# lms-07/LGTEUN

Hardware: AMD Instinct MI355X
Metric: train image-pairs/sec, GF-2 4-band 128x128, K=4, bs=32/GPU (higher is better)
Workload: dtype f32 (GEMMs and the local mixer: split 16-bit MFMA -- f16 pairs in the forward FFN, the W2 products of its backward and P V, bf16 triples elsewhere -- fp32 accumulate; fp32-equivalent); 1 GPU; BASELINE configs[1]: C=4, MS 32x32, PAN 128x128, K=4, 32 pairs/GPU, train step = fwd + L1 + bwd + Adam + StepLR tick; mode=faithful, global_batch=32, parallelism=dp1, dropout=True

## Files before the change

### include/lgteun_hip.h

```cpp
#ifndef LGTEUN_HIP_H
#define LGTEUN_HIP_H

#include <stddef.h>
#include <stdint.h>

#ifdef __cplusplus
extern "C" {
#endif

#define LG_TENSORS_SHARED 12
#define LG_TENSORS_PER_STAGE 119

#define LG_FLAG_FAITHFUL 1
#define LG_FLAG_SAVE 2
#define LG_FLAG_DROPOUT 4

#define LG_FLAG_BWD_LGT 8
#define LG_FLAG_BWD_DATA 16

#define LG_FLAG_CHAINED 32

#define LG_FLAG_DEFER_DEAD 64

#define LG_FLAG_STAGEWISE 128

#define LG_FLAG_LIVE_APART 256

enum lg_kernel_id {
    LG_K_NONE = 0, LG_K_FFN1, LG_K_FFN2, LG_K_FFT, LG_K_ATTN, LG_K_UPFUSE, LG_K_DOWN, LG_K_EMBED, LG_K_TAIL, LG_K_DATASTEP,
    LG_K_FFN1_BWD, LG_K_FFN2_BWD, LG_K_FFT_BWD, LG_K_ATTN_BWD, LG_K_WGRAD, LG_K_BATCH, LG_K_SCENE_GATHER, LG_K_SCENE_BLEND, LG_K_COUNT
};

typedef struct lg_config {
    int32_t C;
    int32_t K;
    int32_t H, W;
    int32_t precision;
    uint32_t variant;
} lg_config;

#define LG_VAR_FFN_IMPL_MASK 3u
#define LG_VAR_FFN_STRIP 1u
#define LG_VAR_FFN_SAVE_MASK (3u << 2)
#define LG_VAR_FFN_SAVE3 (1u << 2)
#define LG_VAR_FFN_SAVE5 (2u << 2)
#define LG_VAR_FFN_BWD32_PAIR (1u << 4)
#define LG_VAR_FFN_DWBWD_TILE (1u << 5)
#define LG_VAR_ATTN_BWD_R3 (1u << 6)
#define LG_VAR_DSTEP_TILES (1u << 7)
#define LG_VAR_ATTN_FWD_VALU (1u << 8)
#define LG_VAR_FFN_BF16X3 (1u << 9)
#define LG_VAR_FFT_FULL (1u << 10)
#define LG_VAR_FFN_BWD_BF16X3 (1u << 11)
#define LG_VAR_ATTN_BWD_CORE_M (1u << 12)
#define LG_VAR_FFN_XS (1u << 13)
#define LG_VAR_ATTN_BF16X3 (1u << 14)
#define LG_VAR_FFN_H3_RECOMPUTE (1u << 15)
#define LG_VAR_ATTN_BWD_RESTATS (1u << 16)
#define LG_VAR_REDUCE_PER_BLOCK (1u << 17)
#define LG_VAR_ALL 0x3ffffu

typedef struct lg_plan lg_plan;

const char* lg_version(void);
#define LG_ABI_VERSION 2
int32_t lg_abi_version(void);
const char* lg_last_error(void);

int lg_plan_create(const lg_config* cfg, const int64_t* offsets, int32_t n_offsets, lg_plan** out);
void lg_plan_destroy(lg_plan* plan);
int lg_plan_describe(const lg_plan* plan, char* buf, size_t n);
size_t lg_workspace_bytes(const lg_plan* plan, int32_t B, int32_t train);

int lgteun_forward(const lg_plan* plan, const float* params, const float* ms, const float* pan, float* out,
                   void* workspace, size_t workspace_bytes, int32_t B, int32_t flags, uint64_t seed, void* stream);

int lgteun_dead_forward(const lg_plan* plan, const float* params, void* workspace, size_t workspace_bytes, int32_t B, int32_t flags,
                        uint64_t seed, void* stream);

int lgteun_backward(const lg_plan* plan, const float* params, float* grads, const float* ms, const float* pan,
                    const float* dout, void* workspace, size_t workspace_bytes, int32_t B, int32_t flags,
                    uint64_t seed, void* stream);

int lg_l1_loss(const float* out, const float* gt, float* dout, float* loss_accum, int64_t n_local, int64_t n_global,
               float scale, void* stream);

int lg_adam_step(float* params, const float* grads, float* exp_avg, float* exp_avg_sq, const int64_t* ranges,
                 int32_t n_ranges, int64_t max_range, int32_t step, float lr, float beta1, float beta2, float eps,
                 float grad_scale, void* stream);

int lg_l2_loss(const float* out, const float* gt, float* dout, float* loss_accum, int64_t n_local, int64_t n_global,
               float scale, void* stream);

#define LG_OPT_ADAM 0
#define LG_OPT_ADAMW 1
#define LG_OPT_SGD 2
#define LG_OPT_RMSPROP 3
#define LG_OPT_AMSGRAD 1
#define LG_OPT_NESTEROV 2
#define LG_OPT_CENTERED 4
int lg_optim_step(float* params, const float* grads, float* state0, float* state1, float* state2, const int64_t* ranges,
                  int32_t n_ranges, int64_t max_range, int32_t step, int32_t algo, int32_t flags, double lr, double h0, double h1,
                  double eps, double weight_decay, double grad_scale, void* stream);

size_t lg_grad_norm_workspace_bytes(int32_t n_ranges, int64_t max_range);
int lg_grad_norm(const float* grads, const int64_t* ranges, int32_t n_ranges, int64_t max_range, double max_norm, float* out,
                 void* workspace, size_t workspace_bytes, void* stream);

int lg_optim_step_ex(float* params, const float* grads, float* state0, float* state1, float* state2, const int64_t* ranges,
                     int32_t n_ranges, int64_t max_range, int32_t step, int32_t algo, int32_t flags, double lr, double h0, double h1,
                     double eps, double weight_decay, double grad_scale, const float* clip_coef, float* ema, double ema_decay,
                     int32_t plain_adam, void* stream);

int lg_prof_enable(int32_t kernel_id, int32_t max_launches);
int lg_prof_reset(void);
void lg_prof_pause(int32_t paused);
int lg_prof_read(double* total_ms, int64_t* launches);
void lg_prof_disable(void);
const char* lg_kernel_name(int32_t kernel_id);

int lg_dropout_mask(uint64_t seed, int32_t stage, int32_t blk, int64_t first, int64_t n, float* out, void* stream);

int lg_op_resample(const float* x, float* y, int32_t planes, int32_t hi, int32_t wi, int32_t mode, void* stream);
int lg_op_data_step(const lg_plan* plan, const float* params, int32_t stage, const float* z_in, const float* ms,
                    const float* pan, float* z_out, float* tmp, int32_t B, void* stream);
int lg_op_lgt(const lg_plan* plan, const float* params, int32_t stage, const float* z, float* out, void* workspace,
              size_t workspace_bytes, int32_t B, int32_t flags, uint64_t seed, void* stream);
int lg_op_lgt_stages(const lg_plan* plan, const float* params, int32_t stage0, int32_t n, const float* z, float* out, void* workspace,
                     size_t workspace_bytes, int32_t B, int32_t flags, uint64_t seed, int32_t grid_cap, void* stream);
int lg_workspace_deadout(const lg_plan* plan, int32_t B, int32_t train, size_t* offset, size_t* stage_stride);
int lg_debug_live_slot(const lg_plan* plan, int32_t B, int32_t train, size_t* out53);
int lg_debug_stage_runs(int32_t kind, int32_t units, int32_t per_stage, int32_t grid, int32_t split, int32_t* out, int32_t n_out);
int lg_debug_stage_decision(int32_t kind, int32_t h, int32_t w, int32_t Bs, int32_t n, int32_t grid_cap, int32_t* out8);
int lg_op_block(const lg_plan* plan, const float* params, int32_t stage, int32_t blk, int32_t which, const float* x,
                float* y, void* workspace, size_t workspace_bytes, int32_t B, void* stream);

int lg_op_block_bwd(const lg_plan* plan, const float* params, float* grads, int32_t stage, int32_t blk, int32_t which,
                    const float* x, const float* dy, float* dx, void* workspace, size_t workspace_bytes, int32_t B,
                    void* stream);

int lg_op_data_step_bwd(const lg_plan* plan, const float* params, float* grads, int32_t stage, const float* z_in, const float* ms,
                        const float* pan, const float* dz_out, float* dz_in, void* workspace, size_t workspace_bytes, int32_t B,
                        void* stream);
int lg_op_lgt_bwd(const lg_plan* plan, const float* params, float* grads, int32_t stage, const float* z, const float* dout, float* dz,
                  void* workspace, size_t workspace_bytes, int32_t B, int32_t flags, uint64_t seed, void* stream);

#define LG_IQA_PEAK 2047.5
#define LG_IQA_SSIM_TAPS 11
#define LG_IQA_SSIM_SIGMA 1.5
#define LG_IQA_Q_BLOCK 8
#define LG_IQA_RATIO 4
#define LG_IQA_QNR_BLOCK 32
#define LG_IQA_MTF_TAPS 41
#define LG_IQA_MTF_GAIN 0.15
#define LG_IQA_MAX_BANDS 16
size_t lg_iqa_workspace_bytes(int32_t B, int32_t C, int32_t H, int32_t W, int32_t no_ref);
int lg_iqa_ref(const float* pred, const float* gt, double* out, int32_t B, int32_t C, int32_t H, int32_t W, float scale,
               void* workspace, size_t workspace_bytes, void* stream);
int lg_iqa_no_ref(const float* pred, const float* pan, const float* ms, double* out, int32_t B, int32_t C, int32_t H, int32_t W,
                  float scale, void* workspace, size_t workspace_bytes, void* stream);
int lg_iqa_mtf_taps(double* out41);

#define LG_IQA_Q2N_BLOCK 32
#define LG_IQA_Q2N_MAX_BANDS 8
size_t lg_iqa_ext_workspace_bytes(int32_t B, int32_t C, int32_t H, int32_t W);
int lg_iqa_ref_ext(const float* pred, const float* gt, double* out, int32_t B, int32_t C, int32_t H, int32_t W, float scale,
                   void* workspace, size_t workspace_bytes, void* stream);
int lg_iqa_q2n(const float* gt, const float* fused, double* out, int32_t B, int32_t C, int32_t H, int32_t W, float scale,
               void* workspace, size_t workspace_bytes, void* stream);

size_t lg_qnr_workspace_bytes(int32_t B, int32_t C, int32_t H, int32_t W);
int lg_qnr_stats(const float* out, const float* pan, const float* ms, const float* pan_l, double* q, double* table, int32_t B, int32_t C,
                 int32_t H, int32_t W, void* workspace, size_t workspace_bytes, void* stream);
int lg_qnr_grad(const float* out, const float* pan, const double* table, float* dout, float* loss_accum, double* indices, int32_t B,
                int64_t B_global, int32_t C, int32_t H, int32_t W, float scale, int32_t accumulate, const void* workspace,
                size_t workspace_bytes, void* stream);

size_t lg_recloss_workspace_bytes(int32_t B, int32_t C, int32_t H, int32_t W);
int lg_sam_loss(const float* out, const float* gt, float* dout, float* loss_accum, int32_t B, int64_t B_global, int32_t C, int32_t H, int32_t W,
                float scale, int32_t accumulate, void* workspace, size_t workspace_bytes, void* stream);
int lg_ssim_loss(const float* out, const float* gt, float* dout, float* loss_accum, int32_t B, int64_t B_global, int32_t C, int32_t H, int32_t W,
                 float scale, float data_range, int32_t accumulate, void* workspace, size_t workspace_bytes, void* stream);

#define LG_DT_U8 0
#define LG_DT_U16 1
#define LG_DT_F32 2
int lg_pyr_down2(const void* pan, float* pan_l, int64_t planes, int32_t H, int32_t W, int32_t dtype, void* stream);
int lg_batch_assemble(const void* pan, const void* lr, const void* mul, const float* pan_l, int64_t N, const int32_t* idx, int64_t idx_offset,
                      const uint32_t* flips, float* o_pan, float* o_lr, float* o_mul, float* o_pan_l, int32_t B, int32_t C, int32_t H, int32_t W,
                      int32_t h, int32_t w, int32_t dtype, float divisor, int32_t n_div, float post_scale, void* stream);

int lg_fir_decimate4(const void* in, void* out, const double* taps, int64_t planes, int32_t H, int32_t W, int32_t n_taps, int32_t phase,
                     int32_t dtype, int32_t out_f32, void* stream);
int lg_window_assemble(const void* pan, const void* lr, const void* mul, const int32_t* origins, int64_t n_windows, int64_t first,
                       const uint32_t* flips, float* o_pan, float* o_lr, float* o_mul, float* o_pan_l, int32_t B, int32_t C, int32_t Hs, int32_t Ws,
                       int32_t P, int32_t Q, int32_t dtype, float divisor, int32_t n_div, float post_scale, void* stream);

int lg_scene_gather(const void* pan, const void* ms, const int32_t* origins, int64_t n_tiles, int64_t first, float* o_pan, float* o_ms,
                    int32_t B, int32_t C, int32_t H, int32_t W, int32_t th, int32_t tw, int32_t dtype, float divisor, int32_t n_div,
                    float post_scale, void* stream);
int lg_scene_blend(const float* tiles, float* scene, int64_t first, int32_t B, int32_t C, int32_t H, int32_t W, int32_t th, int32_t tw,
                   int32_t overlap, void* stream);
int lg_scene_to_u16(const float* src, uint16_t* dst, int64_t n, float scale, void* stream);

#define LG_CLASSICAL_SFIM 0
#define LG_CLASSICAL_GSA 1
size_t lg_classical_workspace_bytes(int32_t B, int32_t C, int32_t h, int32_t w, int32_t method);
int lg_interp23_up4(const float* ms, float* out, int32_t B, int32_t C, int32_t h, int32_t w, void* stream);
int lg_sfim(const float* ms, const float* pan, float* out, int32_t B, int32_t C, int32_t h, int32_t w, void* workspace, size_t workspace_bytes,
            void* stream);
int lg_gsa(const float* ms, const float* pan, float* out, double* stats, int32_t B, int32_t C, int32_t h, int32_t w, void* workspace,
           size_t workspace_bytes, void* stream);
int lg_wavelet(const float* ms, const float* pan, float* out, int32_t B, int32_t C, int32_t h, int32_t w, void* stream);
// ... 16 lines not shown
```

### lgteun_amd/_lib.py

```python
import ctypes
import os
from ctypes import POINTER, c_char_p, c_double, c_float, c_int32, c_int64, c_size_t, c_uint64, c_void_p

_HERE = os.path.dirname(os.path.abspath(__file__))
LIB_PATH = os.environ.get('LGTEUN_HIP_LIB') or os.path.join(_HERE, '_lgteun_hip.so')

LG_FLAG_FAITHFUL = 1
LG_FLAG_SAVE = 2
LG_FLAG_DROPOUT = 4
LG_FLAG_BWD_LGT = 8
LG_FLAG_BWD_DATA = 16
LG_FLAG_CHAINED = 32
LG_FLAG_DEFER_DEAD = 64
LG_FLAG_STAGEWISE = 128
LG_FLAG_LIVE_APART = 256
KERNEL_IDS = {n: i for i, n in enumerate(['none', 'ffn1', 'ffn', 'fft', 'attn', 'upfuse', 'down', 'embed', 'tail', 'datastep', 'ffn1_bwd',
                                           'ffn2_bwd', 'fft_bwd', 'attn_bwd', 'wgrad', 'batch', 'scene_gather', 'scene_blend'])}


class LgConfig(ctypes.Structure):
    _fields_ = [('C', c_int32), ('K', c_int32), ('H', c_int32), ('W', c_int32), ('precision', c_int32), ('variant', ctypes.c_uint32)]


LG_VAR_FFN_STRIP = 1
LG_VAR_FFN_SAVE3, LG_VAR_FFN_SAVE5 = 1 << 2, 2 << 2
LG_VAR_FFN_BWD32_PAIR, LG_VAR_FFN_DWBWD_TILE, LG_VAR_ATTN_BWD_R3 = 1 << 4, 1 << 5, 1 << 6
LG_VAR_DSTEP_TILES = 1 << 7
LG_VAR_ATTN_FWD_VALU = 1 << 8
LG_VAR_FFN_BF16X3 = 1 << 9
LG_VAR_FFT_FULL = 1 << 10
LG_VAR_FFN_BWD_BF16X3 = 1 << 11
LG_VAR_ATTN_BWD_CORE_M = 1 << 12
LG_VAR_FFN_XS = 1 << 13
LG_VAR_ATTN_BF16X3 = 1 << 14
LG_VAR_FFN_H3_RECOMPUTE = 1 << 15
LG_VAR_ATTN_BWD_RESTATS = 1 << 16
LG_VAR_REDUCE_PER_BLOCK = 1 << 17
LG_OPT_ADAM, LG_OPT_ADAMW, LG_OPT_SGD, LG_OPT_RMSPROP = 0, 1, 2, 3
LG_OPT_AMSGRAD, LG_OPT_NESTEROV, LG_OPT_CENTERED = 1, 2, 4
LG_DT_U8, LG_DT_U16, LG_DT_F32 = 0, 1, 2
LG_CLASSICAL_SFIM, LG_CLASSICAL_GSA = 0, 1
LG_MTFGLP_GLP, LG_MTFGLP_HPM, LG_MTFGLP_CBD = 0, 1, 2
LG_ABI_VERSION = 2


def variant_from_env(env=None):
    env = os.environ if env is None else env
    v = {'strip': LG_VAR_FFN_STRIP, 'tile': 2, 'xp': 3}.get(env.get('LG_FFN_IMPL', ''), 0)
    v |= {'3': LG_VAR_FFN_SAVE3, '5': LG_VAR_FFN_SAVE5}.get(env.get('LG_FFN_SAVE', ''), 0)
    if env.get('LG_FFN_BWD32') == 'pair':
        v |= LG_VAR_FFN_BWD32_PAIR
    if env.get('LG_FFN_DWBWD') == 'tile':
        v |= LG_VAR_FFN_DWBWD_TILE
    if env.get('LG_ATTN_BWD') in ('old', 'r3'):
        v |= LG_VAR_ATTN_BWD_R3
    if env.get('LG_DSTEP') == 'tiles':
        v |= LG_VAR_DSTEP_TILES
    if env.get('LG_ATTN_FWD', '') == 'valu':
        v |= LG_VAR_ATTN_FWD_VALU
    if env.get('LG_FFN_SPLIT', '') == 'bf16x3':
        v |= LG_VAR_FFN_BF16X3
    if env.get('LG_FFT', '') == 'full':
        v |= LG_VAR_FFT_FULL
    if env.get('LG_FFN_BWD_SPLIT', '') == 'bf16x3':
        v |= LG_VAR_FFN_BWD_BF16X3
    if env.get('LG_ATTN_BWD_CORE', '') == 'm':
        v |= LG_VAR_ATTN_BWD_CORE_M
    if env.get('LG_FFN_FWD', '') == 'xs':
        v |= LG_VAR_FFN_XS
    if env.get('LG_ATTN_SPLIT', '') == 'bf16x3':
        v |= LG_VAR_ATTN_BF16X3
    if env.get('LG_FFN_H3', '') == 'recompute':
        v |= LG_VAR_FFN_H3_RECOMPUTE
    if env.get('LG_ATTN_BWD_STATS', '') == 'recompute':
        v |= LG_VAR_ATTN_BWD_RESTATS
    if env.get('LG_REDUCE', '') == 'per_block':
        v |= LG_VAR_REDUCE_PER_BLOCK
    return v


class LgteunHipError(RuntimeError):
    pass


_lib = None

SIGNATURES = {
    'lg_version': (c_char_p, []),
    'lg_abi_version': (c_int32, []),
    'lg_last_error': (c_char_p, []),
    'lg_plan_create': (c_int32, [POINTER(LgConfig), POINTER(c_int64), c_int32, POINTER(c_void_p)]),
    'lg_plan_destroy': (None, [c_void_p]),
    'lg_plan_describe': (c_int32, [c_void_p, c_char_p, c_size_t]),
    'lg_workspace_bytes': (c_size_t, [c_void_p, c_int32, c_int32]),
    'lgteun_forward': (c_int32, [c_void_p, c_void_p, c_void_p, c_void_p, c_void_p, c_void_p, c_size_t, c_int32, c_int32,
                                 c_uint64, c_void_p]),
    'lgteun_backward': (c_int32, [c_void_p, c_void_p, c_void_p, c_void_p, c_void_p, c_void_p, c_void_p, c_size_t, c_int32,
                                  c_int32, c_uint64, c_void_p]),
    'lgteun_dead_forward': (c_int32, [c_void_p, c_void_p, c_void_p, c_size_t, c_int32, c_int32, c_uint64, c_void_p]),
    'lg_l1_loss': (c_int32, [c_void_p, c_void_p, c_void_p, c_void_p, c_int64, c_int64, c_float, c_void_p]),
    'lg_adam_step': (c_int32, [c_void_p, c_void_p, c_void_p, c_void_p, c_void_p, c_int32, c_int64, c_int32, c_float, c_float,
                               c_float, c_float, c_float, c_void_p]),
    'lg_l2_loss': (c_int32, [c_void_p, c_void_p, c_void_p, c_void_p, c_int64, c_int64, c_float, c_void_p]),
    'lg_optim_step': (c_int32, [c_void_p, c_void_p, c_void_p, c_void_p, c_void_p, c_void_p, c_int32, c_int64, c_int32, c_int32, c_int32,
                                c_double, c_double, c_double, c_double, c_double, c_double, c_void_p]),
    'lg_grad_norm_workspace_bytes': (c_size_t, [c_int32, c_int64]),
    'lg_grad_norm': (c_int32, [c_void_p, c_void_p, c_int32, c_int64, c_double, c_void_p, c_void_p, c_size_t, c_void_p]),
    'lg_optim_step_ex': (c_int32, [c_void_p, c_void_p, c_void_p, c_void_p, c_void_p, c_void_p, c_int32, c_int64, c_int32, c_int32, c_int32,
                                   c_double, c_double, c_double, c_double, c_double, c_double, c_void_p, c_void_p, c_double, c_int32,
                                   c_void_p]),
    'lg_op_resample': (c_int32, [c_void_p, c_void_p, c_int32, c_int32, c_int32, c_int32, c_void_p]),
    'lg_op_data_step': (c_int32, [c_void_p, c_void_p, c_int32, c_void_p, c_void_p, c_void_p, c_void_p, c_void_p, c_int32,
                                  c_void_p]),
    'lg_op_lgt': (c_int32, [c_void_p, c_void_p, c_int32, c_void_p, c_void_p, c_void_p, c_size_t, c_int32, c_int32, c_uint64,
                            c_void_p]),
    'lg_op_lgt_stages': (c_int32, [c_void_p, c_void_p, c_int32, c_int32, c_void_p, c_void_p, c_void_p, c_size_t, c_int32, c_int32, c_uint64,
                                   c_int32, c_void_p]),
    'lg_debug_stage_runs': (c_int32, [c_int32, c_int32, c_int32, c_int32, c_int32, POINTER(c_int32), c_int32]),
    'lg_debug_stage_decision': (c_int32, [c_int32, c_int32, c_int32, c_int32, c_int32, c_int32, POINTER(c_int32)]),
    'lg_workspace_deadout': (c_int32, [c_void_p, c_int32, c_int32, POINTER(c_size_t), POINTER(c_size_t)]),
    'lg_debug_live_slot': (c_int32, [c_void_p, c_int32, c_int32, POINTER(c_size_t)]),
    'lg_op_block': (c_int32, [c_void_p, c_void_p, c_int32, c_int32, c_int32, c_void_p, c_void_p, c_void_p, c_size_t, c_int32,
                              c_void_p]),
    'lg_dropout_mask': (c_int32, [c_uint64, c_int32, c_int32, c_int64, c_int64, c_void_p, c_void_p]),
    'lg_prof_enable': (c_int32, [c_int32, c_int32]),
    'lg_prof_reset': (c_int32, []),
    'lg_prof_pause': (None, [c_int32]),
    'lg_prof_read': (c_int32, [POINTER(ctypes.c_double), POINTER(c_int64)]),
    'lg_prof_disable': (None, []),
    'lg_kernel_name': (c_char_p, [c_int32]),
    'lg_op_data_step_bwd': (c_int32, [c_void_p, c_void_p, c_void_p, c_int32, c_void_p, c_void_p, c_void_p, c_void_p, c_void_p, c_void_p,
                                      c_size_t, c_int32, c_void_p]),
    'lg_op_lgt_bwd': (c_int32, [c_void_p, c_void_p, c_void_p, c_int32, c_void_p, c_void_p, c_void_p, c_void_p, c_size_t, c_int32, c_int32,
                                c_uint64, c_void_p]),
    'lg_op_block_bwd': (c_int32, [c_void_p, c_void_p, c_void_p, c_int32, c_int32, c_int32, c_void_p, c_void_p, c_void_p, c_void_p,
                                  c_size_t, c_int32, c_void_p]),
    'lg_iqa_workspace_bytes': (c_size_t, [c_int32, c_int32, c_int32, c_int32, c_int32]),
    'lg_iqa_ref': (c_int32, [c_void_p, c_void_p, c_void_p, c_int32, c_int32, c_int32, c_int32, c_float, c_void_p, c_size_t, c_void_p]),
    'lg_iqa_no_ref': (c_int32, [c_void_p, c_void_p, c_void_p, c_void_p, c_int32, c_int32, c_int32, c_int32, c_float, c_void_p, c_size_t,
                                c_void_p]),
    'lg_iqa_mtf_taps': (c_int32, [c_void_p]),
    'lg_iqa_ext_workspace_bytes': (c_size_t, [c_int32, c_int32, c_int32, c_int32]),
    'lg_iqa_ref_ext': (c_int32, [c_void_p, c_void_p, c_void_p, c_int32, c_int32, c_int32, c_int32, c_float, c_void_p, c_size_t, c_void_p]),
    'lg_iqa_q2n': (c_int32, [c_void_p, c_void_p, c_void_p, c_int32, c_int32, c_int32, c_int32, c_float, c_void_p, c_size_t, c_void_p]),
    'lg_qnr_workspace_bytes': (c_size_t, [c_int32, c_int32, c_int32, c_int32]),
    'lg_qnr_stats': (c_int32, [c_void_p, c_void_p, c_void_p, c_void_p, c_void_p, c_void_p, c_int32, c_int32, c_int32, c_int32, c_void_p, c_size_t,
                               c_void_p]),
    'lg_qnr_grad': (c_int32, [c_void_p, c_void_p, c_void_p, c_void_p, c_void_p, c_void_p, c_int32, c_int64, c_int32, c_int32, c_int32, c_float,
                              c_int32, c_void_p, c_size_t, c_void_p]),
    'lg_recloss_workspace_bytes': (c_size_t, [c_int32, c_int32, c_int32, c_int32]),
    'lg_sam_loss': (c_int32, [c_void_p, c_void_p, c_void_p, c_void_p, c_int32, c_int64, c_int32, c_int32, c_int32, c_float, c_int32, c_void_p,
                              c_size_t, c_void_p]),
    'lg_ssim_loss': (c_int32, [c_void_p, c_void_p, c_void_p, c_void_p, c_int32, c_int64, c_int32, c_int32, c_int32, c_float, c_float, c_int32,
                               c_void_p, c_size_t, c_void_p]),
    'lg_pyr_down2': (c_int32, [c_void_p, c_void_p, c_int64, c_int32, c_int32, c_int32, c_void_p]),
    'lg_batch_assemble': (c_int32, [c_void_p, c_void_p, c_void_p, c_void_p, c_int64, c_void_p, c_int64, c_void_p, c_void_p, c_void_p, c_void_p,
                                    c_void_p, c_int32, c_int32, c_int32, c_int32, c_int32, c_int32, c_int32, c_float, c_int32, c_float, c_void_p]),
    'lg_fir_decimate4': (c_int32, [c_void_p, c_void_p, c_void_p, c_int64, c_int32, c_int32, c_int32, c_int32, c_int32, c_int32, c_void_p]),
    'lg_window_assemble': (c_int32, [c_void_p, c_void_p, c_void_p, c_void_p, c_int64, c_int64, c_void_p, c_void_p, c_void_p, c_void_p, c_void_p,
                                     c_int32, c_int32, c_int32, c_int32, c_int32, c_int32, c_int32, c_float, c_int32, c_float, c_void_p]),
    'lg_scene_gather': (c_int32, [c_void_p, c_void_p, c_void_p, c_int64, c_int64, c_void_p, c_void_p, c_int32, c_int32, c_int32, c_int32, c_int32,
                                  c_int32, c_int32, c_float, c_int32, c_float, c_void_p]),
    'lg_scene_blend': (c_int32, [c_void_p, c_void_p, c_int64, c_int32, c_int32, c_int32, c_int32, c_int32, c_int32, c_int32, c_void_p]),
    'lg_scene_to_u16': (c_int32, [c_void_p, c_void_p, c_int64, c_float, c_void_p]),
    'lg_classical_workspace_bytes': (c_size_t, [c_int32, c_int32, c_int32, c_int32, c_int32]),
    'lg_interp23_up4': (c_int32, [c_void_p, c_void_p, c_int32, c_int32, c_int32, c_int32, c_void_p]),
    'lg_sfim': (c_int32, [c_void_p, c_void_p, c_void_p, c_int32, c_int32, c_int32, c_int32, c_void_p, c_size_t, c_void_p]),
    'lg_gsa': (c_int32, [c_void_p, c_void_p, c_void_p, c_void_p, c_int32, c_int32, c_int32, c_int32, c_void_p, c_size_t, c_void_p]),
    'lg_wavelet': (c_int32, [c_void_p, c_void_p, c_void_p, c_int32, c_int32, c_int32, c_int32, c_void_p]),
    'lg_wavelet_taps': (c_int32, [c_void_p]),
    'lg_mtfglp_workspace_bytes': (c_size_t, [c_int32, c_int32, c_int32, c_int32, c_int32, c_int32]),
    'lg_mtf_glp': (c_int32, [c_void_p, c_void_p, c_void_p, c_void_p, c_void_p, c_int32, c_int32, c_int32, c_int32, c_int32, c_int32, c_int32, c_void_p,
                             c_size_t, c_void_p]),
    'lg_bdsd_workspace_bytes': (c_size_t, [c_int32, c_int32, c_int32, c_int32, c_int32]),
    'lg_bdsd': (c_int32, [c_void_p, c_void_p, c_void_p, c_void_p, c_void_p, c_int32, c_void_p, c_int32, c_int32, c_int32, c_int32, c_int32, c_int32, c_void_p,
                          c_size_t, c_void_p]),
}


def lib():
    global _lib
    if _lib is None:
        if not os.path.exists(LIB_PATH):
            raise LgteunHipError(
                f'HIP extension not built: {LIB_PATH} is missing. Run `make` (or __graft_entry__.build()). '
                'lgteun_amd has no CPU/PyTorch fallback.')
        L = ctypes.CDLL(LIB_PATH)
        for name, (res, args) in SIGNATURES.items():
            fn = getattr(L, name)
            fn.restype = res
            fn.argtypes = args
        got = int(L.lg_abi_version())
        if got != LG_ABI_VERSION:
            raise LgteunHipError(f'{LIB_PATH}: ABI version {got}, this binding was written for {LG_ABI_VERSION} (include/lgteun_hip.h): rebuild with `make`')
        _lib = L
    return _lib


def check(rc, what):
    if rc != 0:
        msg = lib().lg_last_error().decode(errors='replace')
        raise LgteunHipError(f'{what} failed (rc={rc}): {msg}')
```

### lgteun_amd/csrc/api.hip

```cpp
#include <stdarg.h>
#include <stdio.h>
#include <stdlib.h>
#include <string.h>

#include "abi.h"
#include "kernels.h"
#include "workspace.h"
#include "forward.h"
#include "backward.h"

static thread_local char g_err[512] = "";

void lg_set_error(const char* fmt, ...) {
    va_list ap;
    va_start(ap, fmt);
    vsnprintf(g_err, sizeof(g_err), fmt, ap);
    va_end(ap);
}

extern "C" const char* lg_version(void) { return "lgteun_hip 0.2 (gfx950)"; }
extern "C" int32_t lg_abi_version(void) { return LG_ABI_VERSION; }
extern "C" const char* lg_last_error(void) { return g_err; }

static void lg_plan_stage_batch(lg_plan* p);
// ... 44 lines not shown
    free(plan->off);
    delete plan;
}

extern "C" int lg_plan_describe(const lg_plan* plan, char* buf, size_t n) {
    if (!plan) { lg_set_error("plan_describe: null argument"); return -1; }
    return lg_describe_route(plan->cfg, plan->route, buf, n);
}

extern "C" size_t lg_workspace_bytes(const lg_plan* plan, int32_t B, int32_t train) {
    if (!plan || B <= 0 || train < 0 || train > 2) return 0;
    NetBufs nb;
    carve(plan, B, train, nullptr, nb);
    size_t fwd = nb.bytes;
    if (train) fwd += bwd_workspace_bytes(plan, B);
    return fwd;
}

extern "C" int lg_workspace_deadout(const lg_plan* plan, int32_t B, int32_t train, size_t* offset, size_t* stage_stride) {
    if (!plan || B <= 0 || train < 0 || train > 2 || !offset || !stage_stride) { lg_set_error("workspace_deadout: invalid argument"); return -1; }
    NetBufs nb;
    char base[1];
    carve(plan, B, train, base, nb);
    *offset = (size_t)(reinterpret_cast<char*>(nb.deadout) - base);
    *stage_stride = (plan->stage_batch && train != 2) ? (size_t)B * plan->cfg.C * plan->cfg.H * plan->cfg.W * sizeof(float) : 0;
    return 0;
}

extern "C" int lg_debug_live_slot(const lg_plan* plan, int32_t B, int32_t train, size_t* out53) {
    if (!plan || B <= 0 || train < 0 || train > 2 || !out53) { lg_set_error("debug_live_slot: invalid argument"); return -1; }
    NetBufs nb;
    char base[1];
    carve(plan, B, train, base, nb);
    const NetBufs lv = live_view(nb);
    size_t* o = out53;
    *o++ = nb.bytes; *o++ = train ? bwd_workspace_bytes(plan, B) : 0; *o++ = nb.live_s0;
    auto off = [&](const float* p) { return (size_t)(reinterpret_cast<const char*>(p) - base); };
    for (int j = 0; j < LG_NBLK; ++j) {
        const BlockBufs &a = nb.blk[j], &l = lv.blk[j];
        const float* pa[5] = {a.xin, a.xmid, a.xout, a.g, a.o2};
        const float* pl[5] = {l.xin, l.xmid, l.xout, l.g, l.o2};
        for (int f = 0; f < 5; ++f) { *o++ = off(pa[f]); *o++ = off(pl[f]); }
    }
    return 0;
}

extern "C" int lgteun_backward(const lg_plan* plan, const float* params, float* grads, const float* ms, const float* pan,
                               const float* dout, void* workspace, size_t workspace_bytes, int32_t B, int32_t flags, uint64_t seed,
                               void* stream) {
    if (!plan || !params || !grads || !ms || !pan || !dout || !workspace || B <= 0) { lg_set_error("backward: null/invalid argument"); return -1; }
    if ((flags & LG_FLAG_CHAINED) && (flags & (LG_FLAG_BWD_LGT | LG_FLAG_BWD_DATA))) {
        lg_set_error("backward: LG_FLAG_BWD_LGT / LG_FLAG_BWD_DATA do not apply to LG_FLAG_CHAINED");
        return -2;
    }
    NetBufs nb;
    if (int rc = carve_checked("backward", plan, B, (flags & LG_FLAG_CHAINED) ? 2 : 1, workspace, workspace_bytes, nb)) return rc;
    return net_backward(plan, params, grads, ms, pan, dout, nb, (char*)workspace + nb.bytes, B, flags, seed, (hipStream_t)stream);
}

extern "C" int lg_op_resample(const float* x, float* y, int32_t planes, int32_t hi, int32_t wi, int32_t mode, void* stream) {
    if (!x || !y || planes <= 0 || hi <= 0 || wi <= 0 || mode < 0 || mode > 2) { lg_set_error("op_resample: invalid argument"); return -1; }
    if (mode == 0 && ((hi & 1) || (wi & 1))) { lg_set_error("op_resample: x0.5 needs even sizes"); return -2; }
    return launch_resample(mode, x, y, planes, hi, wi, (hipStream_t)stream);
}

extern "C" int lg_op_data_step(const lg_plan* plan, const float* params, int32_t stage, const float* z_in, const float* ms,
                               const float* pan, float* z_out, float* tmp, int32_t B, void* stream) {
    if (!plan || !params || !z_in || !ms || !pan || !z_out || !tmp || stage < 0 || stage >= plan->cfg.K) { lg_set_error("op_data_step: invalid argument"); return -1; }
    const lg_config& c = plan->cfg;
    size_t q = (size_t)B * c.C * c.H * c.W / 4;
    return data_step_fwd(plan, params, stage, z_in, ms, pan, z_out, tmp, tmp + q, tmp + 2 * q, tmp + 3 * q, B, (hipStream_t)stream);
}

extern "C" int lg_op_lgt(const lg_plan* plan, const float* params, int32_t stage, const float* z, float* out, void* workspace,
                         size_t workspace_bytes, int32_t B, int32_t flags, uint64_t seed, void* stream) {
    if (!plan || !params || !z || !out || !workspace || stage < 0 || stage >= plan->cfg.K) { lg_set_error("op_lgt: invalid argument"); return -1; }
    NetBufs nb;
    if (int rc = carve_checked("op_lgt", plan, B, (flags & LG_FLAG_SAVE) ? 1 : 0, workspace, workspace_bytes, nb)) return rc;
    nb = live_view(nb);
    if (int rc = prep_stages(plan, params, stage, stage + 1, nb, (hipStream_t)stream)) return rc;
    return lgt_fwd(plan, params, stage, z, out, nb, B, flags, seed, (hipStream_t)stream);
}

extern "C" int lg_op_lgt_stages(const lg_plan* plan, const float* params, int32_t stage0, int32_t n, const float* z, float* out, void* workspace,
                                size_t workspace_bytes, int32_t B, int32_t flags, uint64_t seed, int32_t grid_cap, void* stream) {
    if (!plan || !params || !z || !out || !workspace || B <= 0 || stage0 < 0 || n < 1 || stage0 + n > plan->cfg.K || grid_cap < 0) { lg_set_error("op_lgt_stages: invalid argument"); return -1; }
    if (flags & ~LG_FLAG_DROPOUT) { lg_set_error("op_lgt_stages: only LG_FLAG_DROPOUT applies (nothing is saved)"); return -2; }
    if (n > 1 && (!plan->stage_batch || n > plan->cfg.K - 1)) { lg_set_error("op_lgt_stages: this plan runs one stage per pass (lg_plan_stage_batch), or n > K-1"); return -2; }
    NetBufs nb;
    if (int rc = carve_checked("op_lgt_stages", plan, B, 0, workspace, workspace_bytes, nb)) return rc;
    hipStream_t s = (hipStream_t)stream;
    if (int rc = prep_stages(plan, params, stage0, stage0 + n, nb, s)) return rc;
    return lgt_fwd(plan, params, stage0, z, out, nb, B, flags, seed, s, n, (long)B * plan->cfg.C * plan->cfg.H * plan->cfg.W, grid_cap);
}

extern "C" int lg_debug_stage_runs(int32_t kind, int32_t units, int32_t per_stage, int32_t grid, int32_t split, int32_t* out, int32_t n_out) {
    if (kind < 0 || kind > 1 || units <= 0 || per_stage <= 0 || units % per_stage || grid <= 0 || !out || n_out < 0 || (int64_t)units * grid >= (1ll << 31)) {
        lg_set_error("debug_stage_runs: invalid argument");
        return -1;
    }
    const bool uneven = kind == 0 ? split != 0 : split != 4;
    if (!uneven && grid > units) { lg_set_error("debug_stage_runs: more workgroups than units"); return -1; }
    if (uneven && ((grid & 1) || (kind == 0 ? 2 * units < grid : units < grid) || (kind == 1 && (split < 1 || split > 7)))) { lg_set_error("debug_stage_runs: an uneven split needs an even grid, a unit per workgroup and 1 <= eighths <= 7"); return -2; }
    int rows = 0;
    for (int wg = 0; wg < grid; ++wg) {
        const StageRun r = !uneven ? stage_run_even(units, grid, wg) : (kind == 0 ? stage_run_pairs(units, grid, wg) : stage_run_chunk(units, grid, wg, split));
        int seg0 = r.run0;
        do {
            const int st = seg0 / per_stage, seg1 = stage_seg_end(st, r.run1, per_stage);
            if (rows < n_out) { int32_t* o = out + 5 * (size_t)rows; o[0] = wg; o[1] = seg0; o[2] = seg1; o[3] = st; o[4] = r.base; }
            ++rows;
            seg0 = seg1;
        } while (seg0 < r.run1);
    }
    return rows;
}

extern "C" int lg_debug_stage_decision(int32_t kind, int32_t h, int32_t w, int32_t Bs, int32_t n, int32_t grid_cap, int32_t* out8) {
    if ((kind != 0 && kind != 8 && kind != 16) || h <= 0 || w <= 0 || Bs <= 0 || n < 1 || grid_cap < 0 || !out8 || (int64_t)Bs * n * h * w >= (1ll << 31)) { lg_set_error("debug_stage_decision: invalid argument"); return -1; }
    if (kind == 0) {
        const XrGeo q = ffn_xr_geometry(h, w, Bs * n, Bs, n, grid_cap);
        const int sh = q.dS ? 1 : 0;
        const int32_t o[8] = {q.dS != 0, q.dS, q.nstrips >> sh, (Bs * q.tiles_x * q.strips_y) >> sh, q.grid, q.SH, q.tiles_x, q.strips_y};
        memcpy(out8, o, sizeof(o));
    } else {
        if ((h & 7) || (w & 7) || (Bs * (h / 8) * (w / 8)) % 4) { lg_set_error("debug_stage_decision: not whole window quads per stage"); return -2; }
        const AttnMGeo q = attn_m_geometry(kind, h, w, Bs * n, n, grid_cap, 2);
        const int32_t o[8] = {q.uneven != 0, q.uneven ? q.uneven : 4, q.nquads, q.nquads / n, q.grid, q.nwin, 0, 0};
        memcpy(out8, o, sizeof(o));
    }
    return 0;
}

extern "C" int lg_op_block(const lg_plan* plan, const float* params, int32_t stage, int32_t blk, int32_t which, const float* x,
                           float* y, void* workspace, size_t workspace_bytes, int32_t B, void* stream) {
    if (!plan || !params || !x || !y || !workspace || stage < 0 || stage >= plan->cfg.K || blk < 0 || blk > 4 || which < 0 || which > 2) {
        lg_set_error("op_block: invalid argument");
        return -1;
    }
    hipStream_t s = (hipStream_t)stream;
    NetBufs nb;
    int rc;
    if ((rc = carve_checked("op_block", plan, B, 0, workspace, workspace_bytes, nb))) return rc;
    nb = live_view(nb);
    Blk k = nb.block(plan, params, nullptr, stage, blk);
    BlockBufs& bb = k.b;
    if (which == 0 || which == 1) {
        if ((rc = launch_ln_split(bb.e, x, k.p(B_LN1G), k.p(B_LN1B), bb.g, B, bb.h * bb.w, s))) return rc;
    }
    if (which == 0) {
        FftArgs f;
        f.g = bb.g; f.o = y; f.amp = nullptr; f.pha = nullptr; f.sgn = nullptr; f.scratch = nb.fft_scratch;
        f.ampw = k.p(B_AMPW); f.ampb = k.p(B_AMPB); f.phaw = k.p(B_PHAW); f.phab = k.p(B_PHAB);
        f.ch = bb.e / 2; f.planes = B * f.ch; f.n = bb.h; f.h = bb.h; f.w = bb.w; f.full = plan->route.fft_full;
        return launch_fftmix(f, s);
    }
    if ((rc = prep_stages(plan, params, stage, stage + 1, nb, s))) return rc;
    if (which == 1) {
        bb.xin = const_cast<float*>(x);
        bb.xmid = y;
        return block_mixer_fwd(k, B, 0, 0, s);
    }
    bb.xmid = const_cast<float*>(x);
    bb.xout = y;
    return block_ffn_fwd(k, nullptr, B, 0, s);
}

extern "C" int lg_op_block_bwd(const lg_plan* plan, const float* params, float* grads, int32_t stage, int32_t blk, int32_t which,
                               const float* x, const float* dy, float* dx, void* workspace, size_t workspace_bytes, int32_t B,
                               void* stream) {
    if (!plan || !params || !grads || !x || !dy || !dx || !workspace || stage < 0 || stage >= plan->cfg.K || blk < 0 || blk > 4 ||
        which < 0 || which > 2) {
        lg_set_error("op_block_bwd: invalid argument");
        return -1;
    }
    hipStream_t s = (hipStream_t)stream;
    NetBufs nb;
    int rc;
    if ((rc = carve_checked("op_block_bwd", plan, B, 1, workspace, workspace_bytes, nb))) return rc;
    nb = live_view(nb);
    Blk k = nb.block(plan, params, grads, stage, blk);
    BlockBufs& bb = k.b;
    if (which == 0 || which == 1) {
        if ((rc = launch_ln_split(bb.e, x, k.p(B_LN1G), k.p(B_LN1B), bb.g, B, bb.h * bb.w, s))) return rc;
        if ((rc = prep_stages(plan, params, stage, stage + 1, nb, s))) return rc;
        bb.xin = const_cast<float*>(x);
        if ((rc = block_mixer_fwd(k, B, LG_FLAG_SAVE, 0, s))) return rc;
    } else {
        bb.xmid = const_cast<float*>(x);
        if ((rc = prep_stages(plan, params, stage, stage + 1, nb, s))) return rc;
        if ((rc = block_ffn_fwd(k, nullptr, B, LG_FLAG_SAVE, s))) return rc;
    }
    return op_block_bwd(k, which, dy, dx, (char*)workspace + nb.bytes, B, s);
}

extern "C" int lg_op_data_step_bwd(const lg_plan* plan, const float* params, float* grads, int32_t stage, const float* z_in,
                                   const float* ms, const float* pan, const float* dz_out, float* dz_in, void* workspace,
                                   size_t workspace_bytes, int32_t B, void* stream) {
    if (!plan || !params || !grads || !z_in || !ms || !pan || !dz_out || !dz_in || !workspace || B <= 0 || stage < 0 || stage >= plan->cfg.K) {
        lg_set_error("op_data_step_bwd: invalid argument");
        return -1;
    }
    hipStream_t s = (hipStream_t)stream;
    NetBufs nb;
    int rc;
    if ((rc = carve_checked("op_data_step_bwd", plan, B, 1, workspace, workspace_bytes, nb))) return rc;
    if ((rc = data_step_fwd(plan, params, stage, z_in, ms, pan, nb.Z[stage + 1], nb.t1[stage], nb.r[stage], nb.s1[stage], nb.pr, B, s))) return rc;
    return op_data_step_bwd(plan, params, grads, stage, nb, (char*)workspace + nb.bytes, z_in, pan, dz_out, dz_in, B, s);
}

extern "C" int lg_op_lgt_bwd(const lg_plan* plan, const float* params, float* grads, int32_t stage, const float* z, const float* dout,
                             float* dz, void* workspace, size_t workspace_bytes, int32_t B, int32_t flags, uint64_t seed, void* stream) {
    if (!plan || !params || !grads || !z || !dout || !dz || !workspace || B <= 0 || stage < 0 || stage >= plan->cfg.K) {
        lg_set_error("op_lgt_bwd: invalid argument");
        return -1;
    }
    if (flags & ~LG_FLAG_DROPOUT) { lg_set_error("op_lgt_bwd: only LG_FLAG_DROPOUT applies"); return -2; }
    hipStream_t s = (hipStream_t)stream;
    NetBufs nb;
    int rc;
    if ((rc = carve_checked("op_lgt_bwd", plan, B, 1, workspace, workspace_bytes, nb))) return rc;
    nb = live_view(nb);
    if ((rc = prep_stages(plan, params, stage, stage + 1, nb, s))) return rc;
    if ((rc = lgt_fwd(plan, params, stage, z, nb.deadout, nb, B, flags | LG_FLAG_SAVE, seed, s))) return rc;
    return op_lgt_bwd(plan, params, grads, stage, nb, (char*)workspace + nb.bytes, z, dout, dz, B, flags, seed, s);
}
```

### lgteun_amd/csrc/bwd_kernels.h

```cpp
#pragma once
#include "common.h"

struct WgradArgs {
    const void* Y;
    const void* X;
    float* dW;
    float* db;
    long P;
    int ldy, ldx, ldw;
    int N, K;
    int n_valid, k_valid;
    int ybf, xbf;
    int xgelu;
};
size_t wgrad_slab_floats(int N, int K, long P);
#define PIXEL_PART_WGS 2048
size_t chan_partial_floats(int C, int B, int H, int W);
struct ChanReduce {
    float* dst[14];
    float* dst2[14];
    int stride[14];
    int NK, C, nslices;
    unsigned allc_mask;
};
// ... 125 lines not shown
    float* du;
    const float* dskip;
    float* dx;
    const float* w;
    int B, H, W;
};
int launch_down_bwd_a(int E, const DownBwdArgs& a, hipStream_t s);
int launch_down_bwd_b(int E, const DownBwdArgs& a, hipStream_t s);

struct UpFuseBwdArgs {
    const float* dy;
    float* dt;
    float* dskip;
    float* v;
    float* dxb;
    float* tmp;
    const float *fw, *upw;
    int B, H, W;
};
int launch_upfuse_bwd_a(int E, const UpFuseBwdArgs& a, hipStream_t s);
int launch_upfuse_bwd_b(int E, const UpFuseBwdArgs& a, hipStream_t s);

struct FfnDwBwdArgs {
    const float* dy;
    const void* g3;
    const void* h2;
    void* dh2;
    int hbf;
    int pre;
    const float *w3t;
    const float* dww;
    float *slab_w, *slab_b;
    float *d_dww, *d_dwb;
    int B, h, w;
};
size_t ffn_dw_bwd_slab_floats(int e, int B, int h, int w);
int launch_ffn_dw_bwd(int e, const FfnDwBwdArgs& a, hipStream_t s);
struct Ffn1BwdArgs {
    const void* dh2;
    const void* g1;
    const float* x;
    const float* dy;
    void* dh1;
    float* y2;
    float* dx;
    const float *w2t, *w1t, *ln2g, *ln2b;
    float *d_ln2g, *d_ln2b;
    float* part;
    float *w1slab, *d_w1, *d_b1;
    float *w2slab, *d_w2, *d_b2;
    long P;
    int hbf;
    int pre;
    const float* w1;
    void* wsplit;
};
#define FFN1_BWD_WGS 512
inline bool ffn1_bwd_fuses_w1(int e) { return e <= 32; }
#ifndef LG_FW2
#define LG_FW2 0
#endif
inline bool ffn1_bwd_fuses_w2(int e, int pre) { return LG_FW2 && pre && e == 16; }
int launch_ffn1_bwd(int e, Ffn1BwdKernel k, const Ffn1BwdArgs& a, hipStream_t s);
int launch_ffn1_bwd_x32(const Ffn1BwdArgs& a, const float* w1, void* wsplit, hipStream_t s);
struct Ffn1BwdXArgs {
    const void* dh2;
    int hbf;
    const float* x;
    const float* dy;
    float* dx;
    const float *w1, *b1;
    const float *w2t, *w1t;
    const float *ln2g, *ln2b;
    float* slab;
    float *d_w1, *d_b1, *d_w2, *d_b2, *d_ln2g, *d_ln2b;
    long P;
    const float* scales = nullptr;
};
inline int ffn1_bwd_x_wgs(int e) { return e == 16 ? 512 : 256; }
size_t ffn1_bwd_x_slab_floats(int e);
int launch_ffn1_bwd_xs(int e, const Ffn1BwdXArgs& a, hipStream_t s);
struct FfnDwBwdXArgs {
    const float* dy;
    const void* h3;
    const void* h2;
    void* dh2;
    int hbf;
    const float* w3t;
    const float* dww;
    const float* dwb = nullptr;
    float* slab;
    float *d_dww, *d_dwb, *d_w3, *d_b3;
    int B, h, w;
    float* dh2_max = nullptr;
};
#define FFN_DW_BWD_X_WGS 512
#define FFN_DW_BWD_X_DB 576
#define FFN_DW_BWD_X_W3 640
#define FFN_DW_BWD_X_B3 1664
#define FFN_DW_BWD_X_ROW 1680
#define FFN_DW_BWD_X32_ROW 2720
inline size_t ffn_dw_bwd_x_slab_floats(int e) { return (size_t)FFN_DW_BWD_X_WGS * (e == 16 ? FFN_DW_BWD_X_ROW : FFN_DW_BWD_X32_ROW); }
int launch_ffn_dw_bwd_xs(int e, const FfnDwBwdXArgs& a, hipStream_t s);
#define FFN_DW_BWD_H_WGS 512
#define FFN_DW_BWD_H_ROW 848
inline size_t ffn_dw_bwd_h_slab_floats() { return (size_t)2 * FFN_DW_BWD_H_WGS * FFN_DW_BWD_H_ROW; }
int launch_ffn_dw_bwd_h(const FfnDwBwdXArgs& a, hipStream_t s);
inline int reduce_ffn_dw_bwd_slab(const FfnDwBwdXArgs& a, int e, int nhalf, int gx, int r_db, int r_w3, int r_b3, int row, hipStream_t s) {
    const int n1 = 4 * e, nh = n1 / nhalf;
    ReduceJob j;
    j.dst2 = nullptr; j.nslices = gx; j.slice_stride = row;
    int rc = 0;
    for (int half = 0; half < nhalf && !rc; ++half) {
        const float* base = a.slab + (size_t)half * gx * row;
        auto job = [&](int off, float* dst, int rows, int cols, int ld) {
            j.slab = base + off; j.dst = dst; j.rows = rows; j.cols = cols; j.row_stride = cols; j.ld = ld; j.rows_valid = rows; j.cols_valid = cols;
            return launch_reduce_job(j, s);
        };
        rc = job(0, a.d_dww + (size_t)half * nh * 9, nh, 9, 9);
        if (!rc) rc = job(r_db, a.d_dwb + half * nh, 1, nh, nh);
        if (!rc) rc = job(r_w3, a.d_w3 + half * nh, e, nh, n1);
        if (!rc && half == 0) rc = job(r_b3, a.d_b3, 1, e, e);
    }
    return rc;
}
int launch_transpose(const float* src, float* dst, int rows, int cols, hipStream_t s);
int launch_transpose3(const float* const* src, float* const* dst, const int* rows, const int* cols, int njobs, hipStream_t s, float* const* clear = nullptr, int nclear = 0);

struct ProjO2BwdArgs {
    const float* dy;
    float* do2;
    float* dym;
    const float* projw;
    int HW;
    long total;
    int dropout;
    uint64_t seed;
};
int launch_proj_o2_bwd(int e, const ProjO2BwdArgs& a, hipStream_t s);

struct FftBwdArgs {
    const float* do2;
    const float* sgn;
    const float* amp;
    const float* pha;
    float* dg;
    float* scratch;
    const float *ampw, *ampb, *phaw, *phab;
    float *d_ampw, *d_ampb, *d_phaw, *d_phab;
    float* part;
    int planes, ch, n;
    int h, w;
    int full = 0;
};
size_t fft_bwd_part_floats(int planes, int h, int w);
int launch_fftmix_bwd(const FftBwdArgs& a, hipStream_t s);

struct AttnBwdArgs {
    const float* x;
    const float* dy;
    const float* dym;
    const float* o2;
    const float* dg;
    float* dx;
    float* cat;
    float* y1;
    float* dqkv;
    const float* pos;
    const float* unused = nullptr;
    float* dpos_slab;
    const float *ln1g, *ln1b, *qkvw, *qkvb, *projw;
    float *d_ln1g, *d_ln1b;
    float *d_qkvw, *d_qkvb;
    float* part;
    int B, h, w;
    const float* so = nullptr;
    const float* sl = nullptr;
    float* stats = nullptr;
    int core_m = 0;
};
int launch_attn_bwd_core_m(int e, const AttnBwdArgs& a, int grid, int nwin, int ngroups, hipStream_t s);
#ifndef LG_ATTN_FUSE_QKV
#define LG_ATTN_FUSE_QKV 1
#endif
constexpr bool attn_bwd_fuses_qkv(int e) { return LG_ATTN_FUSE_QKV && e == 16; }
inline size_t attn_bwd_part_floats(int e) { return (size_t)PIXEL_PART_WGS * 2 * e + (attn_bwd_fuses_qkv(e) ? (size_t)1024 * ((3 * e / 2) * (e / 2) + 3 * e / 2) : 0); }
int attn_bwd_grid(int e, int B, int h, int w);
int launch_attn_bwd(int e, const AttnBwdArgs& a, hipStream_t s);

struct ProjO2BwdKArgs {
    const float* dy;
    float* do2;
    uint32_t* keep;
    const float* projw;
    float* slab;
    float* d_projb;
    int HW;
    long total;
    uint64_t seed;
};
#ifndef PROJ_O2_K_WGS
#define PROJ_O2_K_WGS 512
#endif
int launch_proj_o2_bwd_k(int e, const ProjO2BwdKArgs& a, hipStream_t s);
struct AttnBwdFArgs {
    const float* x;
    const float* dy;
    const uint32_t* keep;
    const float* o2;
    const float* dg;
    float* dx;
    const float* pos;
    const float *ln1g, *ln1b, *qkvw, *qkvb, *projw;
    const float* so = nullptr;
    const float* sl = nullptr;
    float* slab;
    float *d_pos, *d_qkvw, *d_qkvb, *d_projw, *d_ln1g, *d_ln1b;
    int B, h, w;
    unsigned rcp_nwx, rcp_nwy;
};
#define ATTN_BWD_F_WGS 256
#define ATTN_BWD_F_WQ 8192
#define ATTN_BWD_F_ROW (8192 + 192 + 24 + 256 + 32)
inline bool attn_bwd_fused(int e) { return e == 16; }
int attn_bwd_f_grid(int B, int h, int w);
int launch_attn_bwd_f(int e, const AttnBwdFArgs& a, hipStream_t s);
```

### lgteun_amd/csrc/k_bwd.hip

```cpp
#include <string.h>

#include "kernels.h"
#include "bwd_kernels.h"
#include "backward.h"

struct BwdBufs {
    float *dzA, *dzB, *gu3, *gs1, *gu1, *gr, *gd3, *gt1, *gd1;
    float *dx[3];
    float *dh2, *dh1, *y2, *do2, *dg, *dym, *cat, *y1, *dqkv;
    float *w3t[LG_NBLK], *w2t[LG_NBLK], *w1t[LG_NBLK], *wsp, *dt, *dskip, *v, *du;
    float* slab_arena;
    float* attn_stats;
    size_t slab_cap;
    ReduceQueue rq;
    size_t bytes;
};

static const size_t R3_DPOS_SLAB = 512 * POS_TABLE;
static size_t dpos_slab_floats() {
    const size_t f = (size_t)ATTN_BWD_F_WGS * ATTN_BWD_F_ROW;
    return f > R3_DPOS_SLAB ? f : R3_DPOS_SLAB;
}
static void carve_bwd(const lg_plan* plan, int B, void* base, BwdBufs& bb) {
    const lg_config& c = plan->cfg;
    Carver cv{reinterpret_cast<char*>(base), 0};
    const size_t P0 = (size_t)c.H * c.W * B, P1 = P0 / 4, E = 4 * (size_t)c.C, C = c.C;
    bb.dzA = cv.take(C * P0); bb.dzB = cv.take(C * P0); bb.gu3 = cv.take(C * P0);
    bb.gs1 = cv.take(C * P1); bb.gu1 = cv.take(C * P1); bb.gt1 = cv.take(C * P1); bb.gd1 = cv.take(C * P1);
    bb.gr = cv.take(C * P1 / 4); bb.gd3 = cv.take(C * P1 / 4);
    for (int i = 0; i < 3; ++i) bb.dx[i] = cv.take(P0 * E);
    bb.dh2 = cv.take(P0 * 4 * E); bb.dh1 = cv.take(P0 * 4 * E);
    bb.y2 = cv.take(P0 * E); bb.do2 = cv.take(P0 * E / 2); bb.dg = cv.take(P0 * E / 2);
    bb.dym = cv.take(P0 * E); bb.cat = cv.take(P0 * E); bb.y1 = cv.take(P0 * 16 > P0 * E / 2 ? P0 * 16 : P0 * E / 2);
    bb.dqkv = cv.take(P0 * 2 * E);
    bb.attn_stats = cv.take(P0 * 8);
    for (int j = 0; j < LG_NBLK; ++j) { bb.w3t[j] = cv.take(8 * E * 2 * E); bb.w2t[j] = cv.take(8 * E * 8 * E); bb.w1t[j] = cv.take(8 * E * 2 * E); }
    bb.wsp = cv.take(ffn_wsplit_bytes(32) / sizeof(float));
    size_t sl = wgrad_slab_floats((int)(8 * E), (int)(8 * E), (long)P0);
    size_t sl2 = wgrad_slab_floats(64, 64, (long)P0);
    size_t sl3 = ffn_dw_bwd_slab_floats((int)E, B, c.H, c.W);
    if (sl2 > sl) sl = sl2;
    size_t sl4 = chan_partial_floats(c.C, B, c.H, c.W);
    const size_t sl5 = (size_t)PIXEL_PART_WGS * (2 * 8 * c.C + 2 * c.C);
    if (sl5 > sl4) sl4 = sl5;
    if (sl4 > sl) sl = sl4;
    if (sl3 > sl) sl = sl3;
    for (const FfnRoute& fr : plan->route.ffn)
        if (fr.px == FFN1_BWD_XS && ffn1_bwd_x_slab_floats(fr.e) > sl) sl = ffn1_bwd_x_slab_floats(fr.e);
    if (ffn_dw_bwd_x_slab_floats(16) > sl) sl = ffn_dw_bwd_x_slab_floats(16);
    if (ffn_dw_bwd_x_slab_floats(32) > sl) sl = ffn_dw_bwd_x_slab_floats(32);
    if (ffn_dw_bwd_h_slab_floats() > sl) sl = ffn_dw_bwd_h_slab_floats();
    bb.slab_cap = LG_NBLK * (4 * sl + dpos_slab_floats());
    bb.slab_arena = cv.take(bb.slab_cap);
    bb.dt = cv.take(P0 * E); bb.dskip = cv.take(P0 * E); bb.v = cv.take(P1 * E); bb.du = cv.take(P1 * E);
    bb.bytes = cv.off;
}

size_t bwd_workspace_bytes(const lg_plan* plan, int B) {
    BwdBufs bb;
    carve_bwd(plan, B, nullptr, bb);
    return bb.bytes;
}

#define RC(x) do { int rc__ = (x); if (rc__) return rc__; } while (0)

struct ReduceQueueScope {
    explicit ReduceQueueScope(BwdBufs& bb, hipStream_t s, bool per_block) {
        bb.rq.init(bb.slab_arena, bb.slab_cap, s, per_block);
        reduce_queue_begin(&bb.rq);
    }
    ~ReduceQueueScope() { (void)reduce_queue_end(); }
};

static int wgrad(const void* Y, int ldy, const void* X, int ldx, float* dW, int ldw, float* db, long P, int N, int K, int nv, int kv,
                 int ybf, int xbf, BwdBufs& bb, hipStream_t s, int xgelu = 0) {
    float* slab = bb.rq.take(wgrad_slab_floats(N, K, P));
    if (!slab) return -3;
    WgradArgs a;
    a.Y = Y; a.X = X; a.dW = dW; a.db = db; a.P = P; a.ldy = ldy; a.ldx = ldx; a.ldw = ldw; a.N = N; a.K = K;
    a.n_valid = nv; a.k_valid = kv; a.ybf = ybf; a.xbf = xbf; a.xgelu = xgelu;
    return launch_wgrad(a, slab, s);
}

static int ffn_transposes(const Blk* blocks, int nk, BwdBufs& bb, hipStream_t s) {
    const float* tsrc[3 * LG_NBLK];
    float* tdst[3 * LG_NBLK];
    float* clear[LG_NBLK];
    int trows[3 * LG_NBLK], tcols[3 * LG_NBLK], n = 0, nclear = 0;
    for (int i = 0; i < nk; ++i) {
        const Blk& k = blocks[i];
        const int j = k.j, e = k.b.e, n1 = 4 * e;
        tsrc[n] = k.p(B_W3); tdst[n] = bb.w3t[j]; trows[n] = e; tcols[n] = n1; ++n;
        tsrc[n] = k.p(B_W2); tdst[n] = bb.w2t[j]; trows[n] = n1; tcols[n] = n1; ++n;
        tsrc[n] = k.p(B_W1); tdst[n] = bb.w1t[j]; trows[n] = n1; tcols[n] = e; ++n;
        if (k.pl->ffn(e).bwd_scales) clear[nclear++] = k.ffn_scales + 6;
    }
    return launch_transpose3(tsrc, tdst, trows, tcols, n, s, clear, nclear);
}

static int ffn_half_bwd(const Blk& k, BwdBufs& bb, const float* dy, float* tmp, int B, hipStream_t s) {
    const BlockBufs& fb = k.b;
    const FfnRoute& fr = k.pl->ffn(fb.e);
    const int j = k.j, e = fb.e, n1 = 4 * e;
    const int hbf = fr.hbf ? 1 : 0;
    const int pre = fr.pre ? 1 : 0;
    const long Pn = (long)B * fb.h * fb.w;
    float* fsc = fr.bwd_scales ? k.ffn_scales : nullptr;
    if (fr.dw == FFN_DWBWD_TILE) {
        FfnDwBwdArgs fd;
        fd.dy = dy; fd.g3 = pre ? fb.a3 : fb.g3; fd.h2 = fb.h2; fd.dh2 = bb.dh2; fd.w3t = bb.w3t[j]; fd.dww = k.p(B_DWW);
        fd.slab_w = bb.rq.take(ffn_dw_bwd_slab_floats(e, B, fb.h, fb.w));
        if (!fd.slab_w) return -3;
        fd.slab_b = fd.slab_w + ffn_dw_bwd_slab_floats(e, B, fb.h, fb.w) / 10 * 9;
        fd.d_dww = k.g(B_DWW); fd.d_dwb = k.g(B_DWB);
        fd.B = B; fd.h = fb.h; fd.w = fb.w; fd.hbf = hbf; fd.pre = pre;
        RC(launch_ffn_dw_bwd(e, fd, s));
    } else {
        const bool h3re = fr.dw == FFN_DWBWD_H;
        FfnDwBwdXArgs fk;
        fk.dy = dy; fk.h3 = h3re ? nullptr : fb.a3; fk.h2 = fb.h2; fk.dh2 = bb.dh2; fk.w3t = bb.w3t[j]; fk.dww = k.p(B_DWW); fk.dwb = k.p(B_DWB);
        fk.slab = bb.rq.take(h3re ? ffn_dw_bwd_h_slab_floats() : ffn_dw_bwd_x_slab_floats(e));
        if (!fk.slab) return -3;
        fk.d_dww = k.g(B_DWW); fk.d_dwb = k.g(B_DWB); fk.d_w3 = k.g(B_W3); fk.d_b3 = k.g(B_B3);
        fk.B = B; fk.h = fb.h; fk.w = fb.w; fk.hbf = hbf;
        fk.dh2_max = fsc ? fsc + 6 : nullptr;
        RC(h3re ? launch_ffn_dw_bwd_h(fk, s) : launch_ffn_dw_bwd_xs(e, fk, s));
    }
    if (fr.px == FFN1_BWD_XS) {
        Ffn1BwdXArgs fx;
        fx.scales = fsc;
        fx.dh2 = bb.dh2; fx.x = fb.xmid; fx.dy = dy; fx.dx = tmp;
        fx.w1 = k.p(B_W1); fx.b1 = k.p(B_B1); fx.w2t = bb.w2t[j]; fx.w1t = bb.w1t[j]; fx.ln2g = k.p(B_LN2G); fx.ln2b = k.p(B_LN2B);
        fx.slab = bb.rq.take(ffn1_bwd_x_slab_floats(e));
        if (!fx.slab) return -3;
        fx.d_w1 = k.g(B_W1); fx.d_b1 = k.g(B_B1); fx.d_w2 = k.g(B_W2); fx.d_b2 = k.g(B_B2); fx.d_ln2g = k.g(B_LN2G); fx.d_ln2b = k.g(B_LN2B);
        fx.P = Pn; fx.hbf = hbf;
        RC(launch_ffn1_bwd_xs(e, fx, s));
    } else {
        Ffn1BwdArgs f1;
        f1.dh2 = bb.dh2; f1.g1 = pre ? fb.a1 : fb.g1; f1.x = fb.xmid; f1.dy = dy; f1.dh1 = bb.dh1; f1.y2 = bb.y2; f1.dx = tmp;
        f1.w2t = bb.w2t[j]; f1.w1t = bb.w1t[j];
        f1.ln2g = k.p(B_LN2G); f1.ln2b = k.p(B_LN2B);
        f1.d_ln2g = k.g(B_LN2G); f1.d_ln2b = k.g(B_LN2B); f1.part = bb.rq.take((size_t)PIXEL_PART_WGS * 2 * e);
        if (!f1.part) return -3;
        f1.P = Pn; f1.hbf = hbf; f1.pre = pre;
        f1.w1 = nullptr; f1.wsplit = nullptr;
        if (fr.px == FFN1_BWD_X32) { f1.w1 = k.p(B_W1); f1.wsplit = bb.wsp; }
        f1.w1slab = nullptr; f1.d_w1 = nullptr; f1.d_b1 = nullptr;
        if (!fr.wgrad_w1) {
            f1.w1slab = bb.rq.take((size_t)FFN1_BWD_WGS * ((size_t)n1 * e + n1));
            if (!f1.w1slab) return -3;
            f1.d_w1 = k.g(B_W1); f1.d_b1 = k.g(B_B1);
        }
        f1.w2slab = nullptr; f1.d_w2 = nullptr; f1.d_b2 = nullptr;
        if (!fr.wgrad_w2) {
            f1.w2slab = bb.rq.take((size_t)FFN1_BWD_WGS * ((size_t)n1 * n1 + n1));
            if (!f1.w2slab) return -3;
            f1.d_w2 = k.g(B_W2); f1.d_b2 = k.g(B_B2);
        }
        RC(launch_ffn1_bwd(e, fr.px, f1, s));
    }
    if (fr.wgrad_w2) RC(wgrad(bb.dh2, n1, fb.a1, n1, k.g(B_W2), n1, k.g(B_B2), Pn, n1, n1, n1, n1, hbf, hbf, bb, s, pre));
    if (fr.wgrad_w1) RC(wgrad(bb.dh1, n1, bb.y2, e, k.g(B_W1), e, k.g(B_B1), Pn, n1, e, n1, e, hbf, 0, bb, s));
    if (fr.wgrad_w3) RC(wgrad(dy, e, fb.a3, n1, k.g(B_W3), n1, k.g(B_B3), Pn, e, n1, e, n1, 0, hbf, bb, s, pre));
    return 0;
}

static int fft_bwd_call(const Blk& k, const float* do2, float* dg, int B, hipStream_t s, float* part) {
    const BlockBufs& fb = k.b;
    const int hc = fb.e / 2;
    FftBwdArgs fa;
    fa.do2 = do2; fa.sgn = fb.sgn; fa.amp = fb.amp; fa.pha = fb.pha; fa.dg = dg; fa.scratch = k.fft_scratch;
    fa.ampw = k.p(B_AMPW); fa.ampb = k.p(B_AMPB); fa.phaw = k.p(B_PHAW); fa.phab = k.p(B_PHAB);
    fa.d_ampw = k.g(B_AMPW); fa.d_ampb = k.g(B_AMPB); fa.d_phaw = k.g(B_PHAW); fa.d_phab = k.g(B_PHAB);
    fa.ch = hc; fa.planes = B * hc; fa.n = fb.h; fa.h = fb.h; fa.w = fb.w; fa.part = part; fa.full = k.pl->route.fft_full;
    return launch_fftmix_bwd(fa, s);
}

static int mixer_half_bwd(const Blk& k, BwdBufs& bb, const float* tmp, float* dx_out, int B, int flags, uint64_t seed, hipStream_t s) {
    const BlockBufs& fb = k.b;
    const int e = fb.e, hc = e / 2;
    const long Pn = (long)B * fb.h * fb.w;
    const int drop = (flags & LG_FLAG_DROPOUT) ? 1 : 0;
    const MixerRoute& mr = k.pl->mixer(e);
    if (mr.bwd == ATTN_BWD_F) {
        uint32_t* keep = drop ? reinterpret_cast<uint32_t*>(bb.dym) : nullptr;
        ProjO2BwdKArgs pk;
        pk.dy = tmp; pk.do2 = bb.do2; pk.keep = keep; pk.projw = k.p(B_PROJW);
        pk.slab = bb.rq.take((size_t)PROJ_O2_K_WGS * e);
        if (!pk.slab) return -3;
        pk.d_projb = k.g(B_PROJB); pk.HW = fb.h * fb.w; pk.total = Pn; pk.seed = mix_seed(seed, k.st, k.j);
        RC(launch_proj_o2_bwd_k(e, pk, s));
        float* fpart = bb.rq.take(fft_bwd_part_floats(B * hc, fb.h, fb.w));
        if (!fpart) return -3;
        RC(fft_bwd_call(k, bb.do2, bb.dg, B, s, fpart));
        AttnBwdFArgs af;
        af.x = fb.xin; af.dy = tmp; af.keep = keep; af.o2 = fb.o2; af.dg = bb.dg; af.dx = dx_out;
        af.pos = k.p(B_POS); af.ln1g = k.p(B_LN1G); af.ln1b = k.p(B_LN1B); af.qkvw = k.p(B_QKVW); af.qkvb = k.p(B_QKVB); af.projw = k.p(B_PROJW);
        af.slab = bb.rq.take((size_t)ATTN_BWD_F_WGS * ATTN_BWD_F_ROW);
        if (!af.slab) return -3;
        af.d_pos = k.g(B_POS); af.d_qkvw = k.g(B_QKVW); af.d_qkvb = k.g(B_QKVB); af.d_projw = k.g(B_PROJW); af.d_ln1g = k.g(B_LN1G); af.d_ln1b = k.g(B_LN1B);
        af.B = B; af.h = fb.h; af.w = fb.w;
        if (mr.stats) { af.so = fb.att_o; af.sl = fb.att_l; }
        return launch_attn_bwd_f(e, af, s);
    }
    ProjO2BwdArgs po;
    po.dy = tmp; po.do2 = bb.do2; po.dym = drop ? bb.dym : nullptr; po.projw = k.p(B_PROJW);
    po.HW = fb.h * fb.w; po.total = Pn; po.dropout = drop; po.seed = mix_seed(seed, k.st, k.j);
    RC(launch_proj_o2_bwd(e, po, s));
    const float* dym = drop ? bb.dym : tmp;
    float* fpart = bb.rq.take(fft_bwd_part_floats(B * hc, fb.h, fb.w));
    if (!fpart) return -3;
    RC(fft_bwd_call(k, bb.do2, bb.dg, B, s, fpart));
    AttnBwdArgs at;
    at.x = fb.xin; at.dy = tmp; at.dym = dym; at.o2 = fb.o2; at.dg = bb.dg; at.dx = dx_out;
    at.cat = bb.cat; at.y1 = bb.y1; at.dqkv = bb.dqkv;
    at.pos = k.p(B_POS); at.dpos_slab = bb.rq.take(R3_DPOS_SLAB);
    if (!at.dpos_slab) return -3;
    at.ln1g = k.p(B_LN1G); at.ln1b = k.p(B_LN1B); at.qkvw = k.p(B_QKVW); at.qkvb = k.p(B_QKVB); at.projw = k.p(B_PROJW);
    at.d_ln1g = k.g(B_LN1G); at.d_ln1b = k.g(B_LN1B); at.part = bb.rq.take(attn_bwd_part_floats(e));
    at.d_qkvw = k.g(B_QKVW); at.d_qkvb = k.g(B_QKVB);
    if (attn_bwd_fuses_qkv(e)) at.y1 = nullptr;
    if (!at.part) return -3;
    at.B = B; at.h = fb.h; at.w = fb.w; at.core_m = mr.bwd == ATTN_BWD_R3_CORE_M ? 1 : 0; at.stats = bb.attn_stats;
    if (mr.stats) { at.so = fb.att_o; at.sl = fb.att_l; }
    RC(launch_attn_bwd(e, at, s));
    const int grid = attn_bwd_grid(e, B, fb.h, fb.w);
    RC(launch_reduce_slab(at.dpos_slab, grid, 1, POS_TABLE, k.g(B_POS), POS_TABLE, 1, POS_TABLE, s));
    RC(wgrad(dym, e, bb.cat, e, k.g(B_PROJW), e, k.g(B_PROJB), Pn, e, e, e, e, 0, 0, bb, s));
    if (!attn_bwd_fuses_qkv(e)) {
        const int y1ld = (hc + 15) / 16 * 16, dqld = (3 * hc + 15) / 16 * 16;
        RC(wgrad(bb.dqkv, dqld, bb.y1, y1ld, k.g(B_QKVW), hc, k.g(B_QKVB), Pn, dqld, y1ld, 3 * hc, hc, 0, 0,
                 bb, s));
    }
    return 0;
}

static int block_bwd(const Blk& k, BwdBufs& bb, const float* dy, float* tmp, float* dx_out, int B, int flags, uint64_t seed, hipStream_t s) {
    RC(ffn_half_bwd(k, bb, dy, tmp, B, s));
    RC(mixer_half_bwd(k, bb, tmp, dx_out, B, flags, seed, s));
    return bb.rq.block_end();
}

int op_block_bwd(const Blk& k, int which, const float* dy, float* dx, void* bwd_ws, int B, hipStream_t s) {
    BwdBufs bb;
    carve_bwd(k.pl, B, bwd_ws, bb);
    if (which == 0) return fft_bwd_call(k, dy, dx, B, s, bb.slab_arena);
    ReduceQueueScope rqs(bb, s, k.pl->route.reduce_per_block);
    int rc = which == 1 ? 0 : ffn_transposes(&k, 1, bb, s);
    if (!rc) rc = which == 1 ? mixer_half_bwd(k, bb, dy, dx, B, 0, 0, s) : ffn_half_bwd(k, bb, dy, dx, B, s);
    const int rc2 = reduce_queue_end();
    return rc ? rc : rc2;
}

static int data_step_bwd(const lg_plan* pl, const float* P, float* G, int st, const NetBufs& nb, BwdBufs& bb, const float* zin,
                         const float* pan, const float* g, float* dz, int B, hipStream_t s) {
    const lg_config& c = pl->cfg;
    const int planes = B * c.C, H = c.H, W = c.W;
    if (pl->route.dstep_fused) {
        DstepBwdArgs a;
        a.g = g; a.z = zin; a.pan = pan; a.t1 = nb.t1[st]; a.r = nb.r[st]; a.s1 = nb.s1[st]; a.dz = dz;
        a.d1w = P + pl->shared(S_D1W); a.d3w = P + pl->shared(S_D3W); a.dt1w = P + pl->shared(S_DT1W); a.dt3w = P + pl->shared(S_DT3W);
        a.dt3b = P + pl->shared(S_DT3B);
        a.rw = P + pl->shared(S_RW); a.rb = P + pl->shared(S_RB); a.rtw = P + pl->shared(S_RTW); a.rtb = P + pl->shared(S_RTB);
        a.eta = P + pl->eta(st);
        a.B = B; a.C = c.C; a.N = H;
        float* part = bb.rq.take(dstep_bwd_part_floats(c.C, B, H));
        if (!part) return -3;
        const size_t bc = (size_t)B * c.C;
        a.part_top = part; a.part_dt1 = part + 14 * bc; a.part_d3 = part + 24 * bc; a.part_d1 = part + 34 * bc; a.part_pre = part + 44 * bc;
        DstepBwdGrads gg;
        gg.d1w = G + pl->shared(S_D1W); gg.d1b = G + pl->shared(S_D1B); gg.d3w = G + pl->shared(S_D3W); gg.d3b = G + pl->shared(S_D3B);
        gg.dt1w = G + pl->shared(S_DT1W); gg.dt1b = G + pl->shared(S_DT1B); gg.dt3w = G + pl->shared(S_DT3W); gg.dt3b = G + pl->shared(S_DT3B);
        gg.rw = G + pl->shared(S_RW); gg.rb = G + pl->shared(S_RB); gg.rtw = G + pl->shared(S_RTW); gg.rtb = G + pl->shared(S_RTB);
        gg.eta = G + pl->eta(st);
        RC(launch_dstep_bwd(a, gg, s));
        return bb.rq.block_end();
    }
    DstepTopArgs t;
    t.g = g; t.s1 = nb.s1[st]; t.z = zin; t.pan = pan; t.gu = bb.gu3; t.dz = dz;
    t.w9 = P + pl->shared(S_DT3W); t.b9 = P + pl->shared(S_DT3B);
    t.rw = P + pl->shared(S_RW); t.rb = P + pl->shared(S_RB); t.rtw = P + pl->shared(S_RTW); t.rtb = P + pl->shared(S_RTB);
    t.eta = P + pl->eta(st);
    t.dw9 = G + pl->shared(S_DT3W); t.dbias = G + pl->shared(S_DT3B);
    t.drw = G + pl->shared(S_RW); t.drb = G + pl->shared(S_RB); t.drtw = G + pl->shared(S_RTW); t.drtb = G + pl->shared(S_RTB);
    t.deta = G + pl->eta(st);
    t.C = c.C; t.B = B; t.H = H; t.W = W; t.part = bb.rq.take(chan_partial_floats(c.C, B, H, W));
    if (!t.part) return -3;
    RC(launch_dstep_top_bwd(t, s));
    RC(launch_resample_adj(1, bb.gu3, bb.gs1, planes, H / 2, W / 2, 0, s));
    DwBwdArgs d;
    d.C = c.C; d.planes = planes;
    d.gout = bb.gs1; d.in = nb.r[st]; d.gin = bb.gu1; d.w9 = P + pl->shared(S_DT1W);
    d.dw9 = G + pl->shared(S_DT1W); d.dbias = G + pl->shared(S_DT1B);
    d.hi = H / 4; d.wi = W / 4; d.n_h = H / 2; d.n_w = W / 2;
    d.part = bb.rq.take(chan_partial_floats(c.C, B, H, W));
    if (!d.part) return -3;
    RC(launch_dw_bwd(1, d, s));
    RC(launch_resample_adj(1, bb.gu1, bb.gr, planes, H / 4, W / 4, 0, s));
    d.gout = bb.gr; d.in = nb.t1[st]; d.gin = bb.gd3; d.w9 = P + pl->shared(S_D3W);
    d.dw9 = G + pl->shared(S_D3W); d.dbias = G + pl->shared(S_D3B);
    d.hi = H / 2; d.wi = W / 2; d.n_h = H / 4; d.n_w = W / 4;
    d.part = bb.rq.take(chan_partial_floats(c.C, B, H, W));
    if (!d.part) return -3;
    RC(launch_dw_bwd(0, d, s));
    RC(launch_resample_adj(0, bb.gd3, bb.gt1, planes, H / 2, W / 2, 0, s));
    d.gout = bb.gt1; d.in = zin; d.gin = bb.gd1; d.w9 = P + pl->shared(S_D1W);
    d.dw9 = G + pl->shared(S_D1W); d.dbias = G + pl->shared(S_D1B);
    d.hi = H; d.wi = W; d.n_h = H / 2; d.n_w = W / 2;
    d.part = bb.rq.take(chan_partial_floats(c.C, B, H, W));
    if (!d.part) return -3;
    RC(launch_dw_bwd(0, d, s));
    RC(launch_resample_adj(0, bb.gd1, dz, planes, H, W, 1, s));
    return bb.rq.block_end();
}

static int lgt_bwd(const lg_plan* pl, const float* P, float* G, int st, const NetBufs& nb, BwdBufs& bb, const float* dout,
                   const float* zin, int B, int flags, uint64_t seed, hipStream_t s) {
    const lg_config& c = pl->cfg;
    const int E = 4 * c.C;
    const long P0 = (long)B * c.H * c.W, P1 = P0 / 4;
    const LgtSlots L{pl, P, G, st};
    Blk k[LG_NBLK];
    for (int j = 0; j < LG_NBLK; ++j) k[j] = nb.block(pl, P, G, st, j);
    float *A = bb.dx[0], *Bf = bb.dx[1], *Cf = bb.dx[2];
    RC(ffn_transposes(k, LG_NBLK, bb, s));
    TailBwdArgs tb;
    tb.dout = dout; tb.x = nb.blk[4].xout; tb.dx = A; tb.dz = bb.dzA; tb.w = L.p(L_TAILW);
// ... 89 lines not shown
```

### lgteun_amd/csrc/k_fft.hip

```cpp
#include <math.h>
#include <string.h>

#include "kernels.h"
#include "bwd_kernels.h"

#define FFT_LD(n) ((n) + 1)
__constant__ float2 c_tw512[256];
static int lg_num_cus() {
    static std::atomic<int> cus[64];
    int d = 0; (void)hipGetDevice(&d); d &= 63;
    int c = cus[d].load(std::memory_order_relaxed);
    if (!c) {
        if (hipDeviceGetAttribute(&c, hipDeviceAttributeMultiprocessorCount, d) != hipSuccess || c <= 0) c = 256;
        cus[d].store(c, std::memory_order_relaxed);
    }
    return c;
}
static int fft_const_twiddles() {
    static DeviceOnce once;
    if (once.need()) {
        float2 h[256];
        for (int k = 0; k < 256; ++k) {
            const double ang = 2.0 * 3.14159265358979323846 * (double)k / 512.0;
            h[k] = make_float2((float)cos(ang), (float)(0.0 - sin(ang)));
// ... 152 lines not shown
}
template <bool INVERSE, bool COLS>
__device__ __forceinline__ void fft_pass(float2* buf, const float2* tw, int n, int lg) {
    if (COLS) fft_lines<INVERSE, 1>(buf, tw, lg, lg, 1, FFT_LD(n));
    else fft_lines<INVERSE, 0, true, INVERSE>(buf, tw, lg, lg, FFT_LD(n), 1);
}

__device__ __forceinline__ void edit_sincos(float x, float& sn, float& cs) {
    if (__builtin_amdgcn_ballot_w64(!(fabsf(x) <= 100.0f)) != 0) { sincosf(x, &sn, &cs); return; }
    const float k = rintf(x * 0.63661977236758134f);
    float r = fmaf(k, -1.57073974609375f, x);
    r = fmaf(k, -5.657970905303955078e-05f, r);
    r = fmaf(k, -9.920936294705029468e-10f, r);
    const float s = r * r;
    const float ps = fmaf(fmaf(-1.9515295891e-4f, s, 8.3321608736e-3f), s, -1.6666654611e-1f);
    const float si = fmaf(ps * s, r, r);
    const float pc = fmaf(fmaf(2.443315711809948e-5f, s, -1.388731625493765e-3f), s, 4.166664568298827e-2f);
    const float co = fmaf(pc * s, s, fmaf(-0.5f, s, 1.0f));
    const unsigned kq = (unsigned)(int)k;
    const float a = (kq & 1u) ? co : si, b = (kq & 1u) ? si : co;
    sn = __uint_as_float(__float_as_uint(a) ^ ((kq & 2u) << 30));
    cs = __uint_as_float(__float_as_uint(b) ^ (((kq + 1u) & 2u) << 30));
}
__device__ __forceinline__ void edit_abs_angle(float2 f, float& amp, float& pha) {
    const float ax = fabsf(f.x), ay = fabsf(f.y);
    const float mx = fmaxf(ax, ay), mn = fminf(ax, ay);
    if (__builtin_amdgcn_ballot_w64(!(mx <= 1e18f) || (mx < 1e-18f && mx > 0.0f)) != 0) { amp = hypotf(f.x, f.y); pha = atan2f(f.y, f.x); return; }
    amp = __builtin_amdgcn_sqrtf(fmaf(f.x, f.x, f.y * f.y));
    const float r = __builtin_amdgcn_rcpf(mx);
    float q = mn * r;
    q = fmaf(fmaf(-mx, q, mn), r, q);
    q = mx == 0.0f ? 0.0f : q;
    const float t = q * q;
    float p = -0.0017540286062285304f;
    p = fmaf(p, t, 0.010727421380579472f); p = fmaf(p, t, -0.030805569142103195f); p = fmaf(p, t, 0.05755317956209183f);
    p = fmaf(p, t, -0.08377385884523392f); p = fmaf(p, t, 0.10942058265209198f); p = fmaf(p, t, -0.14261938631534576f);
    p = fmaf(p, t, 0.1999826729297638f); p = fmaf(p, t, -0.3333328366279602f);
    p = fmaf(p * t, q, q);
    p = ay > ax ? (1.57079637050628662f - p) + -4.37113883e-8f : p;
    p = (__float_as_uint(f.x) >> 31) ? (3.14159274101257324f - p) + -8.74227766e-8f : p;
    pha = copysignf(p, f.y);
}

__device__ __forceinline__ float2 bin_edit_fwd(float2 f, float aw, float ab, float pw, float pb, float& amp, float& pha) {
    edit_abs_angle(f, amp, pha);
    const float am = aw * amp + ab, ph = pw * pha + pb;
    float sn, cs;
    edit_sincos(ph, sn, cs);
    return make_float2((am * cs + 1e-8f) + 1e-8f, am * sn + 1e-8f);
}
__device__ __forceinline__ float2 bin_edit_bwd(float2 f, float c, float nn, float A, float PH, float aw, float ab, float pw, float pb,
                                               float& s_aw, float& s_ab, float& s_pw, float& s_pb) {
    const float dR = f.x * (c / nn), dI = f.y * (c / nn);
    const float Am = aw * A + ab, Ph = pw * PH + pb;
    float sn, cs;
    edit_sincos(Ph, sn, cs);
    const float dAm = dR * cs + dI * sn;
    const float dPh = Am * (dI * cs - dR * sn);
    s_aw += dAm * A; s_ab += dAm; s_pw += dPh * PH; s_pb += dPh;
    const float dA = aw * dAm, dPH = pw * dPh;
    float sn0, cs0;
    edit_sincos(PH, sn0, cs0);
    float dFr = 0.f, dFi = 0.f;
    if (A > 0.f) {
        const float ia = 1.0f / A;
        dFr = dA * cs0 - dPH * sn0 * ia;
        dFi = dA * sn0 + dPH * cs0 * ia;
    }
    const float k2 = nn / c;
    return make_float2(dFr * k2, dFi * k2);
}

__device__ __forceinline__ void half_bin(int it, int n, int lg, int& q, int& p, int& c) {
    const int half = n >> 1;
    if (it < n * half) { q = it >> (lg - 1); c = it & (half - 1); p = 2 * c; }
    else { q = it - n * half; c = half; p = 1; }
}

__host__ __device__ constexpr int fft_threads(int lg) { return lg >= 7 ? 1024 : (lg >= 6 ? 512 : 256); }

template <int LG>
__global__ void k_fftmix(FftArgs a) {
    extern __shared__ float2 smem2[];
    constexpr int lg = LG, n = 1 << LG, half = n >> 1;
    constexpr int LD = FFT_LD(n);
    float2* buf = smem2;
    float2* tw = smem2 + n * LD;
    const int plane = blockIdx.x;
    const int ch = plane % a.ch;
    const float* g = a.g + (size_t)plane * n * n;
    for (int k = threadIdx.x; k < half; k += blockDim.x) {
        float ang = 2.0f * (float)k / (float)n;
        tw[k] = make_float2(cospif(ang), 0.0f - sinpif(ang));
    }
    {
        constexpr int NTH = fft_threads(LG), NLD = (n * n / 4 + NTH - 1) / NTH;
        float4 v[NLD];
#pragma unroll
        for (int k = 0; k < NLD; ++k) { const int i = (k * NTH + (int)threadIdx.x) * 4; v[k] = *reinterpret_cast<const float4*>(g + (i < n * n ? i : 0)); }
#pragma unroll
        for (int k = 0; k < NLD; ++k) {
            const int i = (k * NTH + (int)threadIdx.x) * 4;
            if (i < n * n) {
                float2* d = buf + (i >> lg) * LD + (i & (n - 1));
                d[0] = make_float2(v[k].x, 0.0f); d[1] = make_float2(v[k].y, 0.0f); d[2] = make_float2(v[k].z, 0.0f); d[3] = make_float2(v[k].w, 0.0f);
            }
        }
    }
    __syncthreads();
    fft_pass<false, false>(buf, tw, n, lg);
    for (int y = threadIdx.x; y < n; y += blockDim.x) { buf[y * LD + 0].y = 0.0f; buf[y * LD + 1].y = 0.0f; }
    __syncthreads();
    fft_pass<false, true>(buf, tw, n, lg);
    if (threadIdx.x < 4) buf[(threadIdx.x >> 1) * LD + (threadIdx.x & 1)].y = 0.0f;
    __syncthreads();
    const float aw = a.ampw[ch], ab = a.ampb[ch], pw = a.phaw[ch], pb = a.phab[ch];
    for (int it = threadIdx.x; it < n * (half + 1); it += blockDim.x) {
        int q, p, c;
        half_bin(it, n, lg, q, p, c);
        float amp, pha;
        const float2 ed = bin_edit_fwd(buf[q * LD + p], aw, ab, pw, pb, amp, pha);
        if (a.amp) {
            size_t o = ((size_t)plane * n + q) * (half + 1) + c;
            __builtin_nontemporal_store(amp, a.amp + o);
            __builtin_nontemporal_store(pha, a.pha + o);
        }
        buf[q * LD + p] = ed;
    }
    __syncthreads();
    fft_pass<true, true>(buf, tw, n, lg);
    fft_pass<true, false>(buf, tw, n, lg);
    const float sc = 1.0f / ((float)n * (float)n);
    float* o = a.o + (size_t)plane * n * n;
    for (int i = threadIdx.x * 4; i < n * n; i += blockDim.x * 4) {
        const float2* r = buf + (i >> lg) * LD + (i & (n - 1));
        const float v[4] = {r[0].x * sc, r[1].x * sc, r[2].x * sc, r[3].x * sc};
        *reinterpret_cast<float4*>(o + i) = make_float4(fabsf(v[0]), fabsf(v[1]), fabsf(v[2]), fabsf(v[3]));
        if (a.sgn) {
            float sg[4];
#pragma unroll
            for (int k = 0; k < 4; ++k) sg[k] = (v[k] > 0.f) ? 1.0f : ((v[k] < 0.f) ? -1.0f : 0.0f);
            { typedef float f4 __attribute__((ext_vector_type(4))); __builtin_nontemporal_store((f4){sg[0], sg[1], sg[2], sg[3]}, reinterpret_cast<f4*>(a.sgn + (size_t)plane * n * n + i)); }
        }
    }
}


#define FFT_HP(n) ((n) / 2 + 1)
__host__ __device__ constexpr int fftr_threads(int lg) { return lg >= 7 ? 1024 : (lg >= 6 ? 512 : 256); }

template <int LG>
__device__ __forceinline__ void fftr_unpack(float2* buf, const float2* tw) {
    constexpr int n = 1 << LG, half = n >> 1, quarter = n >> 2, HP = FFT_HP(n);
    for (int it = threadIdx.x; it < n * (quarter + 1); it += blockDim.x) {
        const int y = it & (n - 1), k = it >> LG;
        float2* row = buf + y * HP;
        if (k == 0) {
            const float2 A = row[0];
            row[0] = make_float2(A.x + A.y, 0.0f);
            row[half] = make_float2(A.x - A.y, 0.0f);
        } else {
            const int qa = (int)(__brev((unsigned)k) >> (33 - LG)), qb = (int)(__brev((unsigned)(half - k)) >> (33 - LG));
            const float2 A = row[qa], B = row[qb], w = tw[k];
            const float ex = 0.5f * (A.x + B.x), ey = 0.5f * (A.y - B.y);
            const float ox = 0.5f * (A.y + B.y), oy = 0.5f * (B.x - A.x);
            const float px = w.x * ox - w.y * oy, py = w.x * oy + w.y * ox;
            row[qa] = make_float2(ex + px, ey + py);
            row[qb] = make_float2(ex - px, py - ey);
        }
    }
    __syncthreads();
}
template <int LG>
__device__ __forceinline__ void fftr_pack(float2* buf, const float2* tw) {
    constexpr int n = 1 << LG, half = n >> 1, quarter = n >> 2, HP = FFT_HP(n);
    for (int it = threadIdx.x; it < n * (quarter + 1); it += blockDim.x) {
        const int y = it & (n - 1), k = it >> LG;
        float2* row = buf + y * HP;
        if (k == 0) {
            const float a = row[0].x, b = row[half].x;
            row[0] = make_float2(a + b, a - b);
        } else {
            const int qa = (int)(__brev((unsigned)k) >> (33 - LG)), qb = (int)(__brev((unsigned)(half - k)) >> (33 - LG));
            const float2 A = row[qa], B = row[qb], w = tw[k];
            const float ex = A.x + B.x, ey = A.y - B.y;
            const float dx = A.x - B.x, dy = A.y + B.y;
            const float ox = w.x * dx + w.y * dy, oy = w.x * dy - w.y * dx;
            row[qa] = make_float2(ex - oy, ey + ox);
            row[qb] = make_float2(ex + oy, ox - ey);
        }
    }
    __syncthreads();
}
template <int LG> __device__ __forceinline__ void fftr_rows_fwd(float2* buf, const float2* tw) {
    fft_lines<false, 0, true, false, false, true>(buf, tw, LG - 1, LG, FFT_HP(1 << LG), 1, LG);
    fftr_unpack<LG>(buf, tw);
}
template <int LG> __device__ __forceinline__ void fftr_rows_inv(float2* buf, const float2* tw) {
    fftr_pack<LG>(buf, tw);
    fft_lines<true, 0, true, false, false, true>(buf, tw, LG - 1, LG, FFT_HP(1 << LG), 1, LG);
}
template <bool INVERSE, int LG> __device__ __forceinline__ void fftr_cols(float2* buf, const float2* tw) {
    fft_lines<INVERSE, 2, false, false, false, true>(buf, tw, LG, LG, 1, FFT_HP(1 << LG));
}
__device__ __forceinline__ void fftr_bin(int it, int n, int lg, int& q, int& c) {
    const int half = n >> 1;
    if (it < n * half) { q = it >> (lg - 1); c = it & (half - 1); }
    else { q = it - n * half; c = half; }
}

#ifdef LG_FFT_STAMPS
__device__ unsigned long long fft_stamps[256][12];
#define FFT_STAMP(i) do { if (threadIdx.x == 0 && blockIdx.x < 256) fft_stamps[blockIdx.x][i] = __builtin_readcyclecounter(); } while (0)
#else
#define FFT_STAMP(i) do { } while (0)
#endif
template <int LG, int NTH>
__global__ void __launch_bounds__(NTH, (LG >= 7 && NTH == 512) ? 4 : 1) k_fftmix_r(FftArgs a) {
    extern __shared__ float2 smem2[];
    constexpr int lg = LG, n = 1 << LG, half = n >> 1, HP = FFT_HP(n);
    float2* buf = smem2;
    float2* tw = smem2 + n * HP;
    FFT_STAMP(0);
    const int plane = blockIdx.x;
    const int ch = plane % a.ch;
    const float* g = a.g + (size_t)plane * n * n;
    constexpr int NLD = (n * n / 4 + NTH - 1) / NTH;
    {
        float4 v[NLD];
#pragma unroll
        for (int k = 0; k < NLD; ++k) { const int i = (k * NTH + (int)threadIdx.x) * 4; v[k] = *reinterpret_cast<const float4*>(g + (i < n * n ? i : 0)); }
        fft_tw_from_const(tw, lg);
#pragma unroll
        for (int k = 0; k < NLD; ++k) {
            const int i = (k * NTH + (int)threadIdx.x) * 4;
            if (i < n * n) {
                float2* d = buf + (i >> lg) * HP + ((i & (n - 1)) >> 1);
                d[0] = make_float2(v[k].x, v[k].y); d[1] = make_float2(v[k].z, v[k].w);
            }
        }
    }
    __syncthreads();
    FFT_STAMP(1);
    fftr_rows_fwd<LG>(buf, tw);
    FFT_STAMP(2);
    fftr_cols<false, LG>(buf, tw);
    if (threadIdx.x < 4) buf[(threadIdx.x >> 1) * HP + (threadIdx.x & 1) * half].y = 0.0f;
    __syncthreads();
    FFT_STAMP(3);
    const long po = stage_of_unit(a.sg, plane, a.ch) * a.sg.pstride + ch;
    const float aw = a.ampw[po], ab = a.ampb[po], pw = a.phaw[po], pb = a.phab[po];
    const int splane = plane - a.sg.s0 * a.ch;
    for (int it = threadIdx.x; it < n * (half + 1); it += NTH) {
        int q, c;
        fftr_bin(it, n, lg, q, c);
        float amp, pha;
        const float2 ed = bin_edit_fwd(buf[q * HP + c], aw, ab, pw, pb, amp, pha);
        if (a.amp && splane >= 0) {
            size_t o = ((size_t)splane * n + q) * (half + 1) + c;
            __builtin_nontemporal_store(amp, a.amp + o);
            __builtin_nontemporal_store(pha, a.pha + o);
        }
        buf[q * HP + c] = ed;
    }
    __syncthreads();
    FFT_STAMP(4);
    fftr_cols<true, LG>(buf, tw);
    FFT_STAMP(5);
    fftr_rows_inv<LG>(buf, tw);
    FFT_STAMP(6);
    const float sc = 1.0f / ((float)n * (float)n);
    float* o = a.o + (size_t)plane * n * n;
    int tid_s = threadIdx.x;
    asm volatile("" : "+v"(tid_s));
#pragma unroll
    for (int k = 0; k < NLD; ++k) {
        const int i = (k * NTH + tid_s) * 4;
        if (i >= n * n) break;
        const float2* r = buf + (i >> lg) * HP + ((i & (n - 1)) >> 1);
        const float2 r0 = r[0], r1 = r[1];
        const float v[4] = {r0.x * sc, r0.y * sc, r1.x * sc, r1.y * sc};
        *reinterpret_cast<float4*>(o + i) = make_float4(fabsf(v[0]), fabsf(v[1]), fabsf(v[2]), fabsf(v[3]));
        if (a.sgn && splane >= 0) {
            float sg[4];
#pragma unroll
            for (int u = 0; u < 4; ++u) sg[u] = (v[u] > 0.f) ? 1.0f : ((v[u] < 0.f) ? -1.0f : 0.0f);
            { typedef float f4 __attribute__((ext_vector_type(4))); __builtin_nontemporal_store((f4){sg[0], sg[1], sg[2], sg[3]}, reinterpret_cast<f4*>(a.sgn + (size_t)splane * n * n + i)); }
        }
    }
    FFT_STAMP(7);
}


#define FFT_ROWS_PER_WG(n) (8192 / (n))
#define FFT_ROWS_NT 512
#define FFT_COLS_PER_WG(n) (8192 / (n))

__device__ __forceinline__ void make_twiddles(float2* tw, int n) {
    for (int k = threadIdx.x; k < (n >> 1); k += blockDim.x) {
        float ang = 2.0f * (float)k / (float)n;
        tw[k] = make_float2(cospif(ang), 0.0f - sinpif(ang));
    }
}

template <int LG>
__global__ void k_fft_rows_fwd(const float* __restrict__ in, const float* __restrict__ mul, float2* __restrict__ S, int force_real) {
    extern __shared__ float2 smem2[];
    constexpr int n = 1 << LG, lg = LG, R = FFT_ROWS_PER_WG(n), half = n >> 1, lgR = 13 - LG;
    static_assert((1 << lgR) == R, "rows per tile");
    constexpr int LD = n + 1;
    float2* buf = smem2;
    float2* tw = smem2 + R * LD;
    const size_t plane = blockIdx.x;
    const int row0 = blockIdx.y * R;
    const size_t base = (plane * n + row0) * n;
    {
        const float4* __restrict__ in4 = reinterpret_cast<const float4*>(in + base);
        float4 v[4], m[4];
#pragma unroll
        for (int k = 0; k < 4; ++k) v[k] = in4[threadIdx.x + FFT_ROWS_NT * k];
        if (mul) {
            const float4* __restrict__ mul4 = reinterpret_cast<const float4*>(mul + base);
#pragma unroll
            for (int k = 0; k < 4; ++k) m[k] = mul4[threadIdx.x + FFT_ROWS_NT * k];
        }
        make_twiddles(tw, n);
#pragma unroll
        for (int k = 0; k < 4; ++k) {
            float4 t = v[k];
            if (mul) { t.x *= m[k].x; t.y *= m[k].y; t.z *= m[k].z; t.w *= m[k].w; }
            const int i4 = threadIdx.x + FFT_ROWS_NT * k;
            const int c0 = 4 * (i4 % (n / 4));
            float2* row = buf + (i4 / (n / 4)) * LD;
            row[fft_pos<true>(c0)] = make_float2(t.x, 0.0f); row[fft_pos<true>(c0 + 1)] = make_float2(t.y, 0.0f);
            row[fft_pos<true>(c0 + 2)] = make_float2(t.z, 0.0f); row[fft_pos<true>(c0 + 3)] = make_float2(t.w, 0.0f);
        }
    }
    __syncthreads();
    fft_lines<false, false, true, false, true>(buf, tw, lg, lgR, LD, 1);
    for (int i = threadIdx.x; i < R * (half + 1); i += blockDim.x) {
        const int r = i / (half + 1), kx = i - r * (half + 1);
        float2 v = buf[r * LD + fft_pos<true>((int)(__brev((unsigned)kx) >> (32 - lg)))];
        if (force_real && (kx == 0 || kx == half)) v.y = 0.0f;
        S[(plane * n + row0 + r) * (half + 1) + kx] = v;
    }
}

template <bool BWD, int LG>
__global__ void k_fft_cols(FftArgs fa, FftBwdArgs ba, float2* __restrict__ S) {
    extern __shared__ float2 smem2[];
    constexpr int n = 1 << LG, lg = LG, CB = FFT_COLS_PER_WG(n), half = n >> 1, lgCB = 13 - LG;
    static_assert((1 << lgCB) == CB, "columns per tile");
    float2* buf = smem2;
    float2* tw = smem2 + n * CB;
    float* red = reinterpret_cast<float*>(tw + half);
    const size_t plane = blockIdx.x;
    const int chn = BWD ? ba.ch : fa.ch;
    const int ch = (int)(plane % chn);
    const int kx0 = blockIdx.y * CB;
    const int ncols = min(CB, half + 1 - kx0);
    {
        float2 v[16];
#pragma unroll
        for (int k = 0; k < 16; ++k) {
            const int i = threadIdx.x + 512 * k, y = i >> lgCB, c = i & (CB - 1);
            v[k] = S[(plane * n + y) * (half + 1) + kx0 + min(c, ncols - 1)];
        }
        make_twiddles(tw, n);
#pragma unroll
        for (int k = 0; k < 16; ++k) {
            const int i = threadIdx.x + 512 * k, c = i & (CB - 1);
            buf[i] = (c < ncols) ? v[k] : make_float2(0.f, 0.f);
        }
    }
    __syncthreads();
    fft_lines<false, false>(buf, tw, lg, lgCB, 1, CB);
    if (!BWD) {
        if (threadIdx.x < 2 * CB) {
            const int q = threadIdx.x / CB, c = threadIdx.x - q * CB;
            if (c < ncols && (kx0 + c == 0 || kx0 + c == half)) buf[q * CB + c].y = 0.0f;
        }
        __syncthreads();
    }
    const float aw = (BWD ? ba.ampw : fa.ampw)[ch], ab = (BWD ? ba.ampb : fa.ampb)[ch];
    const float pw = (BWD ? ba.phaw : fa.phaw)[ch], pb = (BWD ? ba.phab : fa.phab)[ch];
    const float nn = (float)n * (float)n;
    float s_aw = 0.f, s_ab = 0.f, s_pw = 0.f, s_pb = 0.f;
#pragma unroll 1
    for (int g = 0; g < 4; ++g) {
        float sa[4], sp[4];
        if (BWD) {
#pragma unroll
            for (int u = 0; u < 4; ++u) {
                const int i = threadIdx.x + 512 * (4 * g + u), q = i >> lgCB, c = min(i & (CB - 1), ncols - 1);
                const size_t o = (plane * n + (int)(__brev((unsigned)q) >> (32 - lg))) * (half + 1) + kx0 + c;
                sa[u] = ba.amp[o]; sp[u] = ba.pha[o];
            }
        }
#pragma unroll
        for (int u = 0; u < 4; ++u) {
            const int i = threadIdx.x + 512 * (4 * g + u);
            const int q = i >> lgCB, c = i & (CB - 1);
            if (c >= ncols) continue;
            const int ky = (int)(__brev((unsigned)q) >> (32 - lg)), kx = kx0 + c;
            const size_t o = (plane * n + ky) * (half + 1) + kx;
            if (!BWD) {
                float amp, pha;
                buf[i] = bin_edit_fwd(buf[i], aw, ab, pw, pb, amp, pha);
                if (fa.amp) { __builtin_nontemporal_store(amp, fa.amp + o); __builtin_nontemporal_store(pha, fa.pha + o); }
            } else {
                const float cw = (kx == 0 || kx == half) ? 1.0f : 2.0f;
                buf[i] = bin_edit_bwd(buf[i], cw, nn, sa[u], sp[u], aw, ab, pw, pb, s_aw, s_ab, s_pw, s_pb);
            }
        }
    }
    __syncthreads();
    fft_lines<true, false>(buf, tw, lg, lgCB, 1, CB);
    for (int i = threadIdx.x; i < n * CB; i += blockDim.x) {
        const int y = i >> lgCB, c = i & (CB - 1);
        if (c < ncols) S[(plane * n + y) * (half + 1) + kx0 + c] = buf[i];
// ... 210 lines not shown

template <bool BWD>
__global__ void k_gfft_cols(FftArgs fa, FftBwdArgs ba, float2* __restrict__ S, int h, int w, GDft d) {
    extern __shared__ float2 smem2[];
    const GLds g = gdft_carve(smem2, d);
    const size_t plane = blockIdx.x;
    const int chn = BWD ? ba.ch : fa.ch;
    const int ch = (int)(plane % chn);
    const int halfw = w >> 1, kx0 = blockIdx.y * d.L;
    const int ncols = min(d.L, halfw + 1 - kx0);
    gdft_setup(g, d);
    for (int i = threadIdx.x; i < h * d.L; i += blockDim.x) {
        const int y = i >> d.lgL, c = i & (d.L - 1);
        g.lines[(c << d.lgM) + y] = (c < ncols) ? S[(plane * h + y) * (halfw + 1) + kx0 + c] : make_float2(0.f, 0.f);
    }
    __syncthreads();
    gdft_lines(g, d);
    if (!BWD) {
        if (threadIdx.x < 2 * d.L) {
            const int q = threadIdx.x >> d.lgL, c = threadIdx.x & (d.L - 1);
            if (c < ncols && (kx0 + c == 0 || kx0 + c == halfw)) g.lines[(c << d.lgM) + (q ? (h >> 1) : 0)].y = 0.0f;
        }
        __syncthreads();
    }
    const float aw = (BWD ? ba.ampw : fa.ampw)[ch], ab = (BWD ? ba.ampb : fa.ampb)[ch];
    const float pw = (BWD ? ba.phaw : fa.phaw)[ch], pb = (BWD ? ba.phab : fa.phab)[ch];
    const float nn = (float)h * (float)w;
    float s_aw = 0.f, s_ab = 0.f, s_pw = 0.f, s_pb = 0.f;
    for (int i = threadIdx.x; i < d.L * h; i += blockDim.x) {
        const int c = i / h, ky = i - c * h;
        if (c >= ncols) continue;
        const int kx = kx0 + c, idx = (c << d.lgM) + ky;
        const size_t o = (plane * h + ky) * (halfw + 1) + kx;
        float2 v;
        if (!BWD) {
            float amp, pha;
            v = bin_edit_fwd(g.lines[idx], aw, ab, pw, pb, amp, pha);
            if (fa.amp) { __builtin_nontemporal_store(amp, fa.amp + o); __builtin_nontemporal_store(pha, fa.pha + o); }
        } else {
            const float cw = (kx == 0 || kx == halfw) ? 1.0f : 2.0f;
            v = bin_edit_bwd(g.lines[idx], cw, nn, ba.amp[o], ba.pha[o], aw, ab, pw, pb, s_aw, s_ab, s_pw, s_pb);
        }
        g.lines[idx] = make_float2(v.x, -v.y);
    }
    __syncthreads();
    gdft_lines(g, d);
    for (int i = threadIdx.x; i < h * d.L; i += blockDim.x) {
        const int y = i >> d.lgL, c = i & (d.L - 1);
        if (c < ncols) {
            const float2 v = g.lines[(c << d.lgM) + y];
            S[(plane * h + y) * (halfw + 1) + kx0 + c] = make_float2(v.x, -v.y);
        }
    }
    if (BWD) {
        float v[4] = {s_aw, s_ab, s_pw, s_pb};
        const int wave = threadIdx.x >> 6, lane = threadIdx.x & 63, nw = blockDim.x >> 6;
#pragma unroll
        for (int i = 0; i < 4; ++i) {
#pragma unroll
            for (int off = 32; off > 0; off >>= 1) v[i] += __shfl_xor(v[i], off);
            if (lane == 0) g.red[wave * 4 + i] = v[i];
        }
        __syncthreads();
        if (threadIdx.x < 4) {
            float sum = 0.f;
            for (int k = 0; k < nw; ++k) sum += g.red[k * 4 + threadIdx.x];
            ba.part[(((plane / chn) * gridDim.y + blockIdx.y) * chn + ch) * 4 + threadIdx.x] = sum;
        }
    }
}

__global__ void k_gfft_rows_inv(const float2* __restrict__ S, float* __restrict__ out, float* __restrict__ sgn, int h, int w, GDft d, int absout) {
    extern __shared__ float2 smem2[];
    const GLds g = gdft_carve(smem2, d);
    const size_t plane = blockIdx.x;
    const int row0 = blockIdx.y * d.L, halfw = w >> 1;
    gdft_setup(g, d);
    for (int i = threadIdx.x; i < d.L * (halfw + 1); i += blockDim.x) {
        const int l = i / (halfw + 1), kx = i - l * (halfw + 1), row = row0 + l;
        const float2 v = (row < h) ? S[(plane * h + row) * (halfw + 1) + kx] : make_float2(0.f, 0.f);
        float2* ln = g.lines + (l << d.lgM);
        if (kx == 0 || kx == halfw) {
            ln[kx] = make_float2(v.x, 0.0f);
        } else {
            ln[kx] = make_float2(v.x, -v.y);
            ln[w - kx] = v;
        }
    }
    __syncthreads();
    gdft_lines(g, d);
    const float sc = 1.0f / ((float)h * (float)w);
    for (int i = threadIdx.x; i < d.L * w; i += blockDim.x) {
        const int l = i / w, x = i - l * w, row = row0 + l;
        if (row >= h) continue;
        const float v = g.lines[(l << d.lgM) + x].x * sc;
        const size_t o = (plane * h + row) * w + x;
        if (absout) {
            out[o] = fabsf(v);
            if (sgn) sgn[o] = (v > 0.f) ? 1.0f : ((v < 0.f) ? -1.0f : 0.0f);
        } else {
            out[o] = v;
        }
    }
}

static int fft_generic_col_groups(int h, int w) { const GDft dh = gdft_plan(h); return (w / 2 + 1 + dh.L - 1) / dh.L; }

static int launch_fft_generic(const FftArgs* fa, const FftBwdArgs* ba, int h, int w, hipStream_t s) {
    const int planes = fa ? fa->planes : ba->planes;
    float2* S = reinterpret_cast<float2*>(fa ? fa->scratch : ba->scratch);
    if (!S) { lg_set_error("fftmix: plane %dx%d needs the generic path but no scratch buffer was given", h, w); return -2; }
    if (h < 8 || w < 8 || h > 1024 || w > 1024 || (h & 7) || (w & 7)) {
        lg_set_error("fftmix: plane %dx%d unsupported (sides: multiples of 8, 8..1024)", h, w);
        return -2;
    }
    static DeviceOnce attr_once;
    if (int rc = lds_attr_once(attr_once, "fft generic", 160 * 1024 - 1024, k_gfft_rows_fwd, k_gfft_cols<false>, k_gfft_cols<true>, k_gfft_rows_inv)) return rc;
    const GDft dw = gdft_plan(w), dh = gdft_plan(h);
    const size_t lds_r = gdft_lds_bytes(dw), lds_c = gdft_lds_bytes(dh);
    dim3 grows(planes, (h + dw.L - 1) / dw.L), gcols(planes, fft_generic_col_groups(h, w));
    if (fa) {
        k_gfft_rows_fwd<<<grows, 1024, lds_r, s>>>(fa->g, nullptr, S, h, w, dw, 1);
        LG_CHECK_LAUNCH();
        FftBwdArgs dummy;
        memset(&dummy, 0, sizeof(dummy));
        k_gfft_cols<false><<<gcols, 1024, lds_c, s>>>(*fa, dummy, S, h, w, dh);
        LG_CHECK_LAUNCH();
        k_gfft_rows_inv<<<grows, 1024, lds_r, s>>>(S, fa->o, fa->sgn, h, w, dw, 1);
        LG_CHECK_LAUNCH();
    } else {
        k_gfft_rows_fwd<<<grows, 1024, lds_r, s>>>(ba->do2, ba->sgn, S, h, w, dw, 0);
        LG_CHECK_LAUNCH();
        FftArgs dummy;
        memset(&dummy, 0, sizeof(dummy));
        k_gfft_cols<true><<<gcols, 1024, lds_c, s>>>(dummy, *ba, S, h, w, dh);
        LG_CHECK_LAUNCH();
        k_gfft_rows_inv<<<grows, 1024, lds_r, s>>>(S, ba->dg, nullptr, h, w, dw, 0);
        LG_CHECK_LAUNCH();
    }
    return 0;
}

int launch_fftmix(const FftArgs& a, hipStream_t s) {
    ProfScope prof__(LG_K_FFT, s, a.sg.n);
    const int ph = a.h ? a.h : a.n, pw = a.w ? a.w : a.n;
    if (a.sg.n > 1 && (a.full || fft_is_generic(ph, pw) || ph > 128)) { lg_set_error("fftmix: only the real-input in-LDS kernel takes several stages in one launch"); return -2; }
    if (fft_is_generic(ph, pw)) return launch_fft_generic(&a, nullptr, ph, pw, s);
    int n = ph, lg = 0;
    while ((1 << lg) < n) ++lg;
    if (n > 128) return launch_fft_split(&a, nullptr, s);
    if (!a.full) {
        if (int rc = fft_const_twiddles()) return rc;
        static DeviceOnce attr_r;
        if (int rc = lds_attr_once(attr_r, "fftmix", 80 * 1024 - 512, k_fftmix_r<7, 1024>, k_fftmix_r<7, 512>)) return rc;
        const size_t ldsr = ((size_t)n * FFT_HP(n) + n / 2) * sizeof(float2);
        switch (lg) {
            case 3: k_fftmix_r<3, fftr_threads(3)><<<a.planes, fftr_threads(3), ldsr, s>>>(a); break;
            case 4: k_fftmix_r<4, fftr_threads(4)><<<a.planes, fftr_threads(4), ldsr, s>>>(a); break;
            case 5: k_fftmix_r<5, fftr_threads(5)><<<a.planes, fftr_threads(5), ldsr, s>>>(a); break;
            case 6: k_fftmix_r<6, fftr_threads(6)><<<a.planes, fftr_threads(6), ldsr, s>>>(a); break;
            default:
                if (a.planes <= lg_num_cus()) k_fftmix_r<7, 1024><<<a.planes, 1024, ldsr, s>>>(a);
                else k_fftmix_r<7, 512><<<a.planes, 512, ldsr, s>>>(a);
                break;
        }
        LG_CHECK_LAUNCH();
        return 0;
    }
    size_t lds = ((size_t)n * FFT_LD(n) + n / 2) * sizeof(float2);
    static DeviceOnce attr_once;
    if (int rc = lds_attr_once(attr_once, "fftmix", 160 * 1024 - 1024, k_fftmix<7>)) return rc;
    int threads = fft_threads(lg);
    switch (lg) {
        case 3: k_fftmix<3><<<a.planes, threads, lds, s>>>(a); break;
        case 4: k_fftmix<4><<<a.planes, threads, lds, s>>>(a); break;
        case 5: k_fftmix<5><<<a.planes, threads, lds, s>>>(a); break;
        case 6: k_fftmix<6><<<a.planes, threads, lds, s>>>(a); break;
        default: k_fftmix<7><<<a.planes, threads, lds, s>>>(a); break;
    }
    LG_CHECK_LAUNCH();
    return 0;
}

template <int LG>
__global__ void k_fftmix_bwd(FftBwdArgs a) {
    extern __shared__ float2 smem2[];
    constexpr int lg = LG, n = 1 << LG, half = n >> 1;
    constexpr int LD = FFT_LD(n);
    float2* buf = smem2;
    float2* tw = smem2 + n * LD;
    float* red = reinterpret_cast<float*>(tw + half);
    const int plane = blockIdx.x;
    const int ch = plane % a.ch;
    const size_t base = (size_t)plane * n * n;
    for (int k = threadIdx.x; k < half; k += blockDim.x) {
        float ang = 2.0f * (float)k / (float)n;
        tw[k] = make_float2(cospif(ang), 0.0f - sinpif(ang));
    }
    constexpr int NTH = fft_threads(LG), NLD = (n * n / 4 + NTH - 1) / NTH, NBIN = n * (half + 1), NIT = (NBIN + NTH - 1) / NTH;
    {
        float4 u[NLD], sg[NLD];
#pragma unroll
        for (int k = 0; k < NLD; ++k) {
            const int i = (k * NTH + (int)threadIdx.x) * 4, ic = i < n * n ? i : 0;
            u[k] = *reinterpret_cast<const float4*>(a.do2 + base + ic);
            sg[k] = *reinterpret_cast<const float4*>(a.sgn + base + ic);
        }
#pragma unroll
        for (int k = 0; k < NLD; ++k) {
            const int i = (k * NTH + (int)threadIdx.x) * 4;
            if (i < n * n) {
                float2* d = buf + (i >> lg) * LD + (i & (n - 1));
                d[0] = make_float2(u[k].x * sg[k].x, 0.0f); d[1] = make_float2(u[k].y * sg[k].y, 0.0f);
                d[2] = make_float2(u[k].z * sg[k].z, 0.0f); d[3] = make_float2(u[k].w * sg[k].w, 0.0f);
            }
        }
    }
    __syncthreads();
    fft_pass<false, false>(buf, tw, n, lg);
    fft_pass<false, true>(buf, tw, n, lg);
    const float aw = a.ampw[ch], ab = a.ampb[ch], pw = a.phaw[ch], pb = a.phab[ch];
    const float nn = (float)n * (float)n;
    float s_aw = 0.f, s_ab = 0.f, s_pw = 0.f, s_pb = 0.f;
    float ampv[NIT], phav[NIT];
#pragma unroll
    for (int k = 0; k < NIT; ++k) {
        const int it = k * NTH + (int)threadIdx.x, itc = it < NBIN ? it : 0;
        int q, p, c;
        half_bin(itc, n, lg, q, p, c);
        const size_t o = ((size_t)plane * n + q) * (half + 1) + c;
        ampv[k] = a.amp[o];
        phav[k] = a.pha[o];
    }
#pragma unroll
    for (int k = 0; k < NIT; ++k) {
        const int it = k * NTH + (int)threadIdx.x;
        if (it < NBIN) {
            int q, p, c;
            half_bin(it, n, lg, q, p, c);
            const float cf = (c == 0 || c == half) ? 1.0f : 2.0f;
            buf[q * LD + p] = bin_edit_bwd(buf[q * LD + p], cf, nn, ampv[k], phav[k], aw, ab, pw, pb, s_aw, s_ab, s_pw, s_pb);
        }
    }
    __syncthreads();
    fft_pass<true, true>(buf, tw, n, lg);
    fft_pass<true, false>(buf, tw, n, lg);
    const float sc = 1.0f / nn;
    for (int i = threadIdx.x * 4; i < n * n; i += blockDim.x * 4) {
        const float2* r = buf + (i >> lg) * LD + (i & (n - 1));
        *reinterpret_cast<float4*>(a.dg + base + i) = make_float4(r[0].x * sc, r[1].x * sc, r[2].x * sc, r[3].x * sc);
    }
    float v[4] = {s_aw, s_ab, s_pw, s_pb};
    const int wave = threadIdx.x >> 6, lane = threadIdx.x & 63, nw = blockDim.x >> 6;
#pragma unroll
    for (int i = 0; i < 4; ++i) {
#pragma unroll
        for (int off = 32; off > 0; off >>= 1) v[i] += __shfl_xor(v[i], off);
        if (lane == 0) red[wave * 4 + i] = v[i];
    }
    __syncthreads();
    if (threadIdx.x < 4) {
        float s = 0.f;
        for (int w = 0; w < nw; ++w) s += red[w * 4 + threadIdx.x];
        a.part[(size_t)plane * 4 + threadIdx.x] = s;
    }
}

template <int LG, int NTH>
__global__ void __launch_bounds__(NTH, (LG >= 7 && NTH == 512) ? 4 : 1) k_fftmix_bwd_r(FftBwdArgs a) {
    extern __shared__ float2 smem2[];
    constexpr int lg = LG, n = 1 << LG, half = n >> 1, HP = FFT_HP(n);
    float2* buf = smem2;
    float2* tw = smem2 + n * HP;
    float* red = reinterpret_cast<float*>(tw + half);
    const int plane = blockIdx.x;
    const int ch = plane % a.ch;
    const size_t base = (size_t)plane * n * n;
    constexpr int NLD = (n * n / 4 + NTH - 1) / NTH, NBIN = n * (half + 1), NIT = (NBIN + NTH - 1) / NTH;
    constexpr int LB = NLD > 4 ? 4 : NLD;
#pragma unroll
    for (int b = 0; b < NLD; b += LB) {
        float4 u[LB], sg[LB];
#pragma unroll
        for (int k = 0; k < LB; ++k) {
            const int i = ((b + k) * NTH + (int)threadIdx.x) * 4, ic = i < n * n ? i : 0;
            u[k] = *reinterpret_cast<const float4*>(a.do2 + base + ic);
            sg[k] = *reinterpret_cast<const float4*>(a.sgn + base + ic);
        }
        if (b == 0) fft_tw_from_const(tw, lg);
#pragma unroll
        for (int k = 0; k < LB; ++k) {
            const int i = ((b + k) * NTH + (int)threadIdx.x) * 4;
            if (i >= n * n) continue;
            float2* d = buf + (i >> lg) * HP + ((i & (n - 1)) >> 1);
            d[0] = make_float2(u[k].x * sg[k].x, u[k].y * sg[k].y); d[1] = make_float2(u[k].z * sg[k].z, u[k].w * sg[k].w);
        }
    }
    __syncthreads();
    fftr_rows_fwd<LG>(buf, tw);
    fftr_cols<false, LG>(buf, tw);
    const float aw = a.ampw[ch], ab = a.ampb[ch], pw = a.phaw[ch], pb = a.phab[ch];
    const float nn = (float)n * (float)n;
    float s_aw = 0.f, s_ab = 0.f, s_pw = 0.f, s_pb = 0.f;
    constexpr int EB = NIT > 9 ? 9 : NIT;
#pragma unroll 1
    for (int b = 0; b < NIT; b += EB) {
        float ampv[EB], phav[EB];
#pragma unroll
        for (int k = 0; k < EB; ++k) {
            const int it = (b + k) * NTH + (int)threadIdx.x, itc = it < NBIN ? it : 0;
            int q, c;
            fftr_bin(itc, n, lg, q, c);
            const size_t o = ((size_t)plane * n + q) * (half + 1) + c;
            ampv[k] = a.amp[o];
            phav[k] = a.pha[o];
        }
#pragma unroll
        for (int k = 0; k < EB; ++k) {
            const int it = (b + k) * NTH + (int)threadIdx.x;
            if (it < NBIN) {
                int q, c;
                fftr_bin(it, n, lg, q, c);
                const float cf = (c == 0 || c == half) ? 1.0f : 2.0f;
                buf[q * HP + c] = bin_edit_bwd(buf[q * HP + c], cf, nn, ampv[k], phav[k], aw, ab, pw, pb, s_aw, s_ab, s_pw, s_pb);
            }
        }
    }
    __syncthreads();
    fftr_cols<true, LG>(buf, tw);
    fftr_rows_inv<LG>(buf, tw);
    const float sc = 1.0f / nn;
    int tid_s = threadIdx.x;
    asm volatile("" : "+v"(tid_s));
#pragma unroll
    for (int k = 0; k < NLD; ++k) {
        const int i = (k * NTH + tid_s) * 4;
        if (i >= n * n) break;
        const float2* r = buf + (i >> lg) * HP + ((i & (n - 1)) >> 1);
        const float2 r0 = r[0], r1 = r[1];
        *reinterpret_cast<float4*>(a.dg + base + i) = make_float4(r0.x * sc, r0.y * sc, r1.x * sc, r1.y * sc);
    }
    float v[4] = {s_aw, s_ab, s_pw, s_pb};
    const int wave = threadIdx.x >> 6, lane = threadIdx.x & 63, nw = NTH >> 6;
#pragma unroll
    for (int i = 0; i < 4; ++i) {
#pragma unroll
        for (int off = 32; off > 0; off >>= 1) v[i] += __shfl_xor(v[i], off);
        if (lane == 0) red[wave * 4 + i] = v[i];
    }
    __syncthreads();
    if (threadIdx.x < 4) {
        float s = 0.f;
        for (int w = 0; w < nw; ++w) s += red[w * 4 + threadIdx.x];
        a.part[(size_t)plane * 4 + threadIdx.x] = s;
    }
}

static int fft_bwd_col_groups(int h, int w) {
    if (fft_is_generic(h, w)) return fft_generic_col_groups(h, w);
    return h > 128 ? (h / 2 + 1 + FFT_COLS_PER_WG(h) - 1) / FFT_COLS_PER_WG(h) : 1;
}
size_t fft_bwd_part_floats(int planes, int h, int w) { return (size_t)planes * fft_bwd_col_groups(h, w) * 4; }
static int fft_bwd_reduce(const FftBwdArgs& a, hipStream_t s) {
    float* dst[4] = {a.d_ampw, a.d_ampb, a.d_phaw, a.d_phab};
    for (int k = 0; k < 4; ++k) {
        ReduceJob j;
        j.slab = a.part + k; j.dst = dst[k]; j.dst2 = nullptr;
        j.nslices = (long)(a.planes / a.ch) * fft_bwd_col_groups(a.h ? a.h : a.n, a.w ? a.w : a.n); j.slice_stride = (long)a.ch * 4;
        j.rows = a.ch; j.cols = 1; j.row_stride = 4; j.ld = 1; j.rows_valid = a.ch; j.cols_valid = 1;
        int rc = launch_reduce_job(j, s);
        if (rc) return rc;
    }
    return 0;
}
static int launch_fftmix_bwd_kernels(const FftBwdArgs& a, hipStream_t s);
int launch_fftmix_bwd(const FftBwdArgs& a, hipStream_t s) {
    if (!a.part) { lg_set_error("fftmix_bwd: partial-sum scratch missing"); return -2; }
    int rc = launch_fftmix_bwd_kernels(a, s);
    return rc ? rc : fft_bwd_reduce(a, s);
}
static int launch_fftmix_bwd_kernels(const FftBwdArgs& a, hipStream_t s) {
    ProfScope prof__(LG_K_FFT_BWD, s);
    const int ph = a.h ? a.h : a.n, pw = a.w ? a.w : a.n;
    if (fft_is_generic(ph, pw)) return launch_fft_generic(nullptr, &a, ph, pw, s);
    int n = ph, lg = 0;
    while ((1 << lg) < n) ++lg;
    if (n > 128) return launch_fft_split(nullptr, &a, s);
    if (!a.full) {
        if (int rc = fft_const_twiddles()) return rc;
        static DeviceOnce attr_r;
        if (int rc = lds_attr_once(attr_r, "fftmix_bwd", 80 * 1024 - 512, k_fftmix_bwd_r<7, 1024>, k_fftmix_bwd_r<7, 512>)) return rc;
        const size_t ldsr = ((size_t)n * FFT_HP(n) + n / 2) * sizeof(float2) + 64 * sizeof(float);
        switch (lg) {
            case 3: k_fftmix_bwd_r<3, fftr_threads(3)><<<a.planes, fftr_threads(3), ldsr, s>>>(a); break;
            case 4: k_fftmix_bwd_r<4, fftr_threads(4)><<<a.planes, fftr_threads(4), ldsr, s>>>(a); break;
            case 5: k_fftmix_bwd_r<5, fftr_threads(5)><<<a.planes, fftr_threads(5), ldsr, s>>>(a); break;
            case 6: k_fftmix_bwd_r<6, fftr_threads(6)><<<a.planes, fftr_threads(6), ldsr, s>>>(a); break;
            default:
                if (a.planes <= lg_num_cus()) k_fftmix_bwd_r<7, 1024><<<a.planes, 1024, ldsr, s>>>(a);
                else k_fftmix_bwd_r<7, 512><<<a.planes, 512, ldsr, s>>>(a);
                break;
        }
        LG_CHECK_LAUNCH();
        return 0;
    }
    size_t lds = ((size_t)n * FFT_LD(n) + n / 2) * sizeof(float2) + 64 * sizeof(float);
    static DeviceOnce attr_once;
    if (int rc = lds_attr_once(attr_once, "fftmix_bwd", 160 * 1024 - 1024, k_fftmix_bwd<7>)) return rc;
    int threads = fft_threads(lg);
    switch (lg) {
        case 3: k_fftmix_bwd<3><<<a.planes, threads, lds, s>>>(a); break;
        case 4: k_fftmix_bwd<4><<<a.planes, threads, lds, s>>>(a); break;
        case 5: k_fftmix_bwd<5><<<a.planes, threads, lds, s>>>(a); break;
        case 6: k_fftmix_bwd<6><<<a.planes, threads, lds, s>>>(a); break;
        default: k_fftmix_bwd<7><<<a.planes, threads, lds, s>>>(a); break;
    }
    LG_CHECK_LAUNCH();
    return 0;
}
```

### lgteun_amd/csrc/k_fwd.hip

```cpp
#include <string.h>

#include "abi.h"
#include "forward.h"

int data_step_fwd(const lg_plan* pl, const float* P, int stage, const float* z_in, const float* ms, const float* pan,
                  float* z_out, float* t1, float* r, float* s1, float* pr, int B, hipStream_t s) {
    const lg_config& c = pl->cfg;
    const int planes = B * c.C, H = c.H, W = c.W;
    if (pl->route.dstep_fused) {
        DstepFwdArgs f;
        f.z = z_in; f.ms = ms; f.pan = pan; f.zout = z_out; f.t1 = t1; f.r = r; f.s1 = s1; f.pr = pr;
        f.d1w = P + pl->shared(S_D1W); f.d1b = P + pl->shared(S_D1B); f.d3w = P + pl->shared(S_D3W); f.d3b = P + pl->shared(S_D3B);
        f.dt1w = P + pl->shared(S_DT1W); f.dt1b = P + pl->shared(S_DT1B); f.dt3w = P + pl->shared(S_DT3W); f.dt3b = P + pl->shared(S_DT3B);
        f.rw = P + pl->shared(S_RW); f.rb = P + pl->shared(S_RB); f.rtw = P + pl->shared(S_RTW); f.rtb = P + pl->shared(S_RTB);
        f.eta = P + pl->eta(stage);
        f.B = B; f.C = c.C; f.N = H;
        return launch_dstep_fwd(f, s);
    }
    DwArgs a;
    memset(&a, 0, sizeof(a));
    a.C = c.C; a.planes = planes;
    int rc;
    a.in = z_in; a.out = t1; a.w9 = P + pl->shared(S_D1W); a.bias = P + pl->shared(S_D1B);
    a.hi = H; a.wi = W; a.ho = H / 2; a.wo = W / 2;
    if ((rc = launch_resample_dw(0, 0, a, s))) return rc;
    a.in = t1; a.out = r; a.w9 = P + pl->shared(S_D3W); a.bias = P + pl->shared(S_D3B); a.sub = ms;
    a.hi = H / 2; a.wi = W / 2; a.ho = H / 4; a.wo = W / 4;
    if ((rc = launch_resample_dw(0, 1, a, s))) return rc;
    a.in = r; a.out = s1; a.w9 = P + pl->shared(S_DT1W); a.bias = P + pl->shared(S_DT1B); a.sub = nullptr;
    a.hi = H / 4; a.wi = W / 4; a.ho = H / 2; a.wo = W / 2;
    if ((rc = launch_resample_dw(1, 0, a, s))) return rc;
    a.in = s1; a.out = z_out; a.w9 = P + pl->shared(S_DT3W); a.bias = P + pl->shared(S_DT3B);
    a.z = z_in; a.pan = pan; a.rw = P + pl->shared(S_RW); a.rb = P + pl->shared(S_RB);
    a.rtw = P + pl->shared(S_RTW); a.rtb = P + pl->shared(S_RTB); a.eta = P + pl->eta(stage);
    a.hi = H / 2; a.wi = W / 2; a.ho = H; a.wo = W;
    return launch_resample_dw(1, 2, a, s);
}

static int mixer_fft_fwd(const Blk& k, int B, int flags, hipStream_t s, const StageSel& sg) {
    const lg_plan* pl = k.pl;
    const BlockBufs& bb = k.b;
    FftArgs f;
    f.g = bb.g; f.o = bb.o2;
    f.amp = (flags & LG_FLAG_SAVE) ? bb.amp : nullptr;
    f.pha = (flags & LG_FLAG_SAVE) ? bb.pha : nullptr;
    f.sgn = (flags & LG_FLAG_SAVE) ? bb.sgn : nullptr;
    f.scratch = k.fft_scratch;
    f.ampw = k.p(B_AMPW); f.ampb = k.p(B_AMPB); f.phaw = k.p(B_PHAW); f.phab = k.p(B_PHAB);
    f.ch = bb.e / 2; f.planes = B * f.ch; f.n = bb.h; f.h = bb.h; f.w = bb.w; f.full = pl->route.fft_full;
    f.sg = sg;
    return launch_fftmix(f, s);
}
static int mixer_local_fwd(const Blk& k, int B, int flags, uint64_t seed, hipStream_t s, const StageSel& sg) {
    const lg_plan* pl = k.pl;
    const BlockBufs& bb = k.b;
    const MixerRoute& mr = pl->mixer(bb.e);
    AttnArgs t;
    t.x = bb.xin; t.o2 = bb.o2; t.y = bb.xmid; t.posT = k.posT; t.pos = k.p(B_POS);
    t.bf16 = mr.bf16 ? 1 : 0;
    t.ln1g = k.p(B_LN1G); t.ln1b = k.p(B_LN1B); t.qkvw = k.p(B_QKVW); t.qkvb = k.p(B_QKVB); t.projw = k.p(B_PROJW); t.projb = k.p(B_PROJB);
    t.B = B; t.h = bb.h; t.w = bb.w;
    t.dropout = (flags & LG_FLAG_DROPOUT) ? 1 : 0;
    t.seed = mix_seed(seed, k.st, k.j);
    t.sg = sg; t.sg.seed = seed; t.sg.stage0 = k.st; t.sg.blk = k.j;
    t.scales = mr.f16x2 ? k.attn_scales : nullptr;
    if ((flags & LG_FLAG_SAVE) && mr.stats) { t.save_o = bb.att_o; t.save_l = bb.att_l; }
    if (sg.n > 1 && mr.fwd == ATTN_FWD_VALU) { lg_set_error("mixer: the vector-pipe kernel takes one stage per launch"); return -2; }
    return mr.fwd == ATTN_FWD_VALU ? launch_attn(bb.e, t, s) : launch_attn_m(bb.e, t, s);
}
int block_mixer_fwd(const Blk& k, int B, int flags, uint64_t seed, hipStream_t s, const StageSel& sg) {
    if (int rc = mixer_fft_fwd(k, B, flags, s, sg)) return rc;
    return mixer_local_fwd(k, B, flags, seed, s, sg);
}

int block_ffn_fwd(const Blk& k, const Blk* next, int B, int flags, hipStream_t s, const StageSel& sg) {
    int rc;
    const BlockBufs& bb = k.b;
    const FfnRoute& fr = k.pl->ffn(bb.e);
    const unsigned saves = (flags & LG_FLAG_SAVE) ? fr.saves : 0;
    Ffn1Args a1;
    a1.x = bb.xmid; a1.a1s = (saves & FFN_SLOT_A1) ? bb.a1 : nullptr; a1.g1s = (saves & FFN_SLOT_G1) ? bb.g1 : nullptr;
    a1.ln2g = k.p(B_LN2G); a1.ln2b = k.p(B_LN2B); a1.w1 = k.p(B_W1); a1.b1 = k.p(B_B1); a1.w2 = k.p(B_W2); a1.b2 = k.p(B_B2);
    a1.P = (long)B * bb.h * bb.w;
    a1.hbf = fr.hbf ? 1 : 0;
    a1.kernel = fr.fwd[(flags & LG_FLAG_SAVE) ? 1 : 0];
    a1.wsplit = k.wsplit;
    a1.wsplit_ready = bb.e >= 32 ? 1 : 0;
    a1.scales = fr.scales ? k.ffn_scales : nullptr;
    Ffn2Args a2;
    a2.h2 = bb.h2; a2.x = bb.xmid; a2.a3s = (saves & FFN_SLOT_A3) ? bb.a3 : nullptr; a2.g3s = (saves & FFN_SLOT_G3) ? bb.g3 : nullptr; a2.y = bb.xout;
    a2.g = next ? next->b.g : nullptr;
    a2.dww = k.p(B_DWW); a2.dwb = k.p(B_DWB); a2.w3 = k.p(B_W3); a2.b3 = k.p(B_B3);
    a2.n1g = next ? next->p(B_LN1G) : nullptr;
    a2.n1b = next ? next->p(B_LN1B) : nullptr;
    a2.B = B; a2.h = bb.h; a2.w = bb.w; a2.hbf = a1.hbf;
    a1.h2 = bb.h2;
    a1.sg = sg;
    if (sg.n > 1 && a1.kernel != FFN_FWD_XR && a1.kernel != FFN_FWD_X32) { lg_set_error("ffn: this route's kernel takes one stage per launch"); return -2; }
    if (a1.kernel == FFN_FWD_UNFUSED) {
        if ((rc = launch_ffn1(bb.e, a1, s))) return rc;
        return launch_ffn2(bb.e, a2, s);
    }
    if (!saves && bb.e != 64) a1.h2 = nullptr;
    return launch_ffn_fused(bb.e, a1, a2, s);
}

int prep_stages(const lg_plan* pl, const float* P, int st0, int st1, const NetBufs& nb, hipStream_t s) {
    if (st1 <= st0) return 0;
    const float* psrc[LG_NBLK * LG_MAX_K];
    float* pdst[LG_NBLK * LG_MAX_K];
    FfnPrepJob jobs[LG_NBLK * LG_MAX_K];
    SplitWJob sj[LG_NBLK * LG_MAX_K];
    int n = 0, ns = 0, rc;
    for (int st = st0; st < st1; ++st)
        for (int j = 0; j < LG_NBLK; ++j, ++n) {
            const Blk k = nb.block(pl, P, nullptr, st, j);
            psrc[n] = k.p(B_POS); pdst[n] = nb.posT_row(st, j);
            FfnPrepJob& q = jobs[n];
            q.ln2g = k.p(B_LN2G); q.ln2b = k.p(B_LN2B); q.w1 = k.p(B_W1); q.b1 = k.p(B_B1); q.w2 = k.p(B_W2); q.b2 = k.p(B_B2);
            q.dww = k.p(B_DWW); q.dwb = k.p(B_DWB); q.w3 = k.p(B_W3);
            q.e = k.b.e;
            q.ln1g = k.p(B_LN1G); q.ln1b = k.p(B_LN1B); q.qkvw = k.p(B_QKVW); q.qkvb = k.p(B_QKVB);
            if (k.b.e < 32 || k.b.e % 32) continue;
            SplitWJob& w = sj[ns++];
            w.w1 = k.p(B_W1); w.w2 = k.p(B_W2); w.w3 = k.p(B_W3);
            w.e = k.b.e; w.np = pl->ffn(k.b.e).wsplit_np;
            w.scales = w.np == 2 ? k.ffn_scales : nullptr;
            w.out = k.wsplit;
        }
    if (pl->route.mix[0].fwd == ATTN_FWD_VALU && (rc = launch_pos_transpose_n(n, psrc, pdst, s))) return rc;
    if (pl->route.ffn[0].scales &&
        (rc = launch_ffn_scales(n, jobs, nb.ffn_scales_row(st0, 0), s, pl->route.mix[0].f16x2 ? nb.attn_scales_row(st0, 0) : nullptr))) return rc;
    return ns ? launch_split_w_jobs(ns, sj, s) : 0;
}

int lgt_fwd(const lg_plan* pl, const float* P, int stage, const float* z, float* out, const NetBufs& nb, int B, int flags, uint64_t seed,
            hipStream_t s, int nst, long zstride, int grid_cap, float* live_out) {
    const lg_config& c = pl->cfg;
    const int E = 4 * c.C;
    const bool ride = live_out != nullptr;
    int rc;
    StageSel sg;
    if (nst > 1) {
        if (!pl->stage_batch || (!ride && (flags & LG_FLAG_SAVE))) { lg_set_error("lgt_fwd: this plan / call runs one stage per pass"); return -2; }
        sg.n = nst; sg.Bs = B; sg.pstride = pl->stage_stride; sg.zstride = zstride; sg.grid_cap = grid_cap;
        nb.stage_strides(sg);
    }
    if (ride && (stage != 0 || nst != c.K || nb.live_s0 != (size_t)(nst - 1) * B)) { lg_set_error("lgt_fwd: the live stage rides behind all K-1 dead ones, in slot K-1"); return -2; }
    const int Bs = B, fdead = flags & ~LG_FLAG_SAVE;
    StageSel sgd = sg;
    if (ride) { sg.s0 = (nst - 1) * Bs; sgd.n = nst - 1; }
    B *= nst;
    const LgtSlots L{pl, P, nullptr, stage};
    Blk k[LG_NBLK], kl[LG_NBLK];
    const NetBufs lv = ride ? live_view(nb) : nb;
    for (int j = 0; j < LG_NBLK; ++j) { k[j] = nb.block(pl, P, nullptr, stage, j); kl[j] = lv.block(pl, P, nullptr, stage + nst - 1, j); }
    auto block = [&](int j, int next) -> int {
        int r;
        if (!ride) return (r = block_mixer_fwd(k[j], B, flags, seed, s, sg)) ? r : block_ffn_fwd(k[j], next < 0 ? nullptr : &k[next], B, flags, s, sg);
        if ((r = mixer_fft_fwd(k[j], B, flags, s, sg))) return r;
        if ((r = mixer_local_fwd(kl[j], Bs, flags, seed, s, StageSel())) || (r = block_ffn_fwd(kl[j], next < 0 ? nullptr : &kl[next], Bs, flags, s, StageSel()))) return r;
        if ((r = mixer_local_fwd(k[j], sgd.n * Bs, fdead, seed, s, sgd))) return r;
        return block_ffn_fwd(k[j], next < 0 ? nullptr : &k[next], sgd.n * Bs, fdead, s, sgd);
    };
    EmbedArgs ea;
    ea.z = z; ea.x = nb.x0; ea.g = nb.blk[0].g;
    ea.dww = L.p(L_PE_DWW); ea.dwb = L.p(L_PE_DWB); ea.w = L.p(L_PE_W); ea.b = L.p(L_PE_B); ea.lng = L.p(L_PE_LNG); ea.lnb = L.p(L_PE_LNB);
    ea.n1g = k[0].p(B_LN1G); ea.n1b = k[0].p(B_LN1B);
    ea.HW = c.H * c.W; ea.total = (long)B * c.H * c.W; ea.sg = sg;
    if ((rc = launch_embed(c.C, ea, s))) return rc;
    if ((rc = block(0, 1))) return rc;
    if ((rc = block(1, -1))) return rc;
    DownArgs da;
    da.x = nb.blk[1].xout; da.y = nb.blk[2].xin; da.g = nb.blk[2].g;
    da.u_save = (flags & LG_FLAG_SAVE) ? nb.u_down : nullptr;
    da.w = L.p(L_DOWNW); da.b = L.p(L_DOWNB);
    da.n1g = k[2].p(B_LN1G); da.n1b = k[2].p(B_LN1B);
    da.B = B; da.H = c.H; da.W = c.W; da.sg = sg;
    if ((rc = launch_down(E, da, s))) return rc;
    if ((rc = block(2, -1))) return rc;
    UpFuseArgs ua;
    ua.xb = nb.blk[2].xout; ua.skip = nb.blk[1].xout; ua.y = nb.blk[3].xin; ua.g = nb.blk[3].g;
    ua.t_save = (flags & LG_FLAG_SAVE) ? nb.t_up : nullptr;
    ua.upw = L.p(L_UPW); ua.upb = L.p(L_UPB); ua.fw = L.p(L_FUSEW); ua.fb = L.p(L_FUSEB);
    ua.n1g = k[3].p(B_LN1G); ua.n1b = k[3].p(B_LN1B);
    ua.B = B; ua.H = c.H; ua.W = c.W; ua.sg = sg;
    if ((rc = launch_upfuse(E, ua, s))) return rc;
    if ((rc = block(3, 4))) return rc;
    if ((rc = block(4, -1))) return rc;
    TailArgs ta;
    ta.x = nb.blk[4].xout; ta.z = z; ta.out = out; ta.out_last = live_out;
    ta.w = L.p(L_TAILW); ta.b = L.p(L_TAILB);
    ta.HW = c.H * c.W; ta.total = (long)B * c.H * c.W; ta.sg = sg;
    return launch_tail(c.C, ta, s);
}

static float* dead_out(const lg_plan* pl, const NetBufs& nb, int i, int B) {
    return nb.deadout + (pl->stage_batch ? (size_t)i * B * pl->cfg.C * pl->cfg.H * pl->cfg.W : 0);
}
static bool dead_as_one_pass(const lg_plan* pl, int flags) { return pl->stage_batch && !(flags & LG_FLAG_STAGEWISE); }
static int dead_stages(const lg_plan* pl, const float* P, const NetBufs& nb, int B, int flags, uint64_t seed, hipStream_t s) {
    flags &= ~LG_FLAG_SAVE;
// ... 60 lines not shown
```

### lgteun_amd/csrc/kernels.h

```cpp
#pragma once
#include "common.h"

struct DwArgs {
    const float* in;
    float* out;
    const float* w9;
    const float* bias;
    const float* sub;
    const float* z;
    const float* pan;
    const float* rw;
    const float* rb;
    const float* rtw;
    const float* rtb;
    const float* eta;
    int C, planes, hi, wi, ho, wo;
};
int launch_resample_dw(int mode, int epi, const DwArgs& a, hipStream_t s);
int launch_resample(int mode, const float* x, float* y, int planes, int hi, int wi, hipStream_t s);
struct DstepFwdArgs {
    const float* z;
    const float* ms;
    const float* pan;
    float* zout;
    float *t1, *r, *s1;
    float* pr;
    const float *d1w, *d1b, *d3w, *d3b, *dt1w, *dt1b, *dt3w, *dt3b, *rw, *rb, *rtw, *rtb, *eta;
    int B, C, N;
};
bool dstep_fused_ok(int C, int H, int W);
int launch_dstep_fwd(const DstepFwdArgs& a, hipStream_t s);

struct StageSel {
    int n = 1;
    int Bs = 0;
    long pstride = 0;
    long zstride = 0;
    int fs_stride = 0;
    int as_stride = 0;
    long ws_stride = 0;
    int grid_cap = 0;
    int s0 = 0;
    uint64_t seed = 0;
    int stage0 = 0, blk = 0;
};
#ifdef __HIPCC__
__device__ __forceinline__ int stage_of(const StageSel& sg, int b) { return sg.n > 1 ? __builtin_amdgcn_readfirstlane(b / sg.Bs) : 0; }
__device__ __forceinline__ int stage_of_unit(const StageSel& sg, int unit, int per_sample) { return sg.n > 1 ? __builtin_amdgcn_readfirstlane(unit / (per_sample * sg.Bs)) : 0; }

struct StageRun { int run0, run1, base; };
__host__ __device__ inline StageRun stage_run_halves(int units, int half, int wg) {
    const int first = wg < half ? 1 : 0, j = wg - (first ? 0 : half);
    return {(int)((unsigned)j * (unsigned)units / (unsigned)half), (int)(((unsigned)j + 1u) * (unsigned)units / (unsigned)half), first ? 0 : units};
}
__host__ __device__ inline StageRun stage_run_even(int units, int grid, int wg) { return stage_run_halves(units, grid, wg); }
__host__ __device__ inline StageRun stage_run_pairs(int npairs, int grid, int wg) { return stage_run_halves(npairs, grid >> 1, wg); }
__host__ __device__ inline StageRun stage_run_chunk(int units, int grid, int wg, int u) {
    const StageRun ch = stage_run_halves(units, u ? grid >> 1 : grid, wg);
    if (!u) return ch;
    const int len = ch.run1 - ch.run0;
    int n1 = (len * u + 4) >> 3;
    n1 = n1 > len - 1 ? len - 1 : n1;
    n1 = n1 < 1 ? 1 : n1;
    return ch.base ? StageRun{ch.run0 + n1, ch.run1, 0} : StageRun{ch.run0, ch.run0 + n1, 0};
}
__host__ __device__ inline int stage_seg_end(int st, int run1, int per_stage) { return run1 < (st + 1) * per_stage ? run1 : (st + 1) * per_stage; }
#endif

struct StripGeo { int tiles_x, SH, strips_y, nstrips, grid; };
inline StripGeo strip_geometry(int h, int w, int B, int Bh, int wgs, int grid_cap) {
    StripGeo q;
    q.tiles_x = (w + 15) / 16;
    q.SH = (h + 7) / 8 * 8;
    while (q.SH > 16 && (long)Bh * q.tiles_x * ((h + q.SH - 1) / q.SH) < wgs) q.SH = (q.SH / 2 + 7) / 8 * 8;
    q.strips_y = (h + q.SH - 1) / q.SH;
    q.nstrips = B * q.tiles_x * q.strips_y;
    q.grid = q.nstrips < wgs ? q.nstrips : wgs;
    if (grid_cap > 0 && q.grid > grid_cap) q.grid = grid_cap;
    return q;
}
struct XrGeo : StripGeo { int dS; };
XrGeo ffn_xr_geometry(int h, int w, int B, int Bs, int n, int grid_cap);
struct AttnMGeo { int nwin, nquads, grid, uneven; };
AttnMGeo attn_m_geometry(int HC, int h, int w, int B, int n, int grid_cap, int per_cu);

struct EmbedArgs {
    const float* z;
    float* x;
    float* g;
    const float *dww, *dwb, *w, *b, *lng, *lnb, *n1g, *n1b;
    int HW;
    long total;
    StageSel sg;
};
int launch_embed(int C, const EmbedArgs& a, hipStream_t s);

struct DownArgs {
    const float* x;
    float* y;
    float* g;
    float* u_save;
    const float *w, *b, *n1g, *n1b;
    int B, H, W;
    StageSel sg;
};
int launch_down(int E, const DownArgs& a, hipStream_t s);

struct UpFuseArgs {
    const float* xb;
    const float* skip;
    float* y;
    float* g;
    float* t_save;
    const float *upw, *upb, *fw, *fb, *n1g, *n1b;
    int B, H, W;
    StageSel sg;
};
int launch_upfuse(int E, const UpFuseArgs& a, hipStream_t s);

struct TailArgs {
    const float* x;
    const float* z;
    float* out;
    float* out_last = nullptr;
    const float *w, *b;
    int HW;
    long total;
    StageSel sg;
};
int launch_tail(int C, const TailArgs& a, hipStream_t s);

struct FftArgs {
    const float* g;
    float* o;
    float* amp;
    float* pha;
    float* sgn;
    float* scratch;
    const float *ampw, *ampb, *phaw, *phab;
    int planes, ch, n;
    int h, w;
    int full = 0;
    StageSel sg;
};
int launch_fftmix(const FftArgs& a, hipStream_t s);
size_t fft_scratch_floats(int planes, int n);
size_t fft_scratch_floats_hw(int planes, int h, int w);
bool fft_is_generic(int h, int w);

struct AttnArgs {
    const float* x;
    const float* o2;
    float* y;
    const float* posT;
    const float* pos;
    const float *ln1g, *ln1b, *qkvw, *qkvb, *projw, *projb;
    int B, h, w;
    int dropout;
    uint64_t seed;
    int bf16;
    float* save_o = nullptr;
    float* save_l = nullptr;
    const float* scales = nullptr;
    StageSel sg;
};
int launch_attn(int e, const AttnArgs& a, hipStream_t s);
int launch_attn_m(int e, const AttnArgs& a, hipStream_t s);
int launch_pos_transpose_n(int n, const float* const* pos, float* const* posT, hipStream_t s);

struct Ffn1Args {
    const float* x;
    void* a1s;
    void* g1s;
    void* h2;
    int hbf;
    int kernel;
    const float *ln2g, *ln2b, *w1, *b1, *w2, *b2;
    long P;
    void* wsplit;
    int wsplit_ready = 0;
    const float* scales;
    StageSel sg;
};
struct FfnPrepJob { const float *ln2g, *ln2b, *w1, *b1, *w2, *b2, *dww, *dwb, *w3; int e; const float *ln1g, *ln1b, *qkvw, *qkvb; };
#define LG_MAX_FFN_PREP_JOBS 40
struct FfnPrepTable { FfnPrepJob j[LG_MAX_FFN_PREP_JOBS]; };
int launch_ffn_scales(int n, const FfnPrepJob* jobs, float* out, hipStream_t s, float* attn_out = nullptr);
struct SplitWJob { const float *w1, *w2, *w3, *scales; void* out; int e, np; };
struct SplitWTable { SplitWJob j[LG_MAX_FFN_PREP_JOBS]; };
int launch_split_w_jobs(int n, const SplitWJob* jobs, hipStream_t s);
int launch_ffn1(int e, const Ffn1Args& a, hipStream_t s);
struct Ffn2Args {
    const void* h2;
    const float* x;
    void* a3s;
    void* g3s;
    int hbf;
    float* y;
    float* g;
    const float *dww, *dwb, *w3, *b3, *n1g, *n1b;
    int B, h, w;
};
int launch_ffn2(int e, const Ffn2Args& a, hipStream_t s);
int launch_ffn_fused(int e, const Ffn1Args& a1, const Ffn2Args& a2, hipStream_t s);
int launch_ffn_xs(const Ffn1Args& a1, const Ffn2Args& a2, hipStream_t s);
int launch_ffn_xr(const Ffn1Args& a1, const Ffn2Args& a2, hipStream_t s);
int launch_ffn_x32(const Ffn1Args& a1, const Ffn2Args& a2, hipStream_t s);
size_t ffn_wsplit_bytes(int e);
int launch_split_w(const float* w1, const float* w2, const float* w3, void* out, int e, int np, hipStream_t s, const float* scales = nullptr);
int launch_ffn_x64(const Ffn1Args& a1, const Ffn2Args& a2, hipStream_t s);

int launch_ln_split(int e, const float* x, const float* n1g, const float* n1b, float* g, int B, int HW, hipStream_t s);
```

### lgteun_amd/csrc/route.h

```cpp
#pragma once
#include <stddef.h>
#include "abi.h"

enum FfnFwdKernel {
    FFN_FWD_XR,
    FFN_FWD_XS,
    FFN_FWD_X32,
    FFN_FWD_X64,
    FFN_FWD_STRIP,
    FFN_FWD_TILE,
    FFN_FWD_UNFUSED
};
enum FfnArith { FFN_ARITH_F32, FFN_ARITH_BF16, FFN_ARITH_F16X2, FFN_ARITH_BF16X3 };
enum FfnSlot { FFN_SLOT_A1 = 1, FFN_SLOT_G1 = 2, FFN_SLOT_H2 = 4, FFN_SLOT_A3 = 8, FFN_SLOT_G3 = 16 };
enum FfnDwBwdKernel { FFN_DWBWD_XS, FFN_DWBWD_H, FFN_DWBWD_TILE };
enum Ffn1BwdKernel { FFN1_BWD_XS, FFN1_BWD_X32, FFN1_BWD_TILE };

struct FfnRoute {
    int e, h, w;
    FfnFwdKernel fwd[2];
    FfnArith arith;
    bool hbf;
    bool scales;
    int wsplit_np;
    unsigned saves;
    bool pre;
    bool a3_pre() const { return pre || dw == FFN_DWBWD_XS; }
    FfnDwBwdKernel dw;
    Ffn1BwdKernel px;
    bool bwd_scales;
    bool wgrad_w2, wgrad_w1, wgrad_w3;
};

enum AttnFwdKernel { ATTN_FWD_M, ATTN_FWD_VALU };
enum AttnBwdKernel { ATTN_BWD_F, ATTN_BWD_R3, ATTN_BWD_R3_CORE_M };
struct MixerRoute {
    int e;
    AttnFwdKernel fwd;
    bool bf16;
    bool f16x2;
    bool stats;
    AttnBwdKernel bwd;
};

struct LgRoute {
    FfnRoute ffn[2];
    MixerRoute mix[2];
    bool dstep_fused;
    bool fft_full;
    bool reduce_per_block;
};

int lg_resolve_route(const lg_config& cfg, LgRoute* r);
int lg_describe_route(const lg_config& cfg, const LgRoute& r, char* buf, size_t n);
```

### lgteun_amd/csrc/route.hip

```cpp
#include <stdio.h>

#include "kernels.h"
#include "bwd_kernels.h"

static void resolve_ffn(const lg_config& cfg, int e, int h, int w, FfnRoute& f) {
    const uint32_t v = cfg.variant;
    const int impl = (int)(v & LG_VAR_FFN_IMPL_MASK);
    const uint32_t sv = v & LG_VAR_FFN_SAVE_MASK;
    const bool split = impl == 0;
    const bool strips = (h & 7) == 0 && (w & 15) == 0;
    f.e = e; f.h = h; f.w = w;
    f.hbf = cfg.precision == 1 && e != 64;
    f.scales = cfg.precision == 0 && split && !(v & LG_VAR_FFN_BF16X3);
    f.arith = !split ? FFN_ARITH_F32 : f.hbf ? FFN_ARITH_BF16 : f.scales ? FFN_ARITH_F16X2 : FFN_ARITH_BF16X3;
    f.wsplit_np = e < 32 ? 0 : f.hbf ? 1 : f.scales ? 2 : 3;

    const int save_form = (e != 16 || !split) ? 5 : sv == LG_VAR_FFN_SAVE5 ? 5 : (sv == LG_VAR_FFN_SAVE3 ? (cfg.precision == 0 ? 3 : 5) : 2);
    f.pre = save_form != 5;
    f.px = (e == 16 && save_form == 2) || (e == 32 && split && !(v & LG_VAR_FFN_BWD32_PAIR)) ? FFN1_BWD_XS : (e == 32 && split) ? FFN1_BWD_X32 : FFN1_BWD_TILE;
    const bool dw_tile = (v & LG_VAR_FFN_DWBWD_TILE) && !(e == 16 && f.hbf);
    f.dw = ((e == 16 && save_form == 2) || (e == 32 && split)) && !dw_tile && strips ? FFN_DWBWD_XS : FFN_DWBWD_TILE;
    const bool xr_built = split && !(v & LG_VAR_FFN_XS) && (f.hbf || f.scales);
    if (e == 16 && f.dw == FFN_DWBWD_XS && (v & LG_VAR_FFN_H3_RECOMPUTE) && xr_built && !f.hbf) f.dw = FFN_DWBWD_H;
    f.bwd_scales = f.px == FFN1_BWD_XS && f.dw != FFN_DWBWD_TILE && f.scales && !(v & LG_VAR_FFN_BWD_BF16X3);
    f.wgrad_w2 = f.px != FFN1_BWD_XS && !ffn1_bwd_fuses_w2(e, f.pre);
    f.wgrad_w1 = f.px != FFN1_BWD_XS && !ffn1_bwd_fuses_w1(e);
    f.wgrad_w3 = f.dw == FFN_DWBWD_TILE;

    f.saves = FFN_SLOT_H2;
    if (f.dw == FFN_DWBWD_XS || f.wgrad_w3) f.saves |= FFN_SLOT_A3;
    if (f.dw == FFN_DWBWD_TILE && !f.pre) f.saves |= FFN_SLOT_G3;
    if (f.px != FFN1_BWD_XS) f.saves |= FFN_SLOT_A1 | (f.pre ? 0 : FFN_SLOT_G1);

    FfnFwdKernel k;
    if (e == 16) k = split ? FFN_FWD_XS : FFN_FWD_STRIP;
    else if (e == 32) k = split ? FFN_FWD_X32 : FFN_FWD_TILE;
    else k = split ? FFN_FWD_X64 : FFN_FWD_UNFUSED;
    f.fwd[0] = f.fwd[1] = k;
    if (e == 16 && xr_built) {
        f.fwd[0] = FFN_FWD_XR;
        if (!(f.saves & ~(unsigned)(FFN_SLOT_H2 | FFN_SLOT_A3))) f.fwd[1] = FFN_FWD_XR;
    }
}

static void resolve_mixer(const lg_config& cfg, int e, MixerRoute& m) {
    const uint32_t v = cfg.variant;
    m.e = e;
    m.fwd = (v & LG_VAR_ATTN_FWD_VALU) ? ATTN_FWD_VALU : ATTN_FWD_M;
    m.bf16 = cfg.precision == 1;
    m.f16x2 = cfg.precision == 0 && m.fwd == ATTN_FWD_M && !(v & LG_VAR_ATTN_BF16X3) && !(v & LG_VAR_FFN_IMPL_MASK) && !(v & LG_VAR_FFN_BF16X3);
    m.bwd = (attn_bwd_fused(e) && !(v & LG_VAR_ATTN_BWD_R3)) ? ATTN_BWD_F : (e == 32 && (v & LG_VAR_ATTN_BWD_CORE_M)) ? ATTN_BWD_R3_CORE_M : ATTN_BWD_R3;
    m.stats = cfg.precision == 0 && m.fwd == ATTN_FWD_M && !(v & LG_VAR_ATTN_BWD_RESTATS) && m.bwd != ATTN_BWD_R3_CORE_M;
}

int lg_resolve_route(const lg_config& cfg, LgRoute* r) {
    const uint32_t v = cfg.variant;
    if (v & ~LG_VAR_ALL) { lg_set_error("plan_create: unknown variant bits 0x%x", v & ~LG_VAR_ALL); return -2; }
    if ((v & LG_VAR_FFN_SAVE_MASK) == LG_VAR_FFN_SAVE_MASK) { lg_set_error("plan_create: invalid FFN save variant"); return -2; }
    if ((v & LG_VAR_FFN_IMPL_MASK) > LG_VAR_FFN_STRIP) { lg_set_error("plan_create: FFN implementation field (LG_VAR_FFN_IMPL_MASK) = %u: only 0 and LG_VAR_FFN_STRIP exist", v & LG_VAR_FFN_IMPL_MASK); return -2; }
    if (cfg.precision == 1 && (v & LG_VAR_FFN_IMPL_MASK)) { lg_set_error("plan_create: FFN implementation field (LG_VAR_FFN_IMPL_MASK): LG_VAR_FFN_STRIP is an fp32 kernel set, precision = 1 has none"); return -2; }
    const int E = 4 * cfg.C;
    resolve_ffn(cfg, E, cfg.H, cfg.W, r->ffn[0]);
    resolve_ffn(cfg, 2 * E, cfg.H / 2, cfg.W / 2, r->ffn[1]);
    resolve_mixer(cfg, E, r->mix[0]);
    resolve_mixer(cfg, 2 * E, r->mix[1]);
    r->dstep_fused = !(v & LG_VAR_DSTEP_TILES) && dstep_fused_ok(cfg.C, cfg.H, cfg.W);
    r->fft_full = (v & LG_VAR_FFT_FULL) != 0;
    r->reduce_per_block = (v & LG_VAR_REDUCE_PER_BLOCK) != 0;
    return 0;
}

static const char* slots_text(unsigned slots, bool a1_pre, bool a3_pre, char (&buf)[48]) {
    int n = 0;
    buf[0] = 0;
    auto add = [&](unsigned bit, const char* name) { if (slots & bit) n += snprintf(buf + n, sizeof(buf) - n, "%s%s", n ? "," : "", name); };
    add(FFN_SLOT_A1, a1_pre ? "a1:h1" : "a1"); add(FFN_SLOT_G1, "g1"); add(FFN_SLOT_H2, "h2"); add(FFN_SLOT_A3, a3_pre ? "a3:h3" : "a3"); add(FFN_SLOT_G3, "g3");
    return n ? buf : "-";
}

int lg_describe_route(const lg_config& cfg, const LgRoute& r, char* buf, size_t n) {
    static const char* const fwd_names[] = {"k_ffn_xr", "k_ffn_xs", "k_ffn_x32", "k_ffn1_x64+k_ffn2_x64", "k_ffn_strip", "k_ffn_fused", "k_ffn1+k_ffn2"};
    static const char* const arith_names[] = {"f32", "bf16", "f16x2", "bf16x3"};
    static const char* const dw_names[] = {"k_ffn_dw_bwd_xs", "k_ffn_dw_bwd_h", "k_ffn_dw_bwd"};
    static const char* const px_names[] = {"k_ffn1_bwd_xs", "k_ffn1_bwd_x32", "k_ffn1_bwd"};
    static const char* const attn_bwd_names[] = {"k_attn_bwd_f", "k_attn_bwd_core+k_attn_bwd_epi", "k_attn_bwd_core_m+k_attn_bwd_epi"};
    size_t off = 0;
    bool full = false;
    auto put = [&](const char* fmt, auto... a) {
        const int k = snprintf(buf + off, n - off, fmt, a...);
        if (k < 0 || (size_t)k >= n - off) full = true; else off += (size_t)k;
    };
    if (!buf || n == 0) { lg_set_error("plan_describe: null argument"); return -1; }
    put("net C=%d %dx%d precision=%d variant=0x%x: dstep=%s fft=%s reduce=%s\n", cfg.C, cfg.H, cfg.W, cfg.precision, cfg.variant,
        r.dstep_fused ? "fused" : "tiles", r.fft_full ? "k_fftmix" : "k_fftmix_r", r.reduce_per_block ? "per_block" : "merged");
    for (int l = 0; l < 2 && !full; ++l) {
        const FfnRoute& f = r.ffn[l];
        const MixerRoute& m = r.mix[l];
        const char* attn = m.fwd == ATTN_FWD_M ? "k_attn_m" : "k_attn";
        const char* attn_arith = m.fwd == ATTN_FWD_VALU ? "f32" : m.bf16 ? "bf16" : m.f16x2 ? "f16x2" : "bf16x3";
        char sb[48];
        put("L%d e=%d %dx%d fwd: ffn=%s arith=%s hidden=%s | mixer=%s arith=%s\n", l, f.e, f.h, f.w, fwd_names[f.fwd[0]], arith_names[f.arith],
            f.hbf ? "bf16" : "fp32", attn, attn_arith);
        put("L%d e=%d %dx%d save: ffn=%s writes=%s | mixer=%s writes=%s\n", l, f.e, f.h, f.w, fwd_names[f.fwd[1]],
            slots_text(f.saves, f.pre, f.a3_pre(), sb), attn, m.stats ? "o,l" : "-");
        unsigned reads = FFN_SLOT_H2;
        if (f.dw == FFN_DWBWD_XS) reads |= FFN_SLOT_A3;
        if (f.dw == FFN_DWBWD_TILE) reads |= f.pre ? FFN_SLOT_A3 : FFN_SLOT_G3;
        if (f.px != FFN1_BWD_XS) reads |= f.pre ? FFN_SLOT_A1 : FFN_SLOT_G1;
        if (f.wgrad_w2) reads |= FFN_SLOT_A1;
        if (f.wgrad_w3) reads |= FFN_SLOT_A3;
        put("L%d e=%d %dx%d bwd: ffn=%s+%s%s%s%s arith=%s reads=%s | mixer=%s stats=%s\n", l, f.e, f.h, f.w, dw_names[f.dw], px_names[f.px],
            f.wgrad_w2 ? "+k_wgrad(W2)" : "", f.wgrad_w1 ? "+k_wgrad(W1)" : "", f.wgrad_w3 ? "+k_wgrad(W3)" : "",
            f.px == FFN1_BWD_TILE ? "f32" : f.px == FFN1_BWD_X32 ? "bf16x3" : f.hbf ? "bf16" : f.bwd_scales ? "f16x2" : "bf16x3", slots_text(reads, f.pre, f.a3_pre(), sb), attn_bwd_names[m.bwd],
            m.stats ? "saved" : "recomputed");
    }
    if (full) { lg_set_error("plan_describe: buffer of %zu bytes is too small", n); return -3; }
    return 0;
}
```

Baseline: 6635 image-pairs/sec.

## Fuse last column-FFT levels with spectral edit in real FFT mixer kernels

In the forward and backward real-FFT mixer kernels for 64 and 128 sizes, the last three column butterfly levels are now done in registers together with the per-bin amplitude/phase edit and the first three inverse levels. This removes an LDS round trip and barriers between the column FFT, the bin edit and the inverse column FFT. The backward kernel also prefetches saved amp/pha for the next item. The pack/unpack loops are reshaped so the k==0 iteration also handles k=quarter, dropping a partial extra pass. An env switch restores the old path; the change adds register pressure and more complex indexing.

```diff
diff --git a/include/lgteun_hip.h b/include/lgteun_hip.h
--- a/include/lgteun_hip.h
+++ b/include/lgteun_hip.h
@@ -58,7 +58,8 @@
 #define LG_VAR_FFN_H3_RECOMPUTE (1u << 15)
 #define LG_VAR_ATTN_BWD_RESTATS (1u << 16)
 #define LG_VAR_REDUCE_PER_BLOCK (1u << 17)
-#define LG_VAR_ALL 0x3ffffu
+#define LG_VAR_FFT_UNFUSED (1u << 21)
+#define LG_VAR_ALL 0x23ffffu
 
 typedef struct lg_plan lg_plan;
 
diff --git a/lgteun_amd/_lib.py b/lgteun_amd/_lib.py
--- a/lgteun_amd/_lib.py
+++ b/lgteun_amd/_lib.py
@@ -36,6 +36,7 @@
 LG_VAR_FFN_H3_RECOMPUTE = 1 << 15
 LG_VAR_ATTN_BWD_RESTATS = 1 << 16
 LG_VAR_REDUCE_PER_BLOCK = 1 << 17
+LG_VAR_FFT_UNFUSED = 1 << 21
 LG_OPT_ADAM, LG_OPT_ADAMW, LG_OPT_SGD, LG_OPT_RMSPROP = 0, 1, 2, 3
 LG_OPT_AMSGRAD, LG_OPT_NESTEROV, LG_OPT_CENTERED = 1, 2, 4
 LG_DT_U8, LG_DT_U16, LG_DT_F32 = 0, 1, 2
@@ -76,6 +77,8 @@
         v |= LG_VAR_ATTN_BWD_RESTATS
     if env.get('LG_REDUCE', '') == 'per_block':
         v |= LG_VAR_REDUCE_PER_BLOCK
+    if env.get('LG_FFT_FUSE', '') == '0':
+        v |= LG_VAR_FFT_UNFUSED
     return v
 
 
diff --git a/lgteun_amd/csrc/api.hip b/lgteun_amd/csrc/api.hip
--- a/lgteun_amd/csrc/api.hip
+++ b/lgteun_amd/csrc/api.hip
@@ -220,7 +220,7 @@
         FftArgs f;
         f.g = bb.g; f.o = y; f.amp = nullptr; f.pha = nullptr; f.sgn = nullptr; f.scratch = nb.fft_scratch;
         f.ampw = k.p(B_AMPW); f.ampb = k.p(B_AMPB); f.phaw = k.p(B_PHAW); f.phab = k.p(B_PHAB);
-        f.ch = bb.e / 2; f.planes = B * f.ch; f.n = bb.h; f.h = bb.h; f.w = bb.w; f.full = plan->route.fft_full;
+        f.ch = bb.e / 2; f.planes = B * f.ch; f.n = bb.h; f.h = bb.h; f.w = bb.w; f.full = plan->route.fft_full; f.fuse = plan->route.fft_fuse;
         return launch_fftmix(f, s);
     }
     if ((rc = prep_stages(plan, params, stage, stage + 1, nb, s))) return rc;
diff --git a/lgteun_amd/csrc/bwd_kernels.h b/lgteun_amd/csrc/bwd_kernels.h
--- a/lgteun_amd/csrc/bwd_kernels.h
+++ b/lgteun_amd/csrc/bwd_kernels.h
@@ -301,6 +301,7 @@
     int planes, ch, n;
     int h, w;
     int full = 0;
+    int fuse = 1;
 };
 size_t fft_bwd_part_floats(int planes, int h, int w);
 int launch_fftmix_bwd(const FftBwdArgs& a, hipStream_t s);
diff --git a/lgteun_amd/csrc/k_bwd.hip b/lgteun_amd/csrc/k_bwd.hip
--- a/lgteun_amd/csrc/k_bwd.hip
+++ b/lgteun_amd/csrc/k_bwd.hip
@@ -173,7 +173,7 @@
     fa.do2 = do2; fa.sgn = fb.sgn; fa.amp = fb.amp; fa.pha = fb.pha; fa.dg = dg; fa.scratch = k.fft_scratch;
     fa.ampw = k.p(B_AMPW); fa.ampb = k.p(B_AMPB); fa.phaw = k.p(B_PHAW); fa.phab = k.p(B_PHAB);
     fa.d_ampw = k.g(B_AMPW); fa.d_ampb = k.g(B_AMPB); fa.d_phaw = k.g(B_PHAW); fa.d_phab = k.g(B_PHAB);
-    fa.ch = hc; fa.planes = B * hc; fa.n = fb.h; fa.h = fb.h; fa.w = fb.w; fa.part = part; fa.full = k.pl->route.fft_full;
+    fa.ch = hc; fa.planes = B * hc; fa.n = fb.h; fa.h = fb.h; fa.w = fb.w; fa.part = part; fa.full = k.pl->route.fft_full; fa.fuse = k.pl->route.fft_fuse;
     return launch_fftmix_bwd(fa, s);
 }
 
diff --git a/lgteun_amd/csrc/k_fft.hip b/lgteun_amd/csrc/k_fft.hip
--- a/lgteun_amd/csrc/k_fft.hip
+++ b/lgteun_amd/csrc/k_fft.hip
@@ -328,14 +328,17 @@
 template <int LG>
 __device__ __forceinline__ void fftr_unpack(float2* buf, const float2* tw) {
     constexpr int n = 1 << LG, half = n >> 1, quarter = n >> 2, HP = FFT_HP(n);
-    for (int it = threadIdx.x; it < n * (quarter + 1); it += blockDim.x) {
-        const int y = it & (n - 1), k = it >> LG;
+    for (int it = threadIdx.x; it < n * quarter; it += blockDim.x) {
+        const int y = it & (n - 1);
+        int k = it >> LG;
         float2* row = buf + y * HP;
         if (k == 0) {
             const float2 A = row[0];
             row[0] = make_float2(A.x + A.y, 0.0f);
             row[half] = make_float2(A.x - A.y, 0.0f);
-        } else {
+            k = quarter;
+        }
+        {
             const int qa = (int)(__brev((unsigned)k) >> (33 - LG)), qb = (int)(__brev((unsigned)(half - k)) >> (33 - LG));
             const float2 A = row[qa], B = row[qb], w = tw[k];
             const float ex = 0.5f * (A.x + B.x), ey = 0.5f * (A.y - B.y);
@@ -350,13 +353,16 @@
 template <int LG>
 __device__ __forceinline__ void fftr_pack(float2* buf, const float2* tw) {
     constexpr int n = 1 << LG, half = n >> 1, quarter = n >> 2, HP = FFT_HP(n);
-    for (int it = threadIdx.x; it < n * (quarter + 1); it += blockDim.x) {
-        const int y = it & (n - 1), k = it >> LG;
+    for (int it = threadIdx.x; it < n * quarter; it += blockDim.x) {
+        const int y = it & (n - 1);
+        int k = it >> LG;
         float2* row = buf + y * HP;
         if (k == 0) {
             const float a = row[0].x, b = row[half].x;
             row[0] = make_float2(a + b, a - b);
-        } else {
+            k = quarter;
+        }
+        {
             const int qa = (int)(__brev((unsigned)k) >> (33 - LG)), qb = (int)(__brev((unsigned)(half - k)) >> (33 - LG));
             const float2 A = row[qa], B = row[qb], w = tw[k];
             const float ex = A.x + B.x, ey = A.y - B.y;
@@ -385,13 +391,32 @@
     else { q = it - n * half; c = half; }
 }
 
+template <bool INVERSE, int LG, int S, int ST> __device__ __forceinline__ void fftr_cols_pass(float2* buf, const float2* tw) {
+    fft_fused<INVERSE, 2, S, false, false, true>(buf, tw, LG, LG, 1, FFT_HP(1 << LG), ST, LG);
+}
+template <int LG, int FS> __device__ __forceinline__ void fftr_mid_item(int it, int& t, int& col) {
+    constexpr int half = 1 << (LG - 1), lgpl = LG - FS;
+    if (it < (half << lgpl)) { t = it >> (LG - 1); col = it & (half - 1); }
+    else { t = it - (half << lgpl); col = half; }
+}
+template <int LG, int FS> __device__ __forceinline__ void fftr_mid_request(const float* __restrict__ amp, const float* __restrict__ pha, int plane, int it,
+                                                                           float (&av)[1 << FS], float (&pv)[1 << FS]) {
+    constexpr int n = 1 << LG, half = n >> 1;
+    int t, col;
+    fftr_mid_item<LG, FS>(it, t, col);
+    const size_t o = ((size_t)plane * n + (t << FS)) * (half + 1) + col;
+#pragma unroll
+    for (int c = 0; c < (1 << FS); ++c) { av[c] = amp[o + c * (half + 1)]; pv[c] = pha[o + c * (half + 1)]; }
+}
+__host__ __device__ constexpr int fftr_fuse_levels(int lg) { return lg >= 6 ? 3 : 0; }
+
 #ifdef LG_FFT_STAMPS
-__device__ unsigned long long fft_stamps[256][12];
-#define FFT_STAMP(i) do { if (threadIdx.x == 0 && blockIdx.x < 256) fft_stamps[blockIdx.x][i] = __builtin_readcyclecounter(); } while (0)
+__device__ unsigned long long fft_stamps[1024][12];
+#define FFT_STAMP(i) do { if (threadIdx.x == 0 && blockIdx.x < 1024) fft_stamps[blockIdx.x][i] = __builtin_readcyclecounter(); } while (0)
 #else
 #define FFT_STAMP(i) do { } while (0)
 #endif
-template <int LG, int NTH>
+template <int LG, int NTH, int FS = 0>
 __global__ void __launch_bounds__(NTH, (LG >= 7 && NTH == 512) ? 4 : 1) k_fftmix_r(FftArgs a) {
     extern __shared__ float2 smem2[];
     constexpr int lg = LG, n = 1 << LG, half = n >> 1, HP = FFT_HP(n);
@@ -420,28 +445,62 @@
     FFT_STAMP(1);
     fftr_rows_fwd<LG>(buf, tw);
     FFT_STAMP(2);
-    fftr_cols<false, LG>(buf, tw);
-    if (threadIdx.x < 4) buf[(threadIdx.x >> 1) * HP + (threadIdx.x & 1) * half].y = 0.0f;
-    __syncthreads();
-    FFT_STAMP(3);
     const long po = stage_of_unit(a.sg, plane, a.ch) * a.sg.pstride + ch;
     const float aw = a.ampw[po], ab = a.ampb[po], pw = a.phaw[po], pb = a.phab[po];
     const int splane = plane - a.sg.s0 * a.ch;
-    for (int it = threadIdx.x; it < n * (half + 1); it += NTH) {
-        int q, c;
-        fftr_bin(it, n, lg, q, c);
-        float amp, pha;
-        const float2 ed = bin_edit_fwd(buf[q * HP + c], aw, ab, pw, pb, amp, pha);
-        if (a.amp && splane >= 0) {
-            size_t o = ((size_t)splane * n + q) * (half + 1) + c;
-            __builtin_nontemporal_store(amp, a.amp + o);
-            __builtin_nontemporal_store(pha, a.pha + o);
-        }
-        buf[q * HP + c] = ed;
-    }
-    __syncthreads();
-    FFT_STAMP(4);
-    fftr_cols<true, LG>(buf, tw);
+    if constexpr (FS > 0) {
+        fftr_cols_pass<false, LG, LG - FS, 0>(buf, tw);
+        FFT_STAMP(3);
+        constexpr int R = 1 << FS, items = (half + 1) << (LG - FS);
+        const bool save = a.amp && splane >= 0;
+#pragma unroll 1
+        for (int it = threadIdx.x; it < items; it += NTH) {
+            int t, col;
+            fftr_mid_item<LG, FS>(it, t, col);
+            float2* base = buf + (t << FS) * HP + col;
+            float2 v[R];
+#pragma unroll
+            for (int c = 0; c < R; ++c) v[c] = base[c * HP];
+            fft_butterflies<false, FS, true>(v, tw, 0, 0, LG);
+            if (t == 0 && (col == 0 || col == half)) { v[0].y = 0.0f; v[1].y = 0.0f; }
+            const size_t o = ((size_t)(save ? splane : 0) * n + (t << FS)) * (half + 1) + col;
+#pragma unroll
+            for (int c = 0; c < R; ++c) {
+                float amp, pha;
+                v[c] = bin_edit_fwd(v[c], aw, ab, pw, pb, amp, pha);
+                if (save) {
+                    __builtin_nontemporal_store(amp, a.amp + o + c * (half + 1));
+                    __builtin_nontemporal_store(pha, a.pha + o + c * (half + 1));
+                }
+            }
+            fft_butterflies<true, FS, true>(v, tw, 0, 0, LG);
+#pragma unroll
+            for (int c = 0; c < R; ++c) base[c * HP] = v[c];
+        }
+        __syncthreads();
+        FFT_STAMP(4);
+        fftr_cols_pass<true, LG, LG - FS, FS>(buf, tw);
+    } else {
+        fftr_cols<false, LG>(buf, tw);
+        if (threadIdx.x < 4) buf[(threadIdx.x >> 1) * HP + (threadIdx.x & 1) * half].y = 0.0f;
+        __syncthreads();
+        FFT_STAMP(3);
+        for (int it = threadIdx.x; it < n * (half + 1); it += NTH) {
+            int q, c;
+            fftr_bin(it, n, lg, q, c);
+            float amp, pha;
+            const float2 ed = bin_edit_fwd(buf[q * HP + c], aw, ab, pw, pb, amp, pha);
+            if (a.amp && splane >= 0) {
+                size_t o = ((size_t)splane * n + q) * (half + 1) + c;
+                __builtin_nontemporal_store(amp, a.amp + o);
+                __builtin_nontemporal_store(pha, a.pha + o);
+            }
+            buf[q * HP + c] = ed;
+        }
+        __syncthreads();
+        FFT_STAMP(4);
+        fftr_cols<true, LG>(buf, tw);
+    }
     FFT_STAMP(5);
     fftr_rows_inv<LG>(buf, tw);
     FFT_STAMP(6);
@@ -958,16 +1017,26 @@
     if (!a.full) {
         if (int rc = fft_const_twiddles()) return rc;
         static DeviceOnce attr_r;
-        if (int rc = lds_attr_once(attr_r, "fftmix", 80 * 1024 - 512, k_fftmix_r<7, 1024>, k_fftmix_r<7, 512>)) return rc;
+        if (int rc = lds_attr_once(attr_r, "fftmix", 80 * 1024 - 512, k_fftmix_r<7, 1024>, k_fftmix_r<7, 512>,
+                                   k_fftmix_r<7, 1024, fftr_fuse_levels(7)>, k_fftmix_r<7, 512, fftr_fuse_levels(7)>)) return rc;
         const size_t ldsr = ((size_t)n * FFT_HP(n) + n / 2) * sizeof(float2);
+        const bool fuse = a.fuse != 0;
         switch (lg) {
             case 3: k_fftmix_r<3, fftr_threads(3)><<<a.planes, fftr_threads(3), ldsr, s>>>(a); break;
             case 4: k_fftmix_r<4, fftr_threads(4)><<<a.planes, fftr_threads(4), ldsr, s>>>(a); break;
             case 5: k_fftmix_r<5, fftr_threads(5)><<<a.planes, fftr_threads(5), ldsr, s>>>(a); break;
-            case 6: k_fftmix_r<6, fftr_threads(6)><<<a.planes, fftr_threads(6), ldsr, s>>>(a); break;
+            case 6:
+                if (fuse) k_fftmix_r<6, fftr_threads(6), fftr_fuse_levels(6)><<<a.planes, fftr_threads(6), ldsr, s>>>(a);
+                else k_fftmix_r<6, fftr_threads(6)><<<a.planes, fftr_threads(6), ldsr, s>>>(a);
+                break;
             default:
-                if (a.planes <= lg_num_cus()) k_fftmix_r<7, 1024><<<a.planes, 1024, ldsr, s>>>(a);
-                else k_fftmix_r<7, 512><<<a.planes, 512, ldsr, s>>>(a);
+                if (a.planes <= lg_num_cus()) {
+                    if (fuse) k_fftmix_r<7, 1024, fftr_fuse_levels(7)><<<a.planes, 1024, ldsr, s>>>(a);
+                    else k_fftmix_r<7, 1024><<<a.planes, 1024, ldsr, s>>>(a);
+                } else {
+                    if (fuse) k_fftmix_r<7, 512, fftr_fuse_levels(7)><<<a.planes, 512, ldsr, s>>>(a);
+                    else k_fftmix_r<7, 512><<<a.planes, 512, ldsr, s>>>(a);
+                }
                 break;
         }
         LG_CHECK_LAUNCH();
@@ -1072,13 +1141,14 @@
     }
 }
 
-template <int LG, int NTH>
+template <int LG, int NTH, int FS = 0>
 __global__ void __launch_bounds__(NTH, (LG >= 7 && NTH == 512) ? 4 : 1) k_fftmix_bwd_r(FftBwdArgs a) {
     extern __shared__ float2 smem2[];
     constexpr int lg = LG, n = 1 << LG, half = n >> 1, HP = FFT_HP(n);
     float2* buf = smem2;
     float2* tw = smem2 + n * HP;
     float* red = reinterpret_cast<float*>(tw + half);
+    FFT_STAMP(0);
     const int plane = blockIdx.x;
     const int ch = plane % a.ch;
     const size_t base = (size_t)plane * n * n;
@@ -1102,39 +1172,83 @@
             d[0] = make_float2(u[k].x * sg[k].x, u[k].y * sg[k].y); d[1] = make_float2(u[k].z * sg[k].z, u[k].w * sg[k].w);
         }
     }
-    __syncthreads();
-    fftr_rows_fwd<LG>(buf, tw);
-    fftr_cols<false, LG>(buf, tw);
     const float aw = a.ampw[ch], ab = a.ampb[ch], pw = a.phaw[ch], pb = a.phab[ch];
     const float nn = (float)n * (float)n;
     float s_aw = 0.f, s_ab = 0.f, s_pw = 0.f, s_pb = 0.f;
-    constexpr int EB = NIT > 9 ? 9 : NIT;
+    if constexpr (FS > 0) {
+        constexpr int R = 1 << FS, items = (half + 1) << (LG - FS);
+        float ampv[R], phav[R];
+        fftr_mid_request<LG, FS>(a.amp, a.pha, plane, (int)threadIdx.x < items ? (int)threadIdx.x : 0, ampv, phav);
+        __syncthreads();
+        FFT_STAMP(1);
+        fftr_rows_fwd<LG>(buf, tw);
+        FFT_STAMP(2);
+        fftr_cols_pass<false, LG, LG - FS, 0>(buf, tw);
+        FFT_STAMP(3);
 #pragma unroll 1
-    for (int b = 0; b < NIT; b += EB) {
-        float ampv[EB], phav[EB];
-#pragma unroll
-        for (int k = 0; k < EB; ++k) {
-            const int it = (b + k) * NTH + (int)threadIdx.x, itc = it < NBIN ? it : 0;
-            int q, c;
-            fftr_bin(itc, n, lg, q, c);
-            const size_t o = ((size_t)plane * n + q) * (half + 1) + c;
-            ampv[k] = a.amp[o];
-            phav[k] = a.pha[o];
-        }
-#pragma unroll
-        for (int k = 0; k < EB; ++k) {
-            const int it = (b + k) * NTH + (int)threadIdx.x;
-            if (it < NBIN) {
+        for (int it = threadIdx.x; it < items; it += NTH) {
+            float an[R], pn[R];
+            const bool more = it + NTH < items;
+            if (more) fftr_mid_request<LG, FS>(a.amp, a.pha, plane, it + NTH, an, pn);
+            int t, col;
+            fftr_mid_item<LG, FS>(it, t, col);
+            float2* cb = buf + (t << FS) * HP + col;
+            float2 v[R];
+#pragma unroll
+            for (int c = 0; c < R; ++c) v[c] = cb[c * HP];
+            fft_butterflies<false, FS, true>(v, tw, 0, 0, LG);
+            const float cf = (col == 0 || col == half) ? 1.0f : 2.0f;
+#pragma unroll
+            for (int c = 0; c < R; ++c) v[c] = bin_edit_bwd(v[c], cf, nn, ampv[c], phav[c], aw, ab, pw, pb, s_aw, s_ab, s_pw, s_pb);
+            fft_butterflies<true, FS, true>(v, tw, 0, 0, LG);
+#pragma unroll
+            for (int c = 0; c < R; ++c) cb[c * HP] = v[c];
+            if (more) {
+#pragma unroll
+                for (int c = 0; c < R; ++c) { ampv[c] = an[c]; phav[c] = pn[c]; }
+            }
+        }
+        __syncthreads();
+        FFT_STAMP(4);
+        fftr_cols_pass<true, LG, LG - FS, FS>(buf, tw);
+    } else {
+        __syncthreads();
+        FFT_STAMP(1);
+        fftr_rows_fwd<LG>(buf, tw);
+        FFT_STAMP(2);
+        fftr_cols<false, LG>(buf, tw);
+        FFT_STAMP(3);
+        constexpr int EB = NIT > 9 ? 9 : NIT;
+#pragma unroll 1
+        for (int b = 0; b < NIT; b += EB) {
+            float ampv[EB], phav[EB];
+#pragma unroll
+            for (int k = 0; k < EB; ++k) {
+                const int it = (b + k) * NTH + (int)threadIdx.x, itc = it < NBIN ? it : 0;
                 int q, c;
-                fftr_bin(it, n, lg, q, c);
-                const float cf = (c == 0 || c == half) ? 1.0f : 2.0f;
-                buf[q * HP + c] = bin_edit_bwd(buf[q * HP + c], cf, nn, ampv[k], phav[k], aw, ab, pw, pb, s_aw, s_ab, s_pw, s_pb);
+                fftr_bin(itc, n, lg, q, c);
+                const size_t o = ((size_t)plane * n + q) * (half + 1) + c;
+                ampv[k] = a.amp[o];
+                phav[k] = a.pha[o];
             }
-        }
-    }
-    __syncthreads();
-    fftr_cols<true, LG>(buf, tw);
+#pragma unroll
+            for (int k = 0; k < EB; ++k) {
+                const int it = (b + k) * NTH + (int)threadIdx.x;
+                if (it < NBIN) {
+                    int q, c;
+                    fftr_bin(it, n, lg, q, c);
+                    const float cf = (c == 0 || c == half) ? 1.0f : 2.0f;
+                    buf[q * HP + c] = bin_edit_bwd(buf[q * HP + c], cf, nn, ampv[k], phav[k], aw, ab, pw, pb, s_aw, s_ab, s_pw, s_pb);
+                }
+            }
+        }
+        __syncthreads();
+        FFT_STAMP(4);
+        fftr_cols<true, LG>(buf, tw);
+    }
+    FFT_STAMP(5);
     fftr_rows_inv<LG>(buf, tw);
+    FFT_STAMP(6);
     const float sc = 1.0f / nn;
     int tid_s = threadIdx.x;
     asm volatile("" : "+v"(tid_s));
@@ -1146,6 +1260,7 @@
         const float2 r0 = r[0], r1 = r[1];
         *reinterpret_cast<float4*>(a.dg + base + i) = make_float4(r0.x * sc, r0.y * sc, r1.x * sc, r1.y * sc);
     }
+    FFT_STAMP(7);
     float v[4] = {s_aw, s_ab, s_pw, s_pb};
     const int wave = threadIdx.x >> 6, lane = threadIdx.x & 63, nw = NTH >> 6;
 #pragma unroll
@@ -1195,16 +1310,26 @@
     if (!a.full) {
         if (int rc = fft_const_twiddles()) return rc;
         static DeviceOnce attr_r;
-        if (int rc = lds_attr_once(attr_r, "fftmix_bwd", 80 * 1024 - 512, k_fftmix_bwd_r<7, 1024>, k_fftmix_bwd_r<7, 512>)) return rc;
+        if (int rc = lds_attr_once(attr_r, "fftmix_bwd", 80 * 1024 - 512, k_fftmix_bwd_r<7, 1024>, k_fftmix_bwd_r<7, 512>,
+                                   k_fftmix_bwd_r<7, 1024, fftr_fuse_levels(7)>, k_fftmix_bwd_r<7, 512, fftr_fuse_levels(7)>)) return rc;
         const size_t ldsr = ((size_t)n * FFT_HP(n) + n / 2) * sizeof(float2) + 64 * sizeof(float);
+        const bool fuse = a.fuse != 0;
         switch (lg) {
             case 3: k_fftmix_bwd_r<3, fftr_threads(3)><<<a.planes, fftr_threads(3), ldsr, s>>>(a); break;
             case 4: k_fftmix_bwd_r<4, fftr_threads(4)><<<a.planes, fftr_threads(4), ldsr, s>>>(a); break;
             case 5: k_fftmix_bwd_r<5, fftr_threads(5)><<<a.planes, fftr_threads(5), ldsr, s>>>(a); break;
-            case 6: k_fftmix_bwd_r<6, fftr_threads(6)><<<a.planes, fftr_threads(6), ldsr, s>>>(a); break;
+            case 6:
+                if (fuse) k_fftmix_bwd_r<6, fftr_threads(6), fftr_fuse_levels(6)><<<a.planes, fftr_threads(6), ldsr, s>>>(a);
+                else k_fftmix_bwd_r<6, fftr_threads(6)><<<a.planes, fftr_threads(6), ldsr, s>>>(a);
+                break;
             default:
-                if (a.planes <= lg_num_cus()) k_fftmix_bwd_r<7, 1024><<<a.planes, 1024, ldsr, s>>>(a);
-                else k_fftmix_bwd_r<7, 512><<<a.planes, 512, ldsr, s>>>(a);
+                if (a.planes <= lg_num_cus()) {
+                    if (fuse) k_fftmix_bwd_r<7, 1024, fftr_fuse_levels(7)><<<a.planes, 1024, ldsr, s>>>(a);
+                    else k_fftmix_bwd_r<7, 1024><<<a.planes, 1024, ldsr, s>>>(a);
+                } else {
+                    if (fuse) k_fftmix_bwd_r<7, 512, fftr_fuse_levels(7)><<<a.planes, 512, ldsr, s>>>(a);
+                    else k_fftmix_bwd_r<7, 512><<<a.planes, 512, ldsr, s>>>(a);
+                }
                 break;
         }
         LG_CHECK_LAUNCH();
diff --git a/lgteun_amd/csrc/k_fwd.hip b/lgteun_amd/csrc/k_fwd.hip
--- a/lgteun_amd/csrc/k_fwd.hip
+++ b/lgteun_amd/csrc/k_fwd.hip
@@ -47,7 +47,7 @@
     f.sgn = (flags & LG_FLAG_SAVE) ? bb.sgn : nullptr;
     f.scratch = k.fft_scratch;
     f.ampw = k.p(B_AMPW); f.ampb = k.p(B_AMPB); f.phaw = k.p(B_PHAW); f.phab = k.p(B_PHAB);
-    f.ch = bb.e / 2; f.planes = B * f.ch; f.n = bb.h; f.h = bb.h; f.w = bb.w; f.full = pl->route.fft_full;
+    f.ch = bb.e / 2; f.planes = B * f.ch; f.n = bb.h; f.h = bb.h; f.w = bb.w; f.full = pl->route.fft_full; f.fuse = pl->route.fft_fuse;
     f.sg = sg;
     return launch_fftmix(f, s);
 }
diff --git a/lgteun_amd/csrc/kernels.h b/lgteun_amd/csrc/kernels.h
--- a/lgteun_amd/csrc/kernels.h
+++ b/lgteun_amd/csrc/kernels.h
@@ -141,6 +141,7 @@
     int planes, ch, n;
     int h, w;
     int full = 0;
+    int fuse = 1;
     StageSel sg;
 };
 int launch_fftmix(const FftArgs& a, hipStream_t s);
diff --git a/lgteun_amd/csrc/route.h b/lgteun_amd/csrc/route.h
--- a/lgteun_amd/csrc/route.h
+++ b/lgteun_amd/csrc/route.h
@@ -48,6 +48,7 @@
     MixerRoute mix[2];
     bool dstep_fused;
     bool fft_full;
+    bool fft_fuse;
     bool reduce_per_block;
 };
 
diff --git a/lgteun_amd/csrc/route.hip b/lgteun_amd/csrc/route.hip
--- a/lgteun_amd/csrc/route.hip
+++ b/lgteun_amd/csrc/route.hip
@@ -66,6 +66,7 @@
     resolve_mixer(cfg, 2 * E, r->mix[1]);
     r->dstep_fused = !(v & LG_VAR_DSTEP_TILES) && dstep_fused_ok(cfg.C, cfg.H, cfg.W);
     r->fft_full = (v & LG_VAR_FFT_FULL) != 0;
+    r->fft_fuse = !(v & LG_VAR_FFT_UNFUSED);
     r->reduce_per_block = (v & LG_VAR_REDUCE_PER_BLOCK) != 0;
     return 0;
 }
@@ -91,8 +92,8 @@
         if (k < 0 || (size_t)k >= n - off) full = true; else off += (size_t)k;
     };
     if (!buf || n == 0) { lg_set_error("plan_describe: null argument"); return -1; }
-    put("net C=%d %dx%d precision=%d variant=0x%x: dstep=%s fft=%s reduce=%s\n", cfg.C, cfg.H, cfg.W, cfg.precision, cfg.variant,
-        r.dstep_fused ? "fused" : "tiles", r.fft_full ? "k_fftmix" : "k_fftmix_r", r.reduce_per_block ? "per_block" : "merged");
+    put("net C=%d %dx%d precision=%d variant=0x%x: dstep=%s fft=%s reduce=%s%s\n", cfg.C, cfg.H, cfg.W, cfg.precision, cfg.variant,
+        r.dstep_fused ? "fused" : "tiles", r.fft_full ? "k_fftmix" : "k_fftmix_r", r.reduce_per_block ? "per_block" : "merged", r.fft_fuse ? "" : " fft_fuse=off");
     for (int l = 0; l < 2 && !full; ++l) {
         const FfnRoute& f = r.ffn[l];
         const MixerRoute& m = r.mix[l];
```

New measurement: 6677 image-pairs/sec (median of 6 runs). Within noise of the previous version (+0.6%).
